# orottier/web-audio-api-rs

Hardware: NVIDIA H100
Metric: offline render-quanta/sec (48kHz stereo, 128-frame) (higher is better)
Workload: dtype f64 filter state / f32 PCM

## Files before the change

### include/wae.h

```cpp
#ifndef WAE_H
#define WAE_H

#include <stddef.h>
#include <stdint.h>

#ifdef __cplusplus
extern "C" {
#endif

#ifndef WAE_API
#define WAE_API __attribute__((visibility("default")))
#endif

#define WAE_RENDER_QUANTUM_SIZE 128u
#define WAE_MAX_CHANNELS 32u

typedef int32_t wae_status;
enum {
    WAE_OK = 0,
    WAE_INVALID_ARGUMENT = 1,
    WAE_INVALID_STATE = 2,
    WAE_NOT_SUPPORTED = 3,
    WAE_UNSUPPORTED = 4,
    WAE_CUDA_ERROR = 5,
    WAE_OUT_OF_MEMORY = 6,
    WAE_NO_DEVICE = 7
};

typedef struct wae_engine wae_engine;
typedef struct wae_graph wae_graph;
typedef uint32_t wae_node_id;

enum { WAE_COUNT_MODE_MAX = 0, WAE_COUNT_MODE_CLAMPED_MAX = 1, WAE_COUNT_MODE_EXPLICIT = 2 };
enum { WAE_INTERPRETATION_SPEAKERS = 0, WAE_INTERPRETATION_DISCRETE = 1 };

typedef struct wae_channel_config {
    uint32_t count;
    uint32_t count_mode;
    uint32_t interpretation;
} wae_channel_config;

typedef struct wae_audio_buffer {
    uint32_t number_of_channels;
    uint64_t length;
    float sample_rate;
    const float* const* channels;
} wae_audio_buffer;


enum { WAE_OSC_SINE = 0, WAE_OSC_SQUARE = 1, WAE_OSC_SAWTOOTH = 2, WAE_OSC_TRIANGLE = 3, WAE_OSC_CUSTOM = 4 };
typedef struct wae_oscillator_options {
    uint32_t type;
    float frequency;
    float detune;
    const float* periodic_wave;
    uint32_t periodic_wave_len;
} wae_oscillator_options;
enum { WAE_OSC_PARAM_FREQUENCY = 0, WAE_OSC_PARAM_DETUNE = 1 };

enum {
    WAE_BIQUAD_LOWPASS = 0, WAE_BIQUAD_HIGHPASS = 1, WAE_BIQUAD_BANDPASS = 2, WAE_BIQUAD_NOTCH = 3,
    WAE_BIQUAD_ALLPASS = 4, WAE_BIQUAD_PEAKING = 5, WAE_BIQUAD_LOWSHELF = 6, WAE_BIQUAD_HIGHSHELF = 7
};
typedef struct wae_biquad_options {
    uint32_t type;
    float q;
    float detune;
    float frequency;
    float gain;
    wae_channel_config channel_config;
} wae_biquad_options;
enum { WAE_BIQUAD_PARAM_Q = 0, WAE_BIQUAD_PARAM_DETUNE = 1, WAE_BIQUAD_PARAM_FREQUENCY = 2, WAE_BIQUAD_PARAM_GAIN = 3 };

typedef struct wae_iir_options {
    const double* feedforward;
    uint32_t feedforward_len;
    const double* feedback;
    uint32_t feedback_len;
    wae_channel_config channel_config;
} wae_iir_options;

typedef struct wae_gain_options {
    float gain;
    wae_channel_config channel_config;
} wae_gain_options;

typedef struct wae_buffer_source_options {
    const wae_audio_buffer* buffer;
    float detune;
    float playback_rate;
    uint32_t loop;
    double loop_start;
    double loop_end;
} wae_buffer_source_options;
enum { WAE_ABSN_PARAM_DETUNE = 0, WAE_ABSN_PARAM_PLAYBACK_RATE = 1 };

typedef struct wae_constant_source_options {
    float offset;
} wae_constant_source_options;

typedef struct wae_convolver_options {
    const wae_audio_buffer* buffer;
    uint32_t disable_normalization;
    wae_channel_config channel_config;
} wae_convolver_options;

enum { WAE_OVERSAMPLE_NONE = 0, WAE_OVERSAMPLE_X2 = 1, WAE_OVERSAMPLE_X4 = 2 };
typedef struct wae_wave_shaper_options {
    const float* curve;
    uint32_t curve_len;
    uint32_t oversample;
    wae_channel_config channel_config;
} wae_wave_shaper_options;

typedef struct wae_delay_options {
    double max_delay_time;
    double delay_time;
    wae_channel_config channel_config;
} wae_delay_options;

typedef struct wae_stereo_panner_options {
    float pan;
    wae_channel_config channel_config;
} wae_stereo_panner_options;

enum { WAE_PANNING_EQUALPOWER = 0, WAE_PANNING_HRTF = 1 };
enum { WAE_DISTANCE_LINEAR = 0, WAE_DISTANCE_INVERSE = 1, WAE_DISTANCE_EXPONENTIAL = 2 };
typedef struct wae_panner_options {
    uint32_t panning_model;
    uint32_t distance_model;
    float position_x, position_y, position_z;
    float orientation_x, orientation_y, orientation_z;
    double ref_distance, max_distance, rolloff_factor;
    double cone_inner_angle, cone_outer_angle, cone_outer_gain;
    wae_channel_config channel_config;
} wae_panner_options;

typedef struct wae_analyser_options {
    uint32_t fft_size;
    double smoothing_time_constant;
    double min_decibels;
    double max_decibels;
    wae_channel_config channel_config;
} wae_analyser_options;

typedef struct wae_dynamics_compressor_options {
    float attack, knee, ratio, release, threshold;
    wae_channel_config channel_config;
} wae_dynamics_compressor_options;

typedef struct wae_channel_merger_options {
    uint32_t number_of_inputs;
} wae_channel_merger_options;
typedef struct wae_channel_splitter_options {
    uint32_t number_of_outputs;
} wae_channel_splitter_options;

enum {
    WAE_EVENT_SET_VALUE = 0,
    WAE_EVENT_SET_VALUE_AT_TIME = 1,
    WAE_EVENT_LINEAR_RAMP_TO_VALUE_AT_TIME = 2,
    WAE_EVENT_EXPONENTIAL_RAMP_TO_VALUE_AT_TIME = 3,
    WAE_EVENT_CANCEL_SCHEDULED_VALUES = 4,
    WAE_EVENT_SET_TARGET_AT_TIME = 5,
    WAE_EVENT_CANCEL_AND_HOLD_AT_TIME = 6,
    WAE_EVENT_SET_VALUE_CURVE_AT_TIME = 7
};
enum { WAE_AUTOMATION_RATE_A = 0, WAE_AUTOMATION_RATE_K = 1 };

typedef struct wae_param_event {
    uint32_t type;
    float value;
    double time;
    double aux;
    const float* values;
    uint32_t values_len;
} wae_param_event;


WAE_API wae_status wae_engine_create(int32_t device_ordinal, wae_engine** out_engine);
WAE_API wae_status wae_engine_destroy(wae_engine* engine);
WAE_API const char* wae_last_error(void);
WAE_API const char* wae_version(void);

enum {
    WAE_OPT_CHUNK_FRAMES = 1,
    WAE_OPT_FUSE = 2,
    WAE_OPT_SERIAL_FILTERS = 3,
    WAE_OPT_PIPELINE_GROUPS = 4,
    WAE_OPT_PARAM_PARALLEL = 5,
    WAE_OPT_BIND_NUMA = 6,
    WAE_OPT_HOST_WORKERS = 7,
    WAE_OPT_CHAIN_TMA = 8,
    WAE_OPT_CHAIN_WAVES = 9,
    WAE_OPT_CHAIN_PREPASS = 10,
    WAE_OPT_VOICE_SUM = 11
};
WAE_API wae_status wae_engine_set_option(wae_engine* engine, uint32_t option, int64_t value);
WAE_API wae_status wae_engine_stream(wae_engine* engine, void** out_stream);


WAE_API wae_status wae_graph_create(wae_engine* engine, uint32_t number_of_channels, uint64_t length,
                                    float sample_rate, wae_graph** out_graph);
WAE_API wae_status wae_graph_render_order(wae_graph* graph, wae_node_id* ids, uint32_t cap, uint32_t* n);
WAE_API wae_status wae_graph_destroy(wae_graph* graph);

WAE_API wae_status wae_create_oscillator(wae_graph*, const wae_oscillator_options*, wae_node_id* out);
WAE_API wae_status wae_create_biquad_filter(wae_graph*, const wae_biquad_options*, wae_node_id* out);
WAE_API wae_status wae_create_iir_filter(wae_graph*, const wae_iir_options*, wae_node_id* out);
WAE_API wae_status wae_create_gain(wae_graph*, const wae_gain_options*, wae_node_id* out);
WAE_API wae_status wae_create_buffer_source(wae_graph*, const wae_buffer_source_options*, wae_node_id* out);
WAE_API wae_status wae_create_constant_source(wae_graph*, const wae_constant_source_options*, wae_node_id* out);
WAE_API wae_status wae_create_convolver(wae_graph*, const wae_convolver_options*, wae_node_id* out);
WAE_API wae_status wae_create_wave_shaper(wae_graph*, const wae_wave_shaper_options*, wae_node_id* out);
WAE_API wae_status wae_create_delay(wae_graph*, const wae_delay_options*, wae_node_id* out);
WAE_API wae_status wae_create_stereo_panner(wae_graph*, const wae_stereo_panner_options*, wae_node_id* out);
WAE_API wae_status wae_create_panner(wae_graph*, const wae_panner_options*, wae_node_id* out);
WAE_API wae_status wae_create_analyser(wae_graph*, const wae_analyser_options*, wae_node_id* out);
WAE_API wae_status wae_create_dynamics_compressor(wae_graph*, const wae_dynamics_compressor_options*, wae_node_id* out);
WAE_API wae_status wae_create_channel_merger(wae_graph*, const wae_channel_merger_options*, wae_node_id* out);
WAE_API wae_status wae_create_channel_splitter(wae_graph*, const wae_channel_splitter_options*, wae_node_id* out);

WAE_API wae_status wae_connect(wae_graph*, wae_node_id from, uint32_t output, wae_node_id to, uint32_t input);
typedef struct wae_param_sim wae_param_sim;
WAE_API wae_status wae_param_sim_create(uint32_t a_rate, float default_value, float min_value, float max_value, wae_param_sim** out);
WAE_API wae_status wae_param_sim_destroy(wae_param_sim* sim);
WAE_API wae_status wae_param_sim_push(wae_param_sim* sim, const wae_param_event* event);
WAE_API wae_status wae_param_sim_set_automation_rate(wae_param_sim* sim, uint32_t a_rate);
WAE_API wae_status wae_param_sim_set_walker(wae_param_sim* sim, uint32_t walker);
WAE_API wae_status wae_param_sim_speculation(wae_param_sim* sim, uint64_t* tried, uint64_t* hits);
WAE_API wae_status wae_param_sim_compute(wae_param_sim* sim, double block_time, double dt, uint32_t count, float* out, uint32_t* len);

WAE_API wae_status wae_graph_suspend(wae_graph* graph, double suspend_time);

WAE_API wae_status wae_connect_param(wae_graph*, wae_node_id from, uint32_t output, wae_node_id to, uint32_t param_index);
WAE_API wae_status wae_disconnect(wae_graph*, wae_node_id from);
#define WAE_NODE_NONE 0xFFFFFFFFu
WAE_API wae_status wae_disconnect_from(wae_graph*, wae_node_id from, int32_t output, wae_node_id to, int32_t input);
WAE_API wae_status wae_disconnect_param(wae_graph*, wae_node_id from, int32_t output, wae_node_id to, uint32_t param_index);

WAE_API wae_status wae_param_event_push(wae_graph*, wae_node_id node, uint32_t param_index, const wae_param_event* event);
WAE_API wae_status wae_param_set_automation_rate(wae_graph*, wae_node_id node, uint32_t param_index, uint32_t rate);
WAE_API wae_status wae_listener_param_event_push(wae_graph*, uint32_t param_index, const wae_param_event* event);

WAE_API wae_status wae_source_start(wae_graph*, wae_node_id node, double when, double offset, double duration);
WAE_API wae_status wae_source_stop(wae_graph*, wae_node_id node, double when);

WAE_API wae_status wae_oscillator_set_type(wae_graph*, wae_node_id node, uint32_t type);
WAE_API wae_status wae_biquad_set_type(wae_graph*, wae_node_id node, uint32_t type);


enum {
    WAE_RENDER_OUT_HOST = 0,
    WAE_RENDER_OUT_DEVICE = 1
};

WAE_API wae_status wae_render_batch(wae_engine* engine, wae_graph* const* graphs, uint32_t n_graphs,
                                    float* out, uint32_t flags);

WAE_API wae_status wae_host_alloc(wae_engine* engine, uint64_t bytes, void** out);
WAE_API wae_status wae_host_free(wae_engine* engine, void* p);
WAE_API wae_status wae_host_register(wae_engine* engine, void* p, uint64_t bytes);
WAE_API wae_status wae_host_unregister(wae_engine* engine, void* p);

WAE_API wae_status wae_selftest_conv_fft(float* data, uint32_t mode);

typedef struct wae_batch wae_batch;
WAE_API wae_status wae_batch_prepare(wae_engine* engine, wae_graph* const* graphs, uint32_t n_graphs, wae_batch** out_batch);
WAE_API wae_status wae_batch_upload(wae_batch* batch);
WAE_API wae_status wae_batch_set_timing(wae_batch* batch, uint32_t per_stage);
WAE_API wae_status wae_batch_run(wae_batch* batch);
WAE_API wae_status wae_batch_run_pipelined(wae_batch* batch, float* host_out);
WAE_API wae_status wae_batch_group_count(wae_batch* batch, uint32_t* n_groups);
WAE_API wae_status wae_batch_group_range(wae_batch* batch, uint32_t group, uint32_t* first_graph, uint32_t* last_graph);
WAE_API wae_status wae_batch_run_group(wae_batch* batch, uint32_t group);
WAE_API wae_status wae_batch_sync(wae_batch* batch);
WAE_API wae_status wae_batch_output_device_ptr(wae_batch* batch, float** out_dev, uint64_t* out_floats);
WAE_API wae_status wae_batch_fetch(wae_batch* batch, float* host_out);
WAE_API wae_status wae_batch_destroy(wae_batch* batch);

typedef struct wae_batch_stats {
    uint64_t kernel_launches_per_run;
    uint64_t stages;
    uint64_t chunks;
    uint64_t arena_bytes;
    uint64_t asset_bytes;
    uint64_t algorithmic_bytes;
    uint64_t graph_quanta;
    float last_run_ms;
    float dominant_kernel_ms;
    char dominant_kernel[64];
} wae_batch_stats;
WAE_API wae_status wae_batch_get_stats(wae_batch* batch, wae_batch_stats* out);
WAE_API wae_status wae_batch_stage_time(wae_batch* batch, uint32_t index, char* name64, float* ms, uint32_t* n_instances);

WAE_API wae_status wae_analyser_get_float_time_domain_data(wae_batch*, uint32_t graph_index, wae_node_id node, float* out, uint32_t len);
WAE_API wae_status wae_analyser_get_float_frequency_data(wae_batch*, uint32_t graph_index, wae_node_id node, float* out, uint32_t len);

WAE_API wae_status wae_engine_set_hrir_sphere(wae_engine* engine, const void* data, uint64_t len);

WAE_API wae_status wae_analyser_get_byte_time_domain_data(wae_batch* batch, uint32_t graph_index, wae_node_id node, uint8_t* out, uint32_t len);
WAE_API wae_status wae_analyser_get_byte_frequency_data(wae_batch* batch, uint32_t graph_index, wae_node_id node, uint8_t* out, uint32_t len);

WAE_API wae_status wae_compressor_reduction(wae_batch* batch, uint32_t graph_index, wae_node_id node, float* out);

WAE_API wae_status wae_resample_linear(wae_engine* engine, const float* in, uint64_t len, float from_rate, float to_rate, float* out,
                                       uint64_t out_cap, uint64_t* out_len);

typedef struct wae_plan_info {
    uint32_t groups;
    uint32_t segments;
    uint32_t stages;
    uint32_t has_feedback;
    uint64_t chunk_frames;
    uint64_t chunks;
    uint64_t arena_floats_per_frame;
    uint64_t source_floats;
    char stage_kinds[512];
} wae_plan_info;
WAE_API wae_status wae_batch_plan(wae_graph* const* graphs, uint32_t n_graphs, wae_plan_info* info);

WAE_API wae_status wae_periodic_wave_table(const float* real, const float* imag, uint32_t len, uint32_t disable_normalization, float* table,
                                           uint32_t table_len);

WAE_API wae_status wae_sched_first_frame_at_or_after(float sample_rate, double time, int64_t* frame, double* frame_time);

WAE_API wae_status wae_spatial_params(uint32_t distance_model, const double* model6, const float* v15, float* out4);

WAE_API int32_t wae_hrtf_locate(const float* pos, const uint32_t* faces, uint32_t n_faces, const float* dir, uint32_t* idx, float* weights);

WAE_API wae_status wae_buffer_source_set_buffer(wae_graph* graph, wae_node_id node, const wae_audio_buffer* buffer);
WAE_API wae_status wae_convolver_set_buffer(wae_graph* graph, wae_node_id node, const wae_audio_buffer* buffer);
WAE_API wae_status wae_wave_shaper_set_curve(wae_graph* graph, wae_node_id node, const float* curve, uint32_t len);
WAE_API wae_status wae_oscillator_set_periodic_wave(wae_graph* graph, wae_node_id node, const float* table, uint32_t len);
enum {
    WAE_ATTR_LOOP = 1, WAE_ATTR_LOOP_START = 2, WAE_ATTR_LOOP_END = 3,
    WAE_ATTR_NORMALIZE = 4,
    WAE_ATTR_OVERSAMPLE = 5,
    WAE_ATTR_PANNING_MODEL = 6, WAE_ATTR_DISTANCE_MODEL = 7, WAE_ATTR_REF_DISTANCE = 8, WAE_ATTR_MAX_DISTANCE = 9,
    WAE_ATTR_ROLLOFF_FACTOR = 10, WAE_ATTR_CONE_INNER_ANGLE = 11, WAE_ATTR_CONE_OUTER_ANGLE = 12, WAE_ATTR_CONE_OUTER_GAIN = 13,
    WAE_ATTR_FFT_SIZE = 14, WAE_ATTR_SMOOTHING_TIME_CONSTANT = 15, WAE_ATTR_MIN_DECIBELS = 16, WAE_ATTR_MAX_DECIBELS = 17
};
WAE_API wae_status wae_node_set_attribute(wae_graph* graph, wae_node_id node, uint32_t attribute, double value);

WAE_API wae_status wae_node_set_channel_count(wae_graph* graph, wae_node_id node, uint32_t count);
WAE_API wae_status wae_node_set_channel_count_mode(wae_graph* graph, wae_node_id node, uint32_t count_mode);
WAE_API wae_status wae_node_set_channel_interpretation(wae_graph* graph, wae_node_id node, uint32_t interpretation);

WAE_API wae_status wae_hrir_resample(const float* hrir, uint32_t len, double ratio, float* out, uint32_t cap, uint32_t* out_len);

WAE_API void wae_biquad_coefs(uint32_t type, double sample_rate, double computed_frequency, double gain, double q, double* out5);
WAE_API void wae_biquad_frequency_response(uint32_t type, float sample_rate, float frequency, float detune, float q, float gain,
                                           const float* frequency_hz, float* mag_response, float* phase_response, uint32_t n);
WAE_API void wae_iir_frequency_response(const double* feedforward, uint32_t n_feedforward, const double* feedback, uint32_t n_feedback,
                                        float sample_rate, const float* frequency_hz, float* mag_response, float* phase_response, uint32_t n);

#ifdef __cplusplus
}
#endif
#endif
```

### web-audio-api-rs_b200/__init__.py

```python
import ctypes
import os

from . import _binding
from ._binding import Api, WaeError
from .context import *
from . import context
from . import parallel

_HERE = os.path.dirname(os.path.abspath(__file__))
LIB_PATH = os.path.join(_HERE, "libwae_b200.so")

_api = None


def api():
    global _api
    if _api is None:
        if not os.path.exists(LIB_PATH):
            raise RuntimeError(f"{LIB_PATH} is missing: run `python -c 'import __graft_entry__ as g; g.build()'` "
                               "(there is no CPU fallback in this package)")
        _api = Api(ctypes.CDLL(LIB_PATH), "wae_")
    return _api


class Engine:

    def __init__(self, device=0):
        a = api()
        h = ctypes.c_void_p()
        a.check(a.engine_create(int(device), ctypes.byref(h)))
        self.handle = h
        self.backend = context.Backend(a, h)
        self.device = device

    def set_option(self, option, value):
        a = api()
        a.check(a.engine_set_option(self.handle, option, int(value)))

    def stream(self):
        a = api()
        p = ctypes.c_void_p()
        a.check(a.engine_stream(self.handle, ctypes.byref(p)))
        return p.value

    def context(self, number_of_channels, length, sample_rate):
        return context.OfflineAudioContext(number_of_channels, length, sample_rate, self.backend)

    def resample(self, samples, from_rate, to_rate):
        import math
        import numpy as np
        a = api()
        x = np.ascontiguousarray(samples, np.float32)
        cap = max(len(x), int(math.ceil(len(x) * (float(to_rate) / float(from_rate)))) + 1)
        out = np.zeros(cap, np.float32)
        n = ctypes.c_uint64(0)
        fp = ctypes.POINTER(ctypes.c_float)
        a.check(a.resample_linear(self.handle, x.ctypes.data_as(fp), len(x), float(from_rate), float(to_rate),
                                  out.ctypes.data_as(fp), cap, ctypes.byref(n)))
        return out[:n.value]

    def close(self):
        if self.handle:
            self.backend.close_batches()
            api().engine_destroy(self.handle)
            self.handle = None


OPT_CHUNK_FRAMES, OPT_FUSE, OPT_SERIAL_FILTERS, OPT_PIPELINE_GROUPS, OPT_PARAM_PARALLEL = 1, 2, 3, 4, 5
OPT_BIND_NUMA, OPT_HOST_WORKERS, OPT_CHAIN_TMA, OPT_CHAIN_WAVES, OPT_CHAIN_PREPASS, OPT_VOICE_SUM = 6, 7, 8, 9, 10, 11
```

### web-audio-api-rs_b200/_binding.py

```python
import ctypes as C

import numpy as np

c_float_p = C.POINTER(C.c_float)
c_double_p = C.POINTER(C.c_double)


class ChannelConfig(C.Structure):
    _fields_ = [("count", C.c_uint32), ("count_mode", C.c_uint32), ("interpretation", C.c_uint32)]


class AudioBufferDesc(C.Structure):
    _fields_ = [("number_of_channels", C.c_uint32), ("length", C.c_uint64), ("sample_rate", C.c_float),
                ("channels", C.POINTER(c_float_p))]


class OscillatorOptions(C.Structure):
    _fields_ = [("type", C.c_uint32), ("frequency", C.c_float), ("detune", C.c_float),
                ("periodic_wave", c_float_p), ("periodic_wave_len", C.c_uint32)]


class BiquadOptions(C.Structure):
    _fields_ = [("type", C.c_uint32), ("q", C.c_float), ("detune", C.c_float), ("frequency", C.c_float),
                ("gain", C.c_float), ("channel_config", ChannelConfig)]


class IirOptions(C.Structure):
    _fields_ = [("feedforward", c_double_p), ("feedforward_len", C.c_uint32), ("feedback", c_double_p),
                ("feedback_len", C.c_uint32), ("channel_config", ChannelConfig)]


class GainOptions(C.Structure):
    _fields_ = [("gain", C.c_float), ("channel_config", ChannelConfig)]


class BufferSourceOptions(C.Structure):
    _fields_ = [("buffer", C.POINTER(AudioBufferDesc)), ("detune", C.c_float), ("playback_rate", C.c_float),
                ("loop", C.c_uint32), ("loop_start", C.c_double), ("loop_end", C.c_double)]


class ConstantSourceOptions(C.Structure):
    _fields_ = [("offset", C.c_float)]


class ConvolverOptions(C.Structure):
    _fields_ = [("buffer", C.POINTER(AudioBufferDesc)), ("disable_normalization", C.c_uint32),
                ("channel_config", ChannelConfig)]


class WaveShaperOptions(C.Structure):
    _fields_ = [("curve", c_float_p), ("curve_len", C.c_uint32), ("oversample", C.c_uint32),
                ("channel_config", ChannelConfig)]


class DelayOptions(C.Structure):
    _fields_ = [("max_delay_time", C.c_double), ("delay_time", C.c_double), ("channel_config", ChannelConfig)]


class StereoPannerOptions(C.Structure):
    _fields_ = [("pan", C.c_float), ("channel_config", ChannelConfig)]


class PannerOptions(C.Structure):
    _fields_ = [("panning_model", C.c_uint32), ("distance_model", C.c_uint32),
                ("position_x", C.c_float), ("position_y", C.c_float), ("position_z", C.c_float),
                ("orientation_x", C.c_float), ("orientation_y", C.c_float), ("orientation_z", C.c_float),
                ("ref_distance", C.c_double), ("max_distance", C.c_double), ("rolloff_factor", C.c_double),
                ("cone_inner_angle", C.c_double), ("cone_outer_angle", C.c_double), ("cone_outer_gain", C.c_double),
                ("channel_config", ChannelConfig)]


class AnalyserOptions(C.Structure):
    _fields_ = [("fft_size", C.c_uint32), ("smoothing_time_constant", C.c_double), ("min_decibels", C.c_double),
                ("max_decibels", C.c_double), ("channel_config", ChannelConfig)]


class DynamicsCompressorOptions(C.Structure):
    _fields_ = [("attack", C.c_float), ("knee", C.c_float), ("ratio", C.c_float), ("release", C.c_float),
                ("threshold", C.c_float), ("channel_config", ChannelConfig)]


class ChannelMergerOptions(C.Structure):
    _fields_ = [("number_of_inputs", C.c_uint32)]


class ChannelSplitterOptions(C.Structure):
    _fields_ = [("number_of_outputs", C.c_uint32)]


class ParamEvent(C.Structure):
    _fields_ = [("type", C.c_uint32), ("value", C.c_float), ("time", C.c_double), ("aux", C.c_double),
                ("values", c_float_p), ("values_len", C.c_uint32)]


(ATTR_LOOP, ATTR_LOOP_START, ATTR_LOOP_END, ATTR_NORMALIZE, ATTR_OVERSAMPLE, ATTR_PANNING_MODEL, ATTR_DISTANCE_MODEL, ATTR_REF_DISTANCE,
 ATTR_MAX_DISTANCE, ATTR_ROLLOFF_FACTOR, ATTR_CONE_INNER_ANGLE, ATTR_CONE_OUTER_ANGLE, ATTR_CONE_OUTER_GAIN, ATTR_FFT_SIZE,
 ATTR_SMOOTHING_TIME_CONSTANT, ATTR_MIN_DECIBELS, ATTR_MAX_DECIBELS) = range(1, 18)


class PlanInfo(C.Structure):
    _fields_ = [("groups", C.c_uint32), ("segments", C.c_uint32), ("stages", C.c_uint32), ("has_feedback", C.c_uint32),
                ("chunk_frames", C.c_uint64), ("chunks", C.c_uint64), ("arena_floats_per_frame", C.c_uint64), ("source_floats", C.c_uint64),
                ("stage_kinds", C.c_char * 512)]


class BatchStats(C.Structure):
    _fields_ = [("kernel_launches_per_run", C.c_uint64), ("stages", C.c_uint64), ("chunks", C.c_uint64),
                ("arena_bytes", C.c_uint64), ("asset_bytes", C.c_uint64), ("algorithmic_bytes", C.c_uint64),
                ("graph_quanta", C.c_uint64), ("last_run_ms", C.c_float), ("dominant_kernel_ms", C.c_float),
                ("dominant_kernel", C.c_char * 64)]


STATUS_NAMES = {0: "OK", 1: "INVALID_ARGUMENT", 2: "INVALID_STATE", 3: "NOT_SUPPORTED", 4: "UNSUPPORTED",
                5: "CUDA_ERROR", 6: "OUT_OF_MEMORY", 7: "NO_DEVICE"}


class WaeError(RuntimeError):

    def __init__(self, status, message):
        super().__init__(f"[{STATUS_NAMES.get(status, status)}] {message}")
        self.status = status
        self.message = message


CREATE_FUNCS = {
    "create_oscillator": OscillatorOptions, "create_biquad_filter": BiquadOptions, "create_iir_filter": IirOptions,
    "create_gain": GainOptions, "create_buffer_source": BufferSourceOptions,
    "create_constant_source": ConstantSourceOptions, "create_convolver": ConvolverOptions,
    "create_wave_shaper": WaveShaperOptions, "create_delay": DelayOptions,
    "create_stereo_panner": StereoPannerOptions, "create_panner": PannerOptions, "create_analyser": AnalyserOptions,
    "create_dynamics_compressor": DynamicsCompressorOptions, "create_channel_merger": ChannelMergerOptions,
    "create_channel_splitter": ChannelSplitterOptions,
}

WAE_SYMBOLS = [
    "wae_engine_create", "wae_engine_destroy", "wae_last_error", "wae_version", "wae_engine_set_option", "wae_engine_stream",
    "wae_graph_create", "wae_graph_destroy",
] + ["wae_" + n for n in CREATE_FUNCS] + [
    "wae_connect", "wae_connect_param", "wae_disconnect", "wae_param_event_push", "wae_param_set_automation_rate",
    "wae_listener_param_event_push", "wae_source_start", "wae_source_stop", "wae_oscillator_set_type",
    "wae_biquad_set_type", "wae_render_batch", "wae_batch_prepare", "wae_batch_upload", "wae_batch_set_timing", "wae_batch_run", "wae_batch_run_pipelined", "wae_batch_sync", "wae_batch_group_count", "wae_batch_group_range", "wae_batch_run_group", "wae_host_alloc", "wae_host_free", "wae_host_register", "wae_host_unregister", "wae_selftest_conv_fft", "wae_param_sim_speculation",
    "wae_batch_output_device_ptr", "wae_batch_fetch", "wae_batch_destroy", "wae_batch_get_stats", "wae_batch_stage_time",
    "wae_analyser_get_float_time_domain_data", "wae_analyser_get_float_frequency_data", "wae_resample_linear", "wae_compressor_reduction", "wae_analyser_get_byte_time_domain_data", "wae_analyser_get_byte_frequency_data", "wae_engine_set_hrir_sphere", "wae_graph_suspend", "wae_param_sim_create", "wae_param_sim_destroy", "wae_param_sim_push",
    "wae_param_sim_set_automation_rate", "wae_param_sim_compute", "wae_biquad_coefs", "wae_biquad_frequency_response", "wae_iir_frequency_response",
    "wae_node_set_channel_count", "wae_node_set_channel_count_mode", "wae_node_set_channel_interpretation", "wae_graph_render_order", "wae_hrir_resample", "wae_batch_plan", "wae_buffer_source_set_buffer", "wae_convolver_set_buffer", "wae_wave_shaper_set_curve",
    "wae_oscillator_set_periodic_wave", "wae_node_set_attribute", "wae_disconnect_from", "wae_disconnect_param", "wae_periodic_wave_table", "wae_param_sim_set_walker", "wae_sched_first_frame_at_or_after", "wae_spatial_params", "wae_hrtf_locate",
]


class Api:

    def __init__(self, lib, prefix):
        self.lib = lib
        self.prefix = prefix
        self.is_product = prefix == "wae_"
        f = self._f
        f("last_error", C.c_char_p, [])
        gp = C.c_void_p
        for name, opt in CREATE_FUNCS.items():
            f(name, C.c_int32, [gp, C.POINTER(opt), C.POINTER(C.c_uint32)])
        f("graph_destroy", C.c_int32, [gp])
        if self.is_product:
            f("graph_render_order", C.c_int32, [gp, C.POINTER(C.c_uint32), C.c_uint32, C.POINTER(C.c_uint32)])
        else:
            f("render_order", C.c_uint32, [gp, C.POINTER(C.c_uint32), C.c_uint32])
        f("graph_suspend", C.c_int32, [gp, C.c_double])
        f("param_sim_create", C.c_int32, [C.c_uint32, C.c_float, C.c_float, C.c_float, C.POINTER(C.c_void_p)])
        f("param_sim_destroy", C.c_int32, [C.c_void_p])
        f("param_sim_push", C.c_int32, [C.c_void_p, C.POINTER(ParamEvent)])
        f("param_sim_set_automation_rate", C.c_int32, [C.c_void_p, C.c_uint32])
        f("param_sim_compute", C.c_int32, [C.c_void_p, C.c_double, C.c_double, C.c_uint32, c_float_p, C.POINTER(C.c_uint32)])
        if self.is_product:
            f("param_sim_set_walker", C.c_int32, [C.c_void_p, C.c_uint32])
            f("param_sim_speculation", C.c_int32, [C.c_void_p, C.POINTER(C.c_uint64), C.POINTER(C.c_uint64)])
            f("selftest_conv_fft", C.c_int32, [c_float_p, C.c_uint32])
            f("sched_first_frame_at_or_after", C.c_int32, [C.c_float, C.c_double, C.POINTER(C.c_int64), C.POINTER(C.c_double)])
        f("connect", C.c_int32, [gp, C.c_uint32, C.c_uint32, C.c_uint32, C.c_uint32])
        f("connect_param", C.c_int32, [gp, C.c_uint32, C.c_uint32, C.c_uint32, C.c_uint32])
        f("disconnect", C.c_int32, [gp, C.c_uint32])
        f("disconnect_from", C.c_int32, [gp, C.c_uint32, C.c_int32, C.c_uint32, C.c_int32])
        f("disconnect_param", C.c_int32, [gp, C.c_uint32, C.c_int32, C.c_uint32, C.c_uint32])
        f("param_event_push", C.c_int32, [gp, C.c_uint32, C.c_uint32, C.POINTER(ParamEvent)])
        f("param_set_automation_rate", C.c_int32, [gp, C.c_uint32, C.c_uint32, C.c_uint32])
        f("listener_param_event_push", C.c_int32, [gp, C.c_uint32, C.POINTER(ParamEvent)])
        f("source_start", C.c_int32, [gp, C.c_uint32, C.c_double, C.c_double, C.c_double])
        f("source_stop", C.c_int32, [gp, C.c_uint32, C.c_double])
        f("oscillator_set_type", C.c_int32, [gp, C.c_uint32, C.c_uint32])
        f("biquad_set_type", C.c_int32, [gp, C.c_uint32, C.c_uint32])
        f("buffer_source_set_buffer", C.c_int32, [gp, C.c_uint32, C.POINTER(AudioBufferDesc)])
        f("convolver_set_buffer", C.c_int32, [gp, C.c_uint32, C.POINTER(AudioBufferDesc)])
        f("wave_shaper_set_curve", C.c_int32, [gp, C.c_uint32, c_float_p, C.c_uint32])
        f("oscillator_set_periodic_wave", C.c_int32, [gp, C.c_uint32, c_float_p, C.c_uint32])
        f("node_set_attribute", C.c_int32, [gp, C.c_uint32, C.c_uint32, C.c_double])
        f("spatial_params", C.c_int32, [C.c_uint32, c_double_p, c_float_p, c_float_p])
        f("hrtf_locate", C.c_int32, [c_float_p, C.POINTER(C.c_uint32), C.c_uint32, c_float_p, C.POINTER(C.c_uint32), c_float_p])
        f("periodic_wave_table", C.c_int32, [c_float_p, c_float_p, C.c_uint32, C.c_uint32, c_float_p, C.c_uint32])
        f("hrir_resample", C.c_int32, [c_float_p, C.c_uint32, C.c_double, c_float_p, C.c_uint32, C.POINTER(C.c_uint32)])
        for name in ("node_set_channel_count", "node_set_channel_count_mode", "node_set_channel_interpretation"):
            f(name, C.c_int32, [gp, C.c_uint32, C.c_uint32])
        f("biquad_coefs", None, [C.c_uint32, C.c_double, C.c_double, C.c_double, C.c_double, c_double_p])
        f("biquad_frequency_response", None, [C.c_uint32, C.c_float, C.c_float, C.c_float, C.c_float, C.c_float,
                                              c_float_p, c_float_p, c_float_p, C.c_uint32])
        f("iir_frequency_response", None, [c_double_p, C.c_uint32, c_double_p, C.c_uint32, C.c_float,
                                           c_float_p, c_float_p, c_float_p, C.c_uint32])
        if self.is_product:
            f("version", C.c_char_p, [])
            f("engine_create", C.c_int32, [C.c_int32, C.POINTER(C.c_void_p)])
            f("engine_destroy", C.c_int32, [C.c_void_p])
            f("engine_set_option", C.c_int32, [C.c_void_p, C.c_uint32, C.c_int64])
            f("engine_stream", C.c_int32, [C.c_void_p, C.POINTER(C.c_void_p)])
            f("graph_create", C.c_int32, [C.c_void_p, C.c_uint32, C.c_uint64, C.c_float, C.POINTER(C.c_void_p)])
            f("render_batch", C.c_int32, [C.c_void_p, C.POINTER(C.c_void_p), C.c_uint32, C.c_void_p, C.c_uint32])
            f("batch_prepare", C.c_int32, [C.c_void_p, C.POINTER(C.c_void_p), C.c_uint32, C.POINTER(C.c_void_p)])
            f("batch_plan", C.c_int32, [C.POINTER(C.c_void_p), C.c_uint32, C.POINTER(PlanInfo)])
            f("batch_upload", C.c_int32, [C.c_void_p])
            f("batch_set_timing", C.c_int32, [C.c_void_p, C.c_uint32])
            f("batch_run", C.c_int32, [C.c_void_p])
            f("batch_run_pipelined", C.c_int32, [C.c_void_p, C.c_void_p])
            f("batch_sync", C.c_int32, [C.c_void_p])
            f("host_alloc", C.c_int32, [C.c_void_p, C.c_uint64, C.POINTER(C.c_void_p)])
            f("host_free", C.c_int32, [C.c_void_p, C.c_void_p])
            f("host_register", C.c_int32, [C.c_void_p, C.c_void_p, C.c_uint64])
            f("host_unregister", C.c_int32, [C.c_void_p, C.c_void_p])
            f("batch_group_count", C.c_int32, [C.c_void_p, C.POINTER(C.c_uint32)])
            f("batch_group_range", C.c_int32, [C.c_void_p, C.c_uint32, C.POINTER(C.c_uint32), C.POINTER(C.c_uint32)])
            f("batch_run_group", C.c_int32, [C.c_void_p, C.c_uint32])
            f("batch_output_device_ptr", C.c_int32, [C.c_void_p, C.POINTER(C.c_void_p), C.POINTER(C.c_uint64)])
            f("batch_fetch", C.c_int32, [C.c_void_p, C.c_void_p])
            f("batch_destroy", C.c_int32, [C.c_void_p])
            f("batch_get_stats", C.c_int32, [C.c_void_p, C.POINTER(BatchStats)])
            f("batch_stage_time", C.c_int32, [C.c_void_p, C.c_uint32, C.c_char_p, c_float_p, C.POINTER(C.c_uint32)])
            f("analyser_get_float_time_domain_data", C.c_int32, [C.c_void_p, C.c_uint32, C.c_uint32, c_float_p, C.c_uint32])
            f("analyser_get_float_frequency_data", C.c_int32, [C.c_void_p, C.c_uint32, C.c_uint32, c_float_p, C.c_uint32])
            f("compressor_reduction", C.c_int32, [C.c_void_p, C.c_uint32, C.c_uint32, c_float_p])
            f("analyser_get_byte_time_domain_data", C.c_int32, [C.c_void_p, C.c_uint32, C.c_uint32, C.POINTER(C.c_uint8), C.c_uint32])
            f("analyser_get_byte_frequency_data", C.c_int32, [C.c_void_p, C.c_uint32, C.c_uint32, C.POINTER(C.c_uint8), C.c_uint32])
            f("engine_set_hrir_sphere", C.c_int32, [C.c_void_p, C.c_void_p, C.c_uint64])
            f("resample_linear", C.c_int32, [C.c_void_p, c_float_p, C.c_uint64, C.c_float, C.c_float, c_float_p, C.c_uint64, C.POINTER(C.c_uint64)])
        else:
            f("graph_create", C.c_int32, [C.c_uint32, C.c_uint64, C.c_float, C.POINTER(C.c_void_p)])
            f("render", C.c_int32, [gp, c_float_p])
            f("render_many", C.c_int32, [C.POINTER(C.c_void_p), C.c_uint32, c_float_p, C.c_uint32, c_double_p])
            f("analyser_get_float_time_domain_data", C.c_int32, [gp, C.c_uint32, c_float_p, C.c_uint32])
            f("analyser_get_float_frequency_data", C.c_int32, [gp, C.c_uint32, c_float_p, C.c_uint32])
            f("analyser_get_byte_frequency_data", C.c_int32, [gp, C.c_uint32, C.POINTER(C.c_uint8), C.c_uint32])
            f("analyser_get_byte_time_domain_data", C.c_int32, [gp, C.c_uint32, C.POINTER(C.c_uint8), C.c_uint32])
            f("compressor_reduction", C.c_int32, [gp, C.c_uint32, c_float_p])
            f("blackman", None, [C.c_uint32, c_float_p])
            f("db_to_lin", C.c_float, [C.c_float])
            f("lin_to_db", C.c_float, [C.c_float])
            f("set_hrir_sphere", C.c_int32, [C.c_void_p, C.c_uint64])
            f("convolver_normalize", C.c_float, [C.POINTER(AudioBufferDesc)])
            f("resample_linear", C.c_uint64, [c_float_p, C.c_uint64, C.c_float, C.c_float, c_float_p, C.c_uint64])
            f("mix", None, [c_float_p, C.c_uint32, C.c_uint32, C.c_uint32, c_float_p])

    def _f(self, name, restype, argtypes):
        fn = getattr(self.lib, self.prefix + name)
        fn.restype = restype
        fn.argtypes = argtypes
        setattr(self, name, fn)

    def check(self, status):
        if status != 0:
            msg = self.last_error()
            raise WaeError(status, msg.decode() if msg else "")


def as_f32(a):
    return np.ascontiguousarray(a, dtype=np.float32)


def fptr(a):
    return a.ctypes.data_as(c_float_p)


def buffer_desc(channels, sample_rate):
    chans = [as_f32(c) for c in channels]
    n = len(chans)
    arr = (c_float_p * n)(*[fptr(c) for c in chans])
    d = AudioBufferDesc(n, len(chans[0]) if n else 0, float(sample_rate), arr)
    return d, (chans, arr)
```

### web-audio-api-rs_b200/csrc/wae_engine.cu

```cuda
#include "wae_graph.h"
#include "wae_hostmath.h"
#include "wae_hrtf_host.h"
#include "wae_resample_host.h"
#include "wae_kernels.h"
#include "wae_param_core.h"
#include "wae_param_host.h"

#include <cuda_runtime.h>
#include <emmintrin.h>

#include <algorithm>
#include <atomic>
#include <chrono>
#include <condition_variable>
#include <cstdlib>
#include <deque>
#include <fstream>
#include <mutex>
#include <sched.h>
#include <sstream>
#include <thread>
#include <cmath>
#include <cstdio>
#include <cstring>
#include <functional>
#include <limits>
#include <map>
#include <memory>
#include <set>
#include <tuple>
#include <unordered_map>
#include <unordered_set>

using namespace wae;
namespace hm = wae::hostmath;

#define CUDA_TRY(expr)                                                                                       \
    do {                                                                                                     \
        cudaError_t _e = (expr);                                                                             \
        if (_e != cudaSuccess) return fail(WAE_CUDA_ERROR, std::string(#expr) + ": " + cudaGetErrorString(_e)); \
    } while (0)

struct WorkerPool {
    std::vector<std::thread> threads;
    std::mutex mu;
    std::condition_variable cv;
    std::deque<std::function<void()>> q;
    bool stop = false;
    WorkerPool(int n, int device) {
        for (int i = 0; i < n; i++)
            threads.emplace_back([this, device] {
                cudaSetDevice(device);
                for (;;) {
                    std::function<void()> f;
                    {
                        std::unique_lock<std::mutex> lk(mu);
                        cv.wait(lk, [this] { return stop || !q.empty(); });
                        if (q.empty()) return;
                        f = std::move(q.front());
                        q.pop_front();
                    }
                    f();
                }
            });
    }
    ~WorkerPool() {
        {
            std::lock_guard<std::mutex> lk(mu);
            stop = true;
        }
        cv.notify_all();
        for (auto& t : threads) t.join();
    }
    void submit(std::function<void()> f) {
        {
            std::lock_guard<std::mutex> lk(mu);
            q.push_back(std::move(f));
        }
        cv.notify_one();
    }
    int size() const { return (int)threads.size(); }
    void parallel_for(int n, const std::function<void(int)>& fn) {
        if (n <= 0) return;
        std::mutex dm;
        std::condition_variable dcv;
        int left = n;
        for (int i = 0; i < n; i++)
            submit([&, i] {
                fn(i);
                std::lock_guard<std::mutex> lk(dm);
                if (--left == 0) dcv.notify_all();
            });
        std::unique_lock<std::mutex> lk(dm);
        dcv.wait(lk, [&] { return left == 0; });
    }
};

struct wae_engine {
    int device = 0;
    cudaStream_t stream = nullptr;
    cudaStream_t s_h2d = nullptr, s_d2h = nullptr;
    int64_t chunk_frames = 0;
    bool fuse = true;
    int voice_sum = -1;
    bool serial_filters = false;
    int pipeline_groups = 0;
    int param_parallel = 2;
    float* d_sine = nullptr;
    wae::HrirSphere* sphere = nullptr;
    float* d_sphere_ir = nullptr;
    float* d_sphere_pos = nullptr;
    uint32_t* d_sphere_tri = nullptr;
    struct RateSphere {
        float* d_ir = nullptr;
        uint32_t taps = 0;
        std::vector<float> ir_host;
    };
    std::map<uint32_t, RateSphere> sphere_rates;
    std::mutex sphere_mu;
    void drop_rate_spheres() {
        for (auto& kv : sphere_rates)
            if (kv.second.d_ir) cudaFree(kv.second.d_ir);
        sphere_rates.clear();
    }
    std::mutex mem_mu;
    std::multimap<size_t, void*> dev_free;
    std::unordered_map<void*, size_t> dev_size;
    size_t dev_cached_bytes = 0;
    static size_t round_block(size_t b) {
        if (b < 512) return 512;
        if (b < ((size_t)1 << 16)) return (b + 511) / 512 * 512;
        if (b < ((size_t)2 << 20)) return (b + 65535) / 65536 * 65536;
        return (b + (((size_t)2 << 20) - 1)) / ((size_t)2 << 20) * ((size_t)2 << 20);
    }
    void* dev_alloc(size_t bytes, bool* fresh = nullptr) {
        const size_t r = round_block(bytes);
        {
            std::lock_guard<std::mutex> lk(mem_mu);
            auto it = dev_free.lower_bound(r);
            if (it != dev_free.end() && it->first <= r + std::max<size_t>(r / 8, 4096)) {
                void* p = it->second;
                dev_cached_bytes -= it->first;
                dev_free.erase(it);
                if (fresh) *fresh = false;
                return p;
            }
        }
        void* p = nullptr;
        if (cudaMalloc(&p, r) != cudaSuccess) {
            cudaGetLastError();
            dev_trim();
            if (cudaMalloc(&p, r) != cudaSuccess) {
                cudaGetLastError();
                return nullptr;
            }
        }
        std::lock_guard<std::mutex> lk(mem_mu);
        dev_size[p] = r;
        if (fresh) *fresh = true;
        return p;
    }
    void dev_release(void* p) {
        std::lock_guard<std::mutex> lk(mem_mu);
        auto it = dev_size.find(p);
        if (it == dev_size.end()) return;
        dev_free.emplace(it->second, p);
        dev_cached_bytes += it->second;
    }
    void dev_trim() {
        std::lock_guard<std::mutex> lk(mem_mu);
        for (auto& kv : dev_free) {
            cudaFree(kv.second);
            dev_size.erase(kv.second);
        }
        dev_free.clear();
        dev_cached_bytes = 0;
    }
    WorkerPool* pool = nullptr;
    int n_workers = 0;
    WorkerPool* workers() {
        if (!pool) {
            int n = n_workers;
            if (n <= 0) {
                const unsigned hw = std::thread::hardware_concurrency();
                n = (int)std::min<unsigned>(16u, std::max<unsigned>(2u, hw / 8u));
            }
            pool = new WorkerPool(n, device);
        }
        return pool;
    }
    static constexpr int kStageSlots = 4;
    float* h_stage[kStageSlots] = {nullptr, nullptr, nullptr, nullptr};
    size_t h_stage_bytes = 0;
    bool ensure_stage(size_t bytes) {
        if (h_stage_bytes >= bytes) return true;
        for (int i = 0; i < kStageSlots; i++) {
            if (h_stage[i]) cudaFreeHost(h_stage[i]);
            h_stage[i] = nullptr;
        }
        h_stage_bytes = 0;
        for (int i = 0; i < kStageSlots; i++)
            if (cudaHostAlloc((void**)&h_stage[i], bytes, cudaHostAllocDefault) != cudaSuccess) {
                cudaGetLastError();
                return false;
            }
        h_stage_bytes = bytes;
        return true;
    }
    char* h_ring = nullptr;
    size_t h_ring_bytes = 0;
    bool ensure_ring(size_t bytes) {
        if (h_ring_bytes >= bytes) return true;
        if (h_ring) cudaFreeHost(h_ring);
        h_ring = nullptr;
        h_ring_bytes = 0;
        if (cudaHostAlloc((void**)&h_ring, bytes, cudaHostAllocDefault) != cudaSuccess) {
            cudaGetLastError();
            return false;
        }
        h_ring_bytes = bytes;
        return true;
    }
    std::string numa_cpus;
};

namespace wae {
int engine_device(const wae_engine* eng) { return eng ? eng->device : 0; }
}

namespace {

enum StageKind : int {
    S_MIX = 0, S_MIX_DYN, S_OSC, S_CONST, S_ABSN, S_BIQUAD, S_IIR, S_GAIN, S_SHAPER, S_SPAN, S_PAN, S_ROUTE, S_DELAY_MONO, S_DELAY, S_DELAY_WRITE, S_COMP, S_ANALYSER,
    S_CONV_FFT, S_CONV_MAC, S_CONV_MAC_ACC, S_CHAIN, S_PARAM, S_OSC_AR, S_BIQUAD_AR, S_ABSN_SLOW, S_HRTF, S_PAN_DYN, S_ABSN_SERIAL, S_SHAPER_OS, S_META, S_VSUM, S_CONV_CMP, S_KINDS
};
const char* kStageNames[S_KINDS] = {"k_mix", "k_mix_dyn", "k_oscillator", "k_constant", "k_buffer_source", "k_biquad_serial", "k_iir_serial", "k_gain",
                                    "k_shaper", "k_stereo_panner", "k_panner_eq", "k_route", "k_delay_mono", "k_delay_read", "k_ring_write", "k_compressor",
                                    "k_analyser", "k_conv_fft_in", "k_conv_mac_ifft", "k_conv_mac_ifft(acc)", "k_chain", "k_param", "k_osc_arate", "k_biquad_arate", "k_buffer_source_slow", "k_hrtf_fir", "k_panner_dyn", "k_buffer_source_serial", "k_shaper_os", "k_meta", "k_voice_sum", "k_conv_compact"};

struct StageBuild {
    int cls = 0;
    int level = 0;
    int kind = 0;
    int variant = 0;
    std::vector<OscInst> osc;
    std::vector<ConstInst> cst;
    std::vector<AbsnInst> absn;
    std::vector<BiquadInst> biquad;
    std::vector<ChainInst> chain;
    std::vector<ParamInst> param;
    std::vector<OscArInst> osc_ar;
    std::vector<BiquadArInst> biquad_ar;
    std::vector<AbsnSlowInst> absn_slow;
    std::vector<ScanCoef> scan_coef;
    size_t n_scan_coef = 0;
    template <typename MakeFn>
    int32_t add_scan_coef(bool build, MakeFn&& make) {
        if (build) scan_coef.push_back(make());
        return (int32_t)n_scan_coef++;
    }
    std::vector<IirInst> iir;
    std::vector<GainInst> gain;
    std::vector<ShaperInst> shaper;
    std::vector<SPanInst> span;
    std::vector<float2> span_gains;
    std::vector<PanInst> pan;
    std::vector<HrtfInst> hrtf;
    std::vector<HrtfSelInst> hrtf_sel;
    std::vector<PanDynInst> pan_dyn;
    std::vector<AbsnSerialInst> absn_serial;
    std::vector<ShaperOsInst> shaper_os;
    std::vector<RouteInst> route;
    std::vector<DelayInst> delay;
    std::vector<CompInst> comp;
    std::vector<AnalyserInst> analyser;
    std::vector<MixInst> mix;
    std::vector<MixEdge> mix_edges;
    std::vector<MixDynInst> mix_dyn;
    std::vector<MetaInst> meta;
    std::vector<ConvInput> conv_in;
    std::vector<ConvPath> conv_path;
    std::vector<ConvCmpInst> conv_cmp;
    std::vector<VoiceGroup> vgroups;
    int max_ch = 1;
};

struct Stage {
    int cls = 0;
    int seg = 0;
    int kind = 0;
    int variant = 0;
    int group = 0;
    int n = 0;
    int n_b = 0;
    int max_ch = 1;
    void* d_a = nullptr;
    void* d_b = nullptr;
    void* d_c = nullptr;
    float ms = 0.f;
    ChainAux chain;
};

struct AnalyserRec {
    uint32_t graph_index;
    uint32_t node;
    float* d_ring;
    uint32_t fft_size;
    double smoothing;
    float* d_last_fft;
    float* d_db;
    bool computed;
    double min_db, max_db;
};

}

struct wae_batch {
    wae_engine* engine = nullptr;
    uint32_t n_graphs = 0, channels = 0;
    uint64_t length = 0;
    int64_t lq = 0;
    int64_t chunk = 0;
    std::vector<void*> allocs;
    std::vector<Stage> stages;
    float* d_out = nullptr;
    std::vector<std::pair<void*, size_t>> zero_on_run;
    std::vector<AnalyserRec> analysers;
    struct CompRec { uint32_t graph; wae_node_id node; const float* d_state; };
    std::vector<CompRec> compressors;
    struct Group {
        uint32_t g0 = 0, g1 = 0;
        size_t stage0 = 0, stage1 = 0;
        std::vector<std::pair<size_t, size_t>> seg_stages;
        std::vector<int64_t> seg_bounds;
        float* d_src = nullptr;
        float* h_src = nullptr;
        struct SrcCopy {
            std::shared_ptr<PcmBuffer> buf;
            size_t offset, floats;
        };
        std::vector<SrcCopy> src_copies;
        std::vector<size_t> graph_src_base;
        size_t src_floats = 0;
        cudaEvent_t ev_h2d = nullptr, ev_done = nullptr;
    };
    std::vector<Group> groups;
    struct StateKey {
        uint32_t graph, node, seq;
        uint64_t salt;
        bool operator<(const StateKey& o) const { return std::tie(graph, node, seq, salt) < std::tie(o.graph, o.node, o.seq, o.salt); }
    };
    std::map<StateKey, std::pair<void*, size_t>> state_map;
    std::vector<void*> pinned;
    cudaStream_t s_h2d = nullptr, s_d2h = nullptr;
    std::recursive_mutex mu;
    struct Timed {
        size_t stage, e0, e1;
    };
    std::vector<Timed> timed;
    wae_batch_stats stats{};
    cudaEvent_t ev0 = nullptr, ev1 = nullptr;
    std::vector<cudaEvent_t> stage_events;
    bool time_stages = false;
    size_t timed_events_used = 0;
    std::atomic<uint64_t> arena_bytes{0}, asset_bytes{0};
    uint64_t n_cuda_malloc = 0;

    char* slab = nullptr;
    size_t slab_used = 0, slab_cap = 0;
    void* slab_alloc(size_t bytes) {
        bytes = (bytes + 255) / 256 * 256;
        if (bytes > (1u << 20)) return nullptr;
        if (!slab || slab_used + bytes > slab_cap) {
            slab_cap = 8u << 20;
            bool fresh = false;
            void* p = engine->dev_alloc(slab_cap, &fresh);
            if (!p) return nullptr;
            n_cuda_malloc += fresh ? 1 : 0;
            allocs.push_back(p);
            cudaMemsetAsync(p, 0, slab_cap, engine->stream);
            zero_on_run.push_back({p, slab_cap});
            slab = (char*)p;
            slab_used = 0;
        }
        void* r = slab + slab_used;
        slab_used += bytes;
        return r;
    }
    char* tslab = nullptr;
    size_t tslab_used = 0, tslab_cap = 0;
    void* table_alloc(size_t bytes) {
        bytes = (bytes + 255) / 256 * 256;
        if (bytes > (512u << 10)) return nullptr;
        if (!tslab || tslab_used + bytes > tslab_cap) {
            tslab_cap = 4u << 20;
            bool fresh = false;
            void* p = engine->dev_alloc(tslab_cap, &fresh);
            if (!p) return nullptr;
            n_cuda_malloc += fresh ? 1 : 0;
            allocs.push_back(p);
            tslab = (char*)p;
            tslab_used = 0;
        }
        void* r = tslab + tslab_used;
        tslab_used += bytes;
        return r;
    }
    template <typename T>
    T* dalloc(size_t count, bool zero = false, bool rezero_on_run = false) {
        std::lock_guard<std::recursive_mutex> lk(mu);
        if (rezero_on_run && count * sizeof(T) <= (1u << 20)) {
            void* r = slab_alloc(count * sizeof(T));
            if (r) return (T*)r;
        }
        size_t bytes = count * sizeof(T);
        if (bytes == 0) bytes = 16;
        if (!rezero_on_run) {
            void* r = table_alloc(bytes);
            if (r) {
                if (zero) cudaMemsetAsync(r, 0, bytes, engine->stream);
                return (T*)r;
            }
        }
        bool fresh = false;
        void* p = engine->dev_alloc(bytes, &fresh);
        if (!p) return nullptr;
        n_cuda_malloc += fresh ? 1 : 0;
        allocs.push_back(p);
        if (zero || rezero_on_run) cudaMemsetAsync(p, 0, bytes, engine->stream);
        if (rezero_on_run) zero_on_run.push_back({p, bytes});
        return (T*)p;
    }
    char* uslab = nullptr;
    std::vector<char> uslab_host;
    size_t uslab_used = 0, uslab_cap = 0, uslab_flushed = 0;
    void flush_uploads() {
        std::lock_guard<std::recursive_mutex> lk(mu);
        if (uslab && uslab_used > uslab_flushed) {
            cudaMemcpyAsync(uslab + uslab_flushed, uslab_host.data() + uslab_flushed, uslab_used - uslab_flushed, cudaMemcpyHostToDevice, engine->stream);
            uslab_flushed = uslab_used;
        }
    }
    void* upload_alloc(size_t bytes) {
        bytes = (bytes + 255) / 256 * 256;
        if (bytes > (512u << 10)) return nullptr;
        if (!uslab || uslab_used + bytes > uslab_cap) {
            flush_uploads();
            bool fresh = false;
            void* p = engine->dev_alloc(4u << 20, &fresh);
            if (!p) return nullptr;
            n_cuda_malloc += fresh ? 1 : 0;
            allocs.push_back(p);
            uslab = (char*)p;
            uslab_cap = 4u << 20;
            uslab_used = uslab_flushed = 0;
            if (uslab_host.size() != uslab_cap) uslab_host.assign(uslab_cap, 0);
        }
        void* r = uslab + uslab_used;
        uslab_used += bytes;
        return r;
    }
    template <typename T>
    T* dupload(const std::vector<T>& v) {
        std::lock_guard<std::recursive_mutex> lk(mu);
        const size_t bytes = v.size() * sizeof(T);
        if (bytes > 0)
            if (void* r = upload_alloc(bytes)) {
                std::memcpy(uslab_host.data() + ((char*)r - uslab), v.data(), bytes);
                return (T*)r;
            }
        return dupload_now(v);
    }
    template <typename T>
    T* dupload_now(const std::vector<T>& v) {
        std::lock_guard<std::recursive_mutex> lk(mu);
        T* p = dalloc<T>(v.size());
        if (p && !v.empty()) cudaMemcpyAsync(p, v.data(), v.size() * sizeof(T), cudaMemcpyHostToDevice, engine->stream);
        return p;
    }
};

namespace {

struct EdgeTable {
    std::vector<const std::vector<Edge>*> v;
    std::vector<char> has;
    static const std::vector<Edge>& none() {
        static const std::vector<Edge> e;
        return e;
    }
    void reset(uint32_t max_id) {
        v.assign((size_t)max_id + 1, &none());
        has.assign((size_t)max_id + 1, 0);
    }
    void set(uint32_t id, const std::vector<Edge>* edges) {
        if (id >= v.size()) {
            v.resize((size_t)id + 1, &none());
            has.resize((size_t)id + 1, 0);
        }
        has[id] = 1;
        v[id] = edges;
    }
    void clear(uint32_t id) { set(id, &none()); }
    bool count(uint32_t id) const { return id < v.size() && has[id]; }
    const std::vector<Edge>* find(uint32_t id) const { return count(id) ? v[id] : nullptr; }
    const std::vector<Edge>& at(uint32_t id) const {
        if (!count(id)) throw std::out_of_range("orderer: unknown node id");
        return *v[id];
    }
};

struct Orderer {
    wae_graph* g;
    EdgeTable edges;
    std::vector<uint32_t> ordered, marked, marked_temp, in_cycle, cycle_breakers, broken;
    static bool contains(const std::vector<uint32_t>& v, uint32_t x) { return std::find(v.begin(), v.end(), x) != v.end(); }
    struct IdSet {
        std::vector<char> f;
        void reset(size_t n) { f.assign(n, 0); }
        bool count(uint32_t id) const { return id < f.size() && f[id]; }
        bool insert(uint32_t id) {
            if (id >= f.size()) f.resize((size_t)id + 1, 0);
            const bool fresh = !f[id];
            f[id] = 1;
            return fresh;
        }
        void erase(uint32_t id) { if (id < f.size()) f[id] = 0; }
    };
    IdSet marked_set, temp_set;
    bool visit(uint32_t id) {
        if (temp_set.count(id)) {
            auto it = std::find(marked_temp.begin(), marked_temp.end(), id);
            for (auto jt = it; jt != marked_temp.end(); ++jt)
                if (g->nodes.at(*jt).cycle_breaker) {
                    cycle_breakers.push_back(*jt);
                    return true;
                }
            in_cycle.insert(in_cycle.end(), it, marked_temp.end());
            return false;
        }
        if (!marked_set.insert(id)) return false;
        marked_temp.push_back(id);
        temp_set.insert(id);
        const std::vector<Edge>& out = edges.at(id);
        for (size_t i = 0; i < out.size(); i++)
            if (edges.count(out[i].other_id) && visit(out[i].other_id)) return true;
        ordered.push_back(id);
        if (!marked_temp.empty() && marked_temp.back() == id) marked_temp.pop_back();
        else marked_temp.erase(std::remove(marked_temp.begin(), marked_temp.end(), id), marked_temp.end());
        temp_set.erase(id);
        return false;
    }
    void run() {
        edges.reset(g->nodes.empty() ? 0 : g->nodes.max_id());
        for (auto& kv : g->nodes) edges.set(kv.first, &kv.second.outgoing);
        ordered.reserve(g->nodes.size());
        for (;;) {
            ordered.clear(); marked.clear(); marked_temp.clear(); in_cycle.clear(); cycle_breakers.clear();
            marked_set.reset(edges.v.size()); temp_set.reset(edges.v.size());
            bool applied = false;
            for (auto& kv : g->nodes) {
                applied = visit(kv.first);
                if (applied) break;
            }
            if (!applied) break;
            for (uint32_t id : cycle_breakers) {
                edges.clear(id);
                if (!contains(broken, id)) broken.push_back(id);
            }
        }
        if (!in_cycle.empty()) {
            std::unordered_set<uint32_t> muted(in_cycle.begin(), in_cycle.end());
            ordered.erase(std::remove_if(ordered.begin(), ordered.end(), [&](uint32_t o) { return muted.count(o) != 0; }), ordered.end());
        }
        std::reverse(ordered.begin(), ordered.end());
    }
};

struct PortRef {
    uint32_t node;
    int port;
};

struct Lay {
    uint8_t lo = 1, hi = 1, nlo = 1, nhi = 1;
    bool may_silent = false;
    bool dyn() const { return lo != hi || may_silent; }
    static Lay fixed(int ch) { return Lay{(uint8_t)ch, (uint8_t)ch, (uint8_t)ch, (uint8_t)ch, false}; }
    static Lay gated(int ch) { return Lay{1, (uint8_t)ch, (uint8_t)ch, (uint8_t)ch, true}; }
};

struct PNode {
    Node* n = nullptr;
    int level = 0;
    std::vector<std::vector<PortRef>> in_edges;
    std::vector<int> in_ch;
    std::vector<BufRef> in_buf;
    std::vector<Lay> in_lay;
    std::vector<int> out_ch;
    std::vector<BufRef> out_buf;
    std::vector<Lay> out_lay;
    bool wrote_dest = false;
    Lay lay_out(int port) const { return port < (int)out_lay.size() ? out_lay[port] : Lay::fixed(out_ch[port]); }
};

struct NodeTable {
    std::vector<PNode> v;
    std::vector<char> has;
    void reset(uint32_t max_id) {
        if (v.size() < (size_t)max_id + 1) v.resize((size_t)max_id + 1);
        has.assign(v.size(), 0);
    }
    PNode& put(uint32_t id, Node* n) {
        if (id >= v.size()) {
            v.resize((size_t)id + 1);
            has.resize((size_t)id + 1, 0);
        }
        PNode& p = v[id];
        p.n = n;
        p.level = 0;
        p.in_edges.resize((size_t)n->n_inputs);
        for (auto& port : p.in_edges) port.clear();
        p.in_ch.clear();
        p.in_buf.clear();
        p.in_lay.clear();
        p.out_ch.clear();
        p.out_buf.clear();
        p.out_lay.clear();
        p.wrote_dest = false;
        has[id] = 1;
        return p;
    }
    PNode* find(uint32_t id) { return id < v.size() && has[id] ? &v[id] : nullptr; }
    bool count(uint32_t id) const { return id < v.size() && has[id]; }
    PNode& at(uint32_t id) {
        if (!(id < v.size() && has[id])) throw std::out_of_range("planner: unknown node id");
        return v[id];
    }
};

struct Planner {
    wae_batch* b;
    wae_engine* eng;
    std::map<std::pair<int, int>, StageBuild> builds;
    std::string error;
    int error_code = 0;
    uint64_t algorithmic_bytes = 0;
    struct IrSpectra {
        float2* h;
        int S;
        int channels;
    };
    std::unordered_map<uint64_t, IrSpectra> own_ir_cache;
    std::unordered_map<uint64_t, IrSpectra>* ir_cache = &own_ir_cache;
    std::map<int, std::pair<const float2*, const float2*>> os_filters;

    bool has_feedback = false;
    std::map<std::pair<uint32_t, uint32_t>, int>* delay_ch_hint = nullptr;
    std::map<std::pair<uint32_t, uint32_t>, int> delay_ch_seen;
    struct DelayRing {
        float* ring;
        uint32_t ring_len;
        int ch;
        int64_t* mono_at;
        int32_t mono_len;
    };
    std::map<std::pair<uint32_t, uint32_t>, DelayRing> delay_rings;
    std::map<std::pair<uint32_t, uint32_t>, int> conv_paths_seen;
    bool dry = false;
    int group_graphs = 1;
    int vs_mode = -1;
    int voice_sum_mode() {
        if (eng->voice_sum >= 0) return eng->voice_sum;
        if (vs_mode < 0) {
            const char* e = getenv("WAE_VOICE_SUM");
            vs_mode = e ? std::max(0, std::min(2, atoi(e))) : 0;
        }
        return vs_mode;
    }
    uint64_t arena_floats_per_frame = 0;
    float* d_src = nullptr;
    std::vector<wae_batch::Group::SrcCopy>* src_copies = nullptr;
    size_t src_cursor = 0;
    struct PendingChain {
        ChainInst inst;
        hm::BiquadCoefs coefs[CHAIN_MAX_BIQUADS] = {};
        int ch = 1;
        int phase = 0;
        int cls = 0;
        Lay lay;
    };

    uint32_t key_graph = 0, key_node = 0, key_seq = 0;
    uint64_t key_salt = 0;
    template <typename T>
    T* alloc(size_t count, bool zero = false, bool rezero_on_run = false) {
        if (dry) return reinterpret_cast<T*>(uintptr_t(256));
        if (seg_start == 0 && seg_end >= b->lq) return b->dalloc<T>(count, zero, rezero_on_run);
        const wae_batch::StateKey key{key_graph, key_node, key_seq++, key_salt};
        const size_t bytes = count * sizeof(T);
        std::lock_guard<std::recursive_mutex> lk(b->mu);
        auto it = b->state_map.find(key);
        if (it != b->state_map.end() && it->second.second == bytes) return (T*)it->second.first;
        T* p = b->dalloc<T>(count, zero, rezero_on_run);
        if (p) b->state_map[key] = {(void*)p, bytes};
        return p;
    }
    std::map<int, std::vector<float*>> arena_pool;
    std::map<int, size_t> arena_used;
    std::map<std::pair<uint32_t, uint32_t>, size_t> src_offsets;
    std::unordered_map<const PcmBuffer*, size_t> buf_offsets;
    struct ParamRecord {
        size_t n_source_events = 0;
        ParamTimeline tl;
        int64_t init_frame = 0;
    };
    std::unordered_map<uint64_t, ParamRecord> param_records;
    const ParamTimeline* param_timeline(uint32_t gi, uint32_t pid, const Param& prm, float sample_rate) {
        const uint64_t rec_key = (uint64_t)gi << 32 | pid;
        auto it = param_records.find(rec_key);
        if (it == param_records.end()) {
            ParamRecord r;
            r.tl = build_param_timeline(prm);
            r.n_source_events = prm.events.size();
            r.init_frame = seg_start;
            return &param_records.emplace(rec_key, std::move(r)).first->second.tl;
        }
        ParamRecord& r = it->second;
        if (r.n_source_events == prm.events.size() || !r.tl.error.empty()) return &r.tl;
        ParamInst host{};
        host.events = r.tl.events.data();
        host.curves = r.tl.curves.data();
        host.n_events = (int32_t)r.tl.events.size();
        host.a_rate = prm.a_rate ? 1 : 0;
        host.sample_rate = sample_rate;
        ParamState st{};
        st.intrinsic = r.tl.intrinsic;
        st.has_last = r.tl.has_last ? 1 : 0;
        st.last = r.tl.last;
        st.inited = 1;
        float buf[128];
        for (int64_t f = r.init_frame; f < seg_start; f += 128) param_compute_buffer(host, st, (double)f / (double)sample_rate, buf);
        ParamTimeline next;
        next.curves = r.tl.curves;
        for (int i = st.head; i < host.n_events; i++) next.events.push_back(i == st.head && st.override_valid ? st.override_ev : r.tl.events[i]);
        next.intrinsic = st.intrinsic;
        next.has_last = st.has_last != 0;
        next.last = st.last;
        fold_param_events(next, prm.events.data() + r.n_source_events, prm.events.size() - r.n_source_events);
        r.tl = std::move(next);
        r.n_source_events = prm.events.size();
        r.init_frame = seg_start;
        return &r.tl;
    }
    int64_t seg_start = 0, seg_end = 0;
    void begin_segment(int64_t f0, int64_t f1) {
        seg_start = f0;
        seg_end = f1;
        builds.clear();
        arena_used.clear();
        arena_floats_per_frame = 0;
    }
    template <typename T>
    T* upload(const std::vector<T>& v) {
        if (dry) return reinterpret_cast<T*>(uintptr_t(256));
        return b->dupload(v);
    }

    bool bail(int code, const std::string& msg) {
        if (!error_code) {
            error_code = code;
            error = msg;
        }
        return false;
    }

    int cur_cls = 0;
    StageBuild& stage(int level, int kind, int variant = 0) {
        const int cls = cur_cls;
        StageBuild& s = builds[{cls * 1000000 + level, kind * 64 + variant}];
        s.cls = cls;
        s.level = level;
        s.kind = kind;
        s.variant = variant;
        return s;
    }

    BufRef arena_buf(int ch, bool with_meta = false) {
        arena_floats_per_frame += (uint64_t)ch;
        const uint32_t mstride = (uint32_t)((b->chunk / 128 + 16) / 16 * 16);
        BufRef r{reinterpret_cast<float*>(uintptr_t(256)), (uint32_t)b->chunk, 0, nullptr, 0, 0};
        if (!dry) {
            std::vector<float*>& pool = arena_pool[ch];
            size_t& used = arena_used[ch];
            if (used < pool.size()) {
                r.p = pool[used++];
            } else {
                const size_t floats = (size_t)ch * (size_t)b->chunk;
                float* p = b->dalloc<float>(floats + ((size_t)ch * mstride + 3) / 4);
                b->arena_bytes += floats * 4;
                if (p) {
                    pool.push_back(p);
                    used++;
                }
                r.p = p;
            }
        }
        if (with_meta && r.p) {
            r.meta = reinterpret_cast<uint8_t*>(r.p + (size_t)ch * (size_t)b->chunk);
            r.meta_stride = mstride;
        }
        return r;
    }
    void meta_stage(int L, int mode, const BufRef& in, int in_ch, const BufRef& out, int out_ch, int count = 0, int aux = 0) {
        MetaInst m{};
        m.in = in;
        m.out = out;
        m.mode = mode;
        m.in_ch = in_ch;
        m.out_ch = out_ch;
        m.count = count;
        m.aux = aux;
        stage(L, S_META).meta.push_back(m);
    }

    NodeTable node_table;
    NodeTable* cur_pn = nullptr;
    struct PRef {
        bool dyn = false;
        float v = 0.f;
        BufRef track{nullptr, 0, 0};
    };
    PRef param_ref(wae_graph* g, uint32_t pid);
    bool plan_graph(wae_graph* g, uint32_t gi);
    bool plan_convolver(wae_graph* g, PNode& pn, int level, const BufRef* dest = nullptr, int64_t dest_limit = -1, const PcmBuffer* ir_override = nullptr);
};

static uint64_t fnv1a(const void* data, size_t bytes, uint64_t h = 1469598103934665603ull) {
    const uint8_t* p = (const uint8_t*)data;
    size_t n8 = bytes / 8;
    const uint64_t* q = (const uint64_t*)p;
    for (size_t i = 0; i < n8; i++) {
        h ^= q[i];
        h *= 1099511628211ull;
    }
    for (size_t i = n8 * 8; i < bytes; i++) {
        h ^= p[i];
        h *= 1099511628211ull;
    }
    return h;
}

static bool plan_digest_wanted() {
    static const bool on = [] { const char* e = getenv("WAE_PLAN_DIGEST"); return e && atoi(e) != 0; }();
    return on;
}
template <typename T>
static uint64_t digest_vec(const std::vector<T>& v, uint64_t h) {
    const uint64_t n = v.size();
    h = fnv1a(&n, sizeof n, h);
    if (v.empty()) return h;
    static const bool dump = [] { const char* e = getenv("WAE_PLAN_DIGEST"); return e && atoi(e) >= 2; }();
    if (dump) {
        std::fprintf(stderr, "  [%s] n %zu size %zu:", __PRETTY_FUNCTION__, v.size(), sizeof(T));
        const uint64_t* q = (const uint64_t*)v.data();
        for (size_t i = 0; i < sizeof(T) / 8 && i < 400; i++) std::fprintf(stderr, " %llx", (unsigned long long)q[i]);
        std::fprintf(stderr, "\n");
    }
    return fnv1a(v.data(), v.size() * sizeof(T), h);
}
static uint64_t digest_builds(const std::map<std::pair<int, int>, StageBuild>& builds, uint64_t h) {
    for (auto& kv : builds) {
        const StageBuild& s = kv.second;
        const int key[6] = {kv.first.first, kv.first.second, s.cls, s.level, s.kind * 64 + s.variant, s.max_ch};
        h = fnv1a(key, sizeof key, h);
        h = digest_vec(s.osc, h); h = digest_vec(s.cst, h); h = digest_vec(s.absn, h); h = digest_vec(s.biquad, h); h = digest_vec(s.chain, h);
        h = digest_vec(s.param, h); h = digest_vec(s.osc_ar, h); h = digest_vec(s.biquad_ar, h); h = digest_vec(s.absn_slow, h);
        h = digest_vec(s.scan_coef, h); h = digest_vec(s.iir, h); h = digest_vec(s.gain, h); h = digest_vec(s.shaper, h); h = digest_vec(s.span, h);
        h = digest_vec(s.span_gains, h); h = digest_vec(s.pan, h); h = digest_vec(s.hrtf, h); h = digest_vec(s.hrtf_sel, h); h = digest_vec(s.pan_dyn, h);
        h = digest_vec(s.absn_serial, h); h = digest_vec(s.shaper_os, h); h = digest_vec(s.route, h); h = digest_vec(s.delay, h); h = digest_vec(s.comp, h);
        h = digest_vec(s.analyser, h); h = digest_vec(s.mix, h); h = digest_vec(s.mix_edges, h); h = digest_vec(s.mix_dyn, h); h = digest_vec(s.meta, h);
        h = digest_vec(s.conv_in, h); h = digest_vec(s.conv_path, h); h = digest_vec(s.vgroups, h);
        if (!s.conv_cmp.empty()) h = digest_vec(s.conv_cmp, h);
    }
    return h;
}

using Builds = std::map<std::pair<int, int>, StageBuild>;
template <typename T>
static void append_vec(std::vector<T>& d, std::vector<T>& s) {
    if (d.empty()) d = std::move(s);
    else d.insert(d.end(), s.begin(), s.end());
}
static void merge_builds(Builds& dst, Builds& src) {
    struct Base {
        size_t mix_edges = 0, scan = 0, chain = 0, conv_in = 0;
    };
    std::map<std::pair<int, int>, Base> base;
    for (auto& kv : src) {
        auto it = dst.find(kv.first);
        if (it != dst.end()) base[kv.first] = Base{it->second.mix_edges.size(), it->second.n_scan_coef, it->second.chain.size(), it->second.conv_in.size()};
        else base[kv.first] = Base{};
    }
    for (auto& kv : src) {
        StageBuild& s = kv.second;
        const Base bs = base[kv.first];
        for (auto& m : s.mix) m.edge_offset += (uint32_t)bs.mix_edges;
        for (auto& m : s.mix_dyn) m.edge_offset += (uint32_t)bs.mix_edges;
        for (auto& c : s.chain)
            for (int k = 0; k < c.n_biquad; k++) c.bq[k].coef += (int32_t)bs.scan;
        for (auto& v : s.vgroups) v.first += (int32_t)bs.chain;
        if (s.kind == S_CONV_MAC || s.kind == S_CONV_MAC_ACC) {
            const std::pair<int, int> fft_key{kv.first.first, S_CONV_FFT * 64};
            size_t off = 0;
            auto bi = base.find(fft_key);
            if (bi != base.end()) off = bi->second.conv_in;
            else if (dst.count(fft_key)) off = dst[fft_key].conv_in.size();
            for (auto& cp : s.conv_path) cp.input += (int32_t)off;
        }
        auto it = dst.find(kv.first);
        if (it == dst.end()) {
            dst.emplace(kv.first, std::move(s));
            continue;
        }
        StageBuild& d = it->second;
        append_vec(d.osc, s.osc); append_vec(d.cst, s.cst); append_vec(d.absn, s.absn); append_vec(d.biquad, s.biquad); append_vec(d.chain, s.chain);
        append_vec(d.param, s.param); append_vec(d.osc_ar, s.osc_ar); append_vec(d.biquad_ar, s.biquad_ar); append_vec(d.absn_slow, s.absn_slow);
        append_vec(d.scan_coef, s.scan_coef); append_vec(d.iir, s.iir); append_vec(d.gain, s.gain); append_vec(d.shaper, s.shaper); append_vec(d.span, s.span);
        append_vec(d.span_gains, s.span_gains); append_vec(d.pan, s.pan); append_vec(d.hrtf, s.hrtf); append_vec(d.hrtf_sel, s.hrtf_sel);
        append_vec(d.pan_dyn, s.pan_dyn); append_vec(d.absn_serial, s.absn_serial); append_vec(d.shaper_os, s.shaper_os); append_vec(d.route, s.route);
        append_vec(d.delay, s.delay); append_vec(d.comp, s.comp); append_vec(d.analyser, s.analyser); append_vec(d.mix, s.mix);
        append_vec(d.mix_edges, s.mix_edges); append_vec(d.mix_dyn, s.mix_dyn); append_vec(d.meta, s.meta); append_vec(d.conv_in, s.conv_in);
        append_vec(d.conv_path, s.conv_path); append_vec(d.vgroups, s.vgroups); append_vec(d.conv_cmp, s.conv_cmp);
        d.n_scan_coef += s.n_scan_coef;
        d.max_ch = std::max(d.max_ch, s.max_ch);
    }
}

static int computed_channels(const ChannelCfg& cfg, int max_in) {
    switch (cfg.mode) {
        case WAE_COUNT_MODE_MAX: return max_in;
        case WAE_COUNT_MODE_EXPLICIT: return cfg.count;
        default: return std::min(max_in, cfg.count);
    }
}

static uint32_t next_pow2(uint64_t v) {
    uint32_t p = 1;
    while (p < v) p <<= 1;
    return p;
}

static ScanCoef make_scan_coef(const hm::BiquadCoefs& c) {
    ScanCoef sc{};
    struct M2 {
        double a, b, c, d;
    };
    auto mul = [](const M2& x, const M2& y) { return M2{x.a * y.a + x.b * y.c, x.a * y.b + x.b * y.d, x.c * y.a + x.d * y.c, x.c * y.b + x.d * y.d}; };
    const M2 M{-c.a1, -c.a2, 1., 0.};
    M2 r{1., 0., 0., 1.};
    for (int j = 0; j < WAE_CHAIN_K; j++) r = mul(M, r);
    const M2 A = r;
    M2 pw = A;
    for (int d = 0; d < 5; d++) {
        sc.Pshfl[d][0] = pw.a; sc.Pshfl[d][1] = pw.b; sc.Pshfl[d][2] = pw.c; sc.Pshfl[d][3] = pw.d;
        pw = mul(pw, pw);
    }
    sc.Pwarp[0] = pw.a; sc.Pwarp[1] = pw.b; sc.Pwarp[2] = pw.c; sc.Pwarp[3] = pw.d;
    M2 pl = A;
    for (int l = 0; l < 32; l++) {
        sc.Plane[l][0] = pl.a; sc.Plane[l][1] = pl.b; sc.Plane[l][2] = pl.c; sc.Plane[l][3] = pl.d;
        pl = mul(A, pl);
    }
    static_assert(WAE_CHAIN_PRE_TILES * WAE_CHAIN_K * 128 == 1 << 15, "GL below is G^(2^15)");
    double g[16] = {0., 0., 0., 0., 1., 0., 0., 0., c.b1, c.b2, -c.a1, -c.a2, 0., 0., 1., 0.}, h[16];
    for (int sq = 0; sq < 15; sq++) {
        for (int r = 0; r < 4; r++)
            for (int cc = 0; cc < 4; cc++) {
                double a = 0.;
                for (int k = 0; k < 4; k++) a += g[4 * r + k] * g[4 * k + cc];
                h[4 * r + cc] = a;
            }
        std::memcpy(g, h, sizeof g);
    }
    std::memcpy(sc.GL, g, sizeof g);
    return sc;
}

bool Planner::plan_convolver(wae_graph* g, PNode& pn, int level, const BufRef* dest, int64_t dest_limit, const PcmBuffer* ir_override) {
    Node& n = *pn.n;
    int in_ch = pn.in_ch[0];
    const bool mono_mix = ir_override && in_ch == 2;
    if (mono_mix) in_ch = 1;
    if ((n.buffer || ir_override) && cur_cls == 1)
        return bail(WAE_UNSUPPORTED, "a ConvolverNode inside a DelayNode feedback cycle is not lowered to the GPU (before or after the cycle it is)");
    const Lay in_lay = pn.in_lay.empty() ? Lay::fixed(in_ch) : pn.in_lay[0];
    if (!n.buffer && !ir_override) {
        pn.out_ch = {in_ch};
        pn.out_buf = {pn.in_buf[0]};
        pn.out_lay = {in_lay};
        return true;
    }
    const PcmBuffer& ir = ir_override ? *ir_override : *n.buffer;
    int ir_ch = (int)ir.channels.size();
    size_t ir_len = ir.length();
    float scale = 1.f;
    if (n.normalize && !ir_override) {
        float power = 0.f;
        for (auto& c : ir.channels) {
            float s = 0.f;
            for (float v : c) s += v * v;
            power += s;
        }
        power = std::sqrt(power / (float)((size_t)ir_ch * ir_len));
        if (!std::isfinite(power) || power < 0.000125f) power = 0.000125f;
        scale = 1.f / power;
        scale *= 0.00125f;
        scale *= 44100.f / ir.sample_rate;
        if (ir_ch == 4) scale *= 0.5f;
    }
    int n_conv = std::max(ir_ch, 2);
    std::vector<std::vector<float>> scaled(ir_ch);
    size_t trimmed_len = 0;
    for (int c = 0; c < ir_ch; c++) {
        scaled[c].resize(ir_len);
        for (size_t i = 0; i < ir_len; i++) scaled[c][i] = ir.channels[c][i] * scale;
    }
    std::vector<int> S(ir_ch);
    for (int c = 0; c < ir_ch; c++) {
        size_t m = ir_len;
        while (!ir_override && m > 0 && std::fabs(scaled[c][m - 1]) < 0.000001f) m--;
        while (ir_override && m > 0 && scaled[c][m - 1] == 0.f) m--;
        S[c] = (int)((m + WAE_CONV_BLOCK - 1) / WAE_CONV_BLOCK);
        trimmed_len = std::max(trimmed_len, m);
        for (size_t i = m; i < ir_len; i++) scaled[c][i] = 0.f;
    }
    int Smax = *std::max_element(S.begin(), S.end());
    pn.out_ch = {ir_ch == 1 && in_ch == 1 ? 1 : 2};
    const bool compact = in_lay.dyn() && ir_ch == 1 && in_lay.hi >= 2;
    if (compact && in_ch != 2) return bail(WAE_UNSUPPORTED, "unsupported convolver channel routing");
    if (ir_ch == 1 && in_ch == 2 && !ir_override) {
        int& seen = conv_paths_seen[{key_graph, key_node}];
        seen |= compact ? 1 : 2;
        if (seen == 3)
            return bail(WAE_UNSUPPORTED, "a ConvolverNode with a mono response whose input changes between a constant two-channel layout and a "
                                         "changing one at a suspend point is not lowered to the GPU (its second convolver's history would not "
                                         "carry over, convolver.rs:378-400)");
    }
    const uint32_t key_base = key_seq;
    auto role = [&](uint32_t r) { key_seq = key_base + r; };
    const bool conv_dyn = in_lay.dyn();
    const bool direct = dest && !conv_dyn && Smax > 0 && pn.out_ch[0] == (int)b->channels;
    pn.out_buf = {direct ? *dest : arena_buf(pn.out_ch[0], conv_dyn && Smax > 0)};
    pn.wrote_dest = direct;
    if (conv_dyn && Smax > 0) {
        const int oc = pn.out_ch[0];
        pn.out_lay = {Lay{(uint8_t)(in_lay.may_silent ? 1 : oc), (uint8_t)oc, (uint8_t)oc, (uint8_t)oc, in_lay.may_silent}};
        if (compact)
            pn.out_lay = {Lay{(uint8_t)(in_lay.may_silent || in_lay.lo < 2 ? 1 : 2), 2,
                              (uint8_t)(in_lay.may_silent || in_lay.nlo < 2 ? 1 : 2), 2, in_lay.may_silent}};
        MetaInst m{};
        m.in = pn.in_buf[0];
        m.out = pn.out_buf[0];
        m.mode = META_CONV;
        m.in_ch = in_ch;
        m.out_ch = oc;
        m.aux = ir_ch;
        m.tail_len = (int64_t)ir_len;
        role(0);
        m.state = alloc<int64_t>(1, true, true);
        if (!m.state) return bail(WAE_OUT_OF_MEMORY, "out of device memory (convolver tail counter)");
        stage(level, S_META).meta.push_back(m);
    }
    if (Smax == 0) {
        StageBuild& ms = stage(level, S_MIX);
        ms.mix.push_back(MixInst{pn.out_buf[0], pn.out_ch[0], 0, 0, (uint32_t)ms.mix_edges.size(), -1});
        return true;
    }
    uint64_t key = fnv1a(&scale, sizeof(scale));
    for (int c = 0; c < ir_ch; c++) key = fnv1a(ir.channels[c].data(), ir_len * sizeof(float), key);
    key = fnv1a(&ir_len, sizeof(ir_len), key);
    IrSpectra spec;
    std::unique_lock<std::recursive_mutex> ir_lock(b->mu);
    auto it = ir_cache->find(key);
    if (it != ir_cache->end()) {
        spec = it->second;
    } else {
        std::vector<float> flat((size_t)ir_ch * ir_len);
        for (int c = 0; c < ir_ch; c++) std::memcpy(flat.data() + (size_t)c * ir_len, scaled[c].data(), ir_len * sizeof(float));
        float* d_ir = dry ? upload(flat) : b->dupload_now(flat);
        if (!dry) cudaStreamSynchronize(eng->stream);
        spec.S = Smax;
        spec.channels = ir_ch;
        spec.h = dry ? alloc<float2>(1) : b->dalloc<float2>((size_t)ir_ch * (Smax + WAE_CONV_H_PAD) * WAE_CONV_SPEC, true);
        if (!d_ir || !spec.h) return bail(WAE_OUT_OF_MEMORY, "out of device memory (IR spectra)");
        if (!dry) launch_conv_ir_fft(d_ir, (int64_t)ir_len, (int64_t)ir_len, spec.h, Smax, ir_ch, eng->stream);
        b->asset_bytes += (size_t)ir_ch * (Smax + WAE_CONV_H_PAD) * WAE_CONV_SPEC * 8;
        (*ir_cache)[key] = spec;
    }
    ir_lock.unlock();
    StageBuild& fs = stage(level, S_CONV_FFT);
    int blocks_per_chunk = (int)((b->chunk + WAE_CONV_BLOCK - 1) / WAE_CONV_BLOCK);
    int ring_blocks = Smax + blocks_per_chunk;
    int in_base = (int)fs.conv_in.size();
    for (int c = 0; c < (compact ? 1 : in_ch); c++) {
        ConvInput ci;
// ... 1230 lines not shown
                        h.sel = si.sel;
                        hs.hrtf_sel.push_back(si);
                    } else {
                        float proj[3];
                        spatial::projected_source(sp0, proj);
                        const float dir[3] = {proj[0], proj[2], proj[1]};
                        h.static_sel = HrtfSel{{0, 0, 0}, {0.f, 0.f, 0.f}, sp0.cone_gain * sp0.dist_gain, 0.f};
                        sph->locate(dir, h.static_sel.v, h.static_sel.w);
                    }
                    hs.hrtf.push_back(h);
                    break;
                }
                if (moving) {
                    PanDynInst d{};
                    d.in = p.in_buf[0];
                    d.out = p.out_buf[0];
                    d.sp = tr;
                    d.model = model;
                    d.in_ch = ch;
                    stage(L, S_PAN_DYN).pan_dyn.push_back(d);
                    break;
                }
                PanInst pi{};
                pi.in = p.in_buf[0];
                pi.out = p.out_buf[0];
                pi.in_ch = ch;
                pi.azimuth = sp0.azimuth;
                pi.dist_gain = sp0.dist_gain;
                pi.cone_gain = sp0.cone_gain;
                stage(L, S_PAN).pan.push_back(pi);
                break;
            }
            case K_DELAY_W: {
                p.out_ch = {p.in_ch[0]};
                p.out_buf = {p.in_buf[0]};
                p.out_lay = {in0};
                if (Orderer::contains(ord.broken, id)) {
                    delay_ch_seen[{gi, n.delay_peer}] = p.in_ch[0];
                    auto it = delay_rings.find({gi, id});
                    if (it == delay_rings.end()) return bail(WAE_UNSUPPORTED, "DelayNode writer processed before its reader inside a cycle");
                    if (it->second.ch != p.in_ch[0]) {
                        if (!dry) return bail(WAE_UNSUPPORTED, "channel layout of a DelayNode in a feedback cycle did not converge");
                        break;
                    }
                    DelayInst d{};
                    d.in = p.in_buf[0];
                    d.ch = it->second.ch;
                    d.ring = it->second.ring;
                    d.ring_len = it->second.ring_len;
                    d.mono_at = it->second.mono_at;
                    d.mono_len = it->second.mono_len;
                    d.dyn = it->second.mono_at ? 3 : 0;
                    stage(L, S_DELAY_WRITE).delay.push_back(d);
                }
                break;
            }
            case K_DELAY_R: {
                PRef pdl = param_ref(g, n.params[0]);
                float dt = pdl.v;
                const bool in_cycle = Orderer::contains(ord.broken, n.delay_peer);
                int ch = p.in_ch[0];
                if (in_cycle) {
                    ch = 1;
                    if (delay_ch_hint) {
                        auto it = delay_ch_hint->find({gi, id});
                        if (it != delay_ch_hint->end()) ch = it->second;
                    }
                }
                if (!need_out(ch)) return bail(WAE_OUT_OF_MEMORY, "out of device memory (arena)");
                DelayInst d{};
                d.in = p.in_buf[0];
                d.out = p.out_buf[0];
                d.ch = ch;
                d.in_cycle = in_cycle ? 1 : 0;
                if (pdl.dyn) d.delay_track = pdl.track;
                d.sample_rate = g->sample_rate;
                double delay = (double)dt;
                if (in_cycle) delay = std::max(delay, 128. / sr);
                double num_samples = delay * sr;
                double position = 0. - num_samples;
                double pf = std::floor(position);
                d.fl = (int64_t)pf;
                d.k = (float)(position - pf);
                uint64_t max_frames = (uint64_t)std::ceil(std::max(n.max_delay_time, 128. / sr) * sr) + 2;
                d.ring_len = next_pow2(max_frames + 128);
                d.ring = alloc<float>((size_t)ch * d.ring_len, true, true);
                if (!d.ring) return bail(WAE_OUT_OF_MEMORY, "out of device memory (delay ring)");
                b->arena_bytes += (size_t)ch * d.ring_len * 4;
                if (ch <= 2) {
                    d.dyn = 1;
                    d.mono_len = (int32_t)next_pow2((uint64_t)(b->chunk / 128 + 2));
                    d.mono_at = alloc<int64_t>((size_t)d.mono_len, true, true);
                    if (!d.mono_at) return bail(WAE_OUT_OF_MEMORY, "out of device memory (delay layout track)");
                    const Lay wl = in_cycle ? Lay{1, (uint8_t)ch, 1, (uint8_t)ch, true} : in0;
                    out_dynamic(Lay{1, (uint8_t)ch, (uint8_t)(wl.dyn() ? 1 : ch), (uint8_t)ch, true});
                    d.out = p.out_buf[0];
                    if (!in_cycle) stage(L, S_DELAY_MONO).delay.push_back(d);
                }
                stage(L, S_DELAY).delay.push_back(d);
                if (in_cycle) delay_rings[{gi, n.delay_peer}] = DelayRing{d.ring, d.ring_len, ch, d.mono_at, d.mono_len};
                else stage(L, S_DELAY_WRITE).delay.push_back(d);
                break;
            }
            case K_COMP: {
                PRef cp[5];
                for (int i = 0; i < 5; i++) cp[i] = param_ref(g, n.params[i]);
                const float at = cp[0].v, kn = cp[1].v, ra = cp[2].v, re = cp[3].v, th = cp[4].v;
                int ch = p.in_ch[0];
                if (!need_out(ch)) return bail(WAE_OUT_OF_MEMORY, "out of device memory (arena)");
                CompInst c{};
                c.in = p.in_buf[0];
                c.out = p.out_buf[0];
                c.ch = ch;
                int ring_size = (int)std::ceil(g->sample_rate * 0.006f / 128.f) + 1;
                c.delay_frames = (ring_size - 1) * 128;
                c.ring_len = next_pow2((uint64_t)c.delay_frames + 128);
                c.ring = alloc<float>((size_t)ch * c.ring_len, true, true);
                c.state = alloc<float>(2, true, true);
                c.meta_ring = alloc<uint8_t>(8, true, true);
                if (!c.ring || !c.state || !c.meta_ring) return bail(WAE_OUT_OF_MEMORY, "out of device memory (compressor)");
                out_dynamic(Lay{1, in0.hi, in0.nlo, in0.nhi, true});
                c.out = p.out_buf[0];
                c.threshold = th; c.knee = kn; c.ratio = ra; c.attack = at; c.release = re;
                for (int i = 0; i < 5; i++) c.track[i] = cp[i].dyn ? cp[i].track : BufRef{nullptr, 0, 0};
                c.sample_rate = g->sample_rate;
                stage(L, S_COMP).comp.push_back(c);
                if (!dry) {
                    std::lock_guard<std::recursive_mutex> lk(b->mu);
                    bool known = false;
                    for (auto& r : b->compressors) known = known || (r.graph == gi && r.node == id);
                    if (!known) b->compressors.push_back(wae_batch::CompRec{gi, id, c.state});
                }
                break;
            }
            case K_ANALYSER: {
                int ch = p.in_ch[0];
                p.out_ch = {ch};
                p.out_buf = {p.in_buf[0]};
                p.out_lay = {in0};
                AnalyserInst a{};
                a.in = p.in_buf[0];
                a.out = BufRef{nullptr, 0, 0};
                a.ch = ch;
                a.ring = alloc<float>(32768 + 128, true, true);
                if (!a.ring) return bail(WAE_OUT_OF_MEMORY, "out of device memory (analyser ring)");
                stage(L, S_ANALYSER).analyser.push_back(a);
                {
                    float* last = alloc<float>(16384, true, true);
                    float* db = alloc<float>(16384);
                    if (!last || !db) return bail(WAE_OUT_OF_MEMORY, "out of device memory (analyser)");
                    if (!dry) {
                        std::lock_guard<std::recursive_mutex> lk(b->mu);
                        bool known = false;
                        for (auto& r : b->analysers) known = known || (r.graph_index == gi && r.node == id);
                        if (!known) b->analysers.push_back(AnalyserRec{gi, id, a.ring, n.fft_size, n.smoothing, last, db, false, n.min_db, n.max_db});
                    }
                }
                algorithmic_bytes += (uint64_t)b->lq * 4;
                break;
            }
            case K_MERGER: {
                int k = n.n_inputs;
                if (!need_out(k)) return bail(WAE_OUT_OF_MEMORY, "out of device memory (arena)");
                {
                    bool some_always_on = false, any_dyn = false;
                    for (int i = 0; i < k; i++) {
                        some_always_on = some_always_on || !p.in_lay[i].may_silent;
                        any_dyn = any_dyn || p.in_lay[i].dyn();
                    }
                    if (any_dyn && !some_always_on) {
                        out_dynamic(Lay{1, (uint8_t)k, (uint8_t)k, (uint8_t)k, true});
                        if (p.out_buf[0].meta) {
                            MetaInst m{};
                            m.out = p.out_buf[0];
                            m.mode = META_MERGE;
                            m.out_ch = k;
                            m.count = k;
                            m.n_more = k;
                            m.more = upload(p.in_buf);
                            if (!m.more) return bail(WAE_OUT_OF_MEMORY, "out of device memory (merger inputs)");
                            stage(L, S_META).meta.push_back(m);
                        }
                    }
                }
                for (int i = 0; i < k; i++) stage(L, S_ROUTE).route.push_back(RouteInst{p.in_buf[i], p.out_buf[0], 0, i, 0, 1});
                break;
            }
            case K_SPLITTER: {
                int k = n.n_outputs;
                p.out_ch.assign(k, 1);
                p.out_buf.resize(k);
                p.out_lay.assign(k, Lay::fixed(1));
                for (int i = 0; i < k; i++) {
                    if (i < p.in_ch[0] && in0.dyn()) {
                        p.out_buf[i] = arena_buf(1, true);
                        if (!p.out_buf[i].p) return bail(WAE_OUT_OF_MEMORY, "out of device memory (arena)");
                        p.out_lay[i] = Lay{1, 1, 1, 1, true};
                        stage(L, S_ROUTE).route.push_back(RouteInst{p.in_buf[0], p.out_buf[i], i, 0, 0, p.in_ch[0]});
                        meta_stage(L, META_SPLIT, p.in_buf[0], p.in_ch[0], p.out_buf[i], 1, 0, i);
                    } else if (i < p.in_ch[0]) {
                        BufRef r = p.in_buf[0];
                        r.p += (size_t)i * r.stride;
                        p.out_buf[i] = r;
                    } else {
                        p.out_buf[i] = arena_buf(1);
                        stage(L, S_ROUTE).route.push_back(RouteInst{p.in_buf[0], p.out_buf[i], 0, 0, 1, 0});
                    }
                }
                break;
            }
            case K_CONV: {
                const BufRef* dest = nullptr;
                BufRef fin{b->d_out + (size_t)gi * b->channels * b->length, (uint32_t)b->length, 1};
                if (fuse && cur_cls == 0 && b->length <= 0xffffffffull) {
                    int n_out = 0;
                    uint32_t to = 0;
                    int to_port = -1;
                    for (auto& e : ord.edges.at(id))
                        if (e.other_index >= 0) n_out++, to = e.other_id, to_port = e.other_index;
                    if (n_out == 1 && to_port == 0 && g->nodes.at(to).kind == K_DEST && pn.at(to).in_edges[0].size() == 1 &&
                        computed_channels(g->nodes.at(to).cfg, (n.buffer && n.buffer->channels.size() == 1 && p.in_ch[0] == 1) ? 1 : 2) == (int)b->channels)
                        dest = &fin;
                }
                if (!plan_convolver(g, p, L, dest, (int64_t)b->length)) return false;
                break;
            }
            default: return bail(WAE_UNSUPPORTED, "node kind not lowered to the GPU");
        }
    }
    while (!pending.empty())
        if (!materialize(pending.begin()->first)) return false;
    return true;
}

template <typename T>
static void* up(wae_batch* b, const std::vector<T>& v) {
    return (void*)b->dupload(v);
}

struct EpochView {
    wae_graph* g;
    size_t e;
    EpochView(wae_graph* g_, int64_t frame) : g(g_), e(0) {
        while (e < g->epochs.size() && (int64_t)g->epochs[e].frame <= frame) e++;
        if (e < g->epochs.size()) std::swap(g->nodes, g->epochs[e].nodes);
    }
    ~EpochView() {
        if (e < g->epochs.size()) std::swap(g->nodes, g->epochs[e].nodes);
    }
    EpochView(const EpochView&) = delete;
    EpochView& operator=(const EpochView&) = delete;
};

static bool bind_to_device_numa_node(wae_engine* eng) {
    char bus[64] = {0};
    if (cudaDeviceGetPCIBusId(bus, sizeof bus, eng->device) != cudaSuccess) {
        cudaGetLastError();
        return false;
    }
    for (char* c = bus; *c; c++) *c = (char)std::tolower((unsigned char)*c);
    std::ifstream f(std::string("/sys/bus/pci/devices/") + bus + "/local_cpulist");
    std::string list;
    if (!f || !std::getline(f, list) || list.empty()) return false;
    cpu_set_t set;
    CPU_ZERO(&set);
    std::stringstream ss(list);
    std::string part;
    int n = 0;
    while (std::getline(ss, part, ',')) {
        int a = 0, b2 = 0;
        if (std::sscanf(part.c_str(), "%d-%d", &a, &b2) == 2) {
            for (int c = a; c <= b2 && c < CPU_SETSIZE; c++, n++) CPU_SET(c, &set);
        } else if (std::sscanf(part.c_str(), "%d", &a) == 1 && a < CPU_SETSIZE) {
            CPU_SET(a, &set);
            n++;
        }
    }
    if (n == 0 || sched_setaffinity(0, sizeof set, &set) != 0) return false;
    eng->numa_cpus = list;
    return true;
}

}

extern "C" {

WAE_API wae_status wae_engine_create(int32_t device_ordinal, wae_engine** out) {
    if (!out) return fail(WAE_INVALID_ARGUMENT, "null out pointer");
    int count = 0;
    cudaError_t e = cudaGetDeviceCount(&count);
    if (e != cudaSuccess || count == 0)
        return fail(WAE_NO_DEVICE, std::string("no CUDA device usable (") + cudaGetErrorString(e) + "): this library has no CPU fallback");
    if (device_ordinal < 0 || device_ordinal >= count) return fail(WAE_NO_DEVICE, "device ordinal out of range");
    CUDA_TRY(cudaSetDevice(device_ordinal));
    cudaDeviceProp prop;
    CUDA_TRY(cudaGetDeviceProperties(&prop, device_ordinal));
    if (prop.major != 9 || prop.minor != 0) return fail(WAE_NO_DEVICE, "the kernels are built for sm_90a (H100) only");
    set_num_sms(prop.multiProcessorCount);
    auto* eng = new wae_engine;
    eng->device = device_ordinal;
    CUDA_TRY(cudaStreamCreateWithFlags(&eng->stream, cudaStreamNonBlocking));
    CUDA_TRY(cudaStreamCreateWithFlags(&eng->s_h2d, cudaStreamNonBlocking));
    CUDA_TRY(cudaStreamCreateWithFlags(&eng->s_d2h, cudaStreamNonBlocking));
    if (const char* e = getenv("WAE_BIND_NUMA"))
        if (atoi(e) != 0) bind_to_device_numa_node(eng);
    std::vector<float> sine = hm::sine_table();
    CUDA_TRY(cudaMalloc(&eng->d_sine, sine.size() * sizeof(float)));
    CUDA_TRY(cudaMemcpy(eng->d_sine, sine.data(), sine.size() * sizeof(float), cudaMemcpyHostToDevice));
    upload_twiddles();
    CUDA_TRY(cudaDeviceSynchronize());
    *out = eng;
    return WAE_OK;
}

WAE_API wae_status wae_engine_destroy(wae_engine* eng) {
    if (!eng) return WAE_OK;
    cudaSetDevice(eng->device);
    if (eng->d_sine) cudaFree(eng->d_sine);
    if (eng->d_sphere_ir) cudaFree(eng->d_sphere_ir);
    if (eng->d_sphere_pos) cudaFree(eng->d_sphere_pos);
    if (eng->d_sphere_tri) cudaFree(eng->d_sphere_tri);
    eng->drop_rate_spheres();
    delete eng->sphere;
    delete eng->pool;
    eng->dev_trim();
    for (int i = 0; i < wae_engine::kStageSlots; i++)
        if (eng->h_stage[i]) cudaFreeHost(eng->h_stage[i]);
    if (eng->h_ring) cudaFreeHost(eng->h_ring);
    if (eng->stream) cudaStreamDestroy(eng->stream);
    if (eng->s_h2d) cudaStreamDestroy(eng->s_h2d);
    if (eng->s_d2h) cudaStreamDestroy(eng->s_d2h);
    delete eng;
    return WAE_OK;
}

WAE_API wae_status wae_engine_set_hrir_sphere(wae_engine* eng, const void* data, uint64_t len) {
    if (!eng) return fail(WAE_INVALID_ARGUMENT, "null engine");
    auto* sp = new HrirSphere();
    std::string err;
    if (!sp->parse(static_cast<const uint8_t*>(data), len, err)) {
        delete sp;
        return fail(WAE_INVALID_ARGUMENT, err.c_str());
    }
    CUDA_TRY(cudaSetDevice(eng->device));
    float* d = nullptr;
    if (cudaMalloc(&d, sp->ir.size() * sizeof(float)) != cudaSuccess) {
        delete sp;
        return fail(WAE_OUT_OF_MEMORY, "out of device memory (HRIR sphere)");
    }
    float* dpos = nullptr;
    uint32_t* dtri = nullptr;
    if (cudaMalloc(&dpos, sp->pos.size() * sizeof(float)) != cudaSuccess || cudaMalloc(&dtri, sp->tri.size() * sizeof(uint32_t)) != cudaSuccess) {
        cudaFree(d);
        if (dpos) cudaFree(dpos);
        delete sp;
        return fail(WAE_OUT_OF_MEMORY, "out of device memory (HRIR sphere)");
    }
    cudaMemcpy(d, sp->ir.data(), sp->ir.size() * sizeof(float), cudaMemcpyHostToDevice);
    cudaMemcpy(dpos, sp->pos.data(), sp->pos.size() * sizeof(float), cudaMemcpyHostToDevice);
    cudaMemcpy(dtri, sp->tri.data(), sp->tri.size() * sizeof(uint32_t), cudaMemcpyHostToDevice);
    CUDA_TRY(cudaStreamSynchronize(eng->stream));
    if (eng->d_sphere_ir) cudaFree(eng->d_sphere_ir);
    if (eng->d_sphere_pos) cudaFree(eng->d_sphere_pos);
    if (eng->d_sphere_tri) cudaFree(eng->d_sphere_tri);
    eng->drop_rate_spheres();
    eng->d_sphere_pos = dpos;
    eng->d_sphere_tri = dtri;
    delete eng->sphere;
    eng->sphere = sp;
    eng->d_sphere_ir = d;
    return WAE_OK;
}

WAE_API wae_status wae_engine_stream(wae_engine* eng, void** out_stream) {
    *out_stream = (void*)eng->stream;
    return WAE_OK;
}

WAE_API wae_status wae_engine_set_option(wae_engine* eng, uint32_t option, int64_t value) {
    switch (option) {
        case WAE_OPT_CHUNK_FRAMES:
            if (value < 0 || value % 128 != 0) return fail(WAE_INVALID_ARGUMENT, "chunk frames must be a multiple of 128");
            eng->chunk_frames = value;
            return WAE_OK;
        case WAE_OPT_FUSE: eng->fuse = value != 0; return WAE_OK;
        case WAE_OPT_VOICE_SUM: eng->voice_sum = value < 0 ? 0 : (value > 2 ? 2 : (int)value); return WAE_OK;
        case WAE_OPT_SERIAL_FILTERS: eng->serial_filters = value != 0; return WAE_OK;
        case WAE_OPT_PIPELINE_GROUPS:
            if (value < 0 || value > 1024) return fail(WAE_INVALID_ARGUMENT, "pipeline groups must be in [0, 1024]");
            eng->pipeline_groups = (int)value;
            return WAE_OK;
        case WAE_OPT_PARAM_PARALLEL: eng->param_parallel = value > 2 ? 2 : (int)value; return WAE_OK;
        case WAE_OPT_BIND_NUMA:
            if (value != 0 && eng->pool) return fail(WAE_INVALID_STATE, "bind the engine to its NUMA node before its first render (worker threads already run)");
            if (value != 0 && !bind_to_device_numa_node(eng)) return fail(WAE_UNSUPPORTED, "could not read / apply the CPU list of the GPU's NUMA node");
            return WAE_OK;
        case WAE_OPT_HOST_WORKERS:
            if (value < 0 || value > 256) return fail(WAE_INVALID_ARGUMENT, "host workers must be in [0, 256]");
            if (eng->pool) return fail(WAE_INVALID_STATE, "the worker threads already run");
            eng->n_workers = (int)value;
            return WAE_OK;
        case WAE_OPT_CHAIN_TMA: chain_set_tuning(value != 0 ? 1 : 0, -1); return WAE_OK;
        case WAE_OPT_CHAIN_WAVES:
            if (value < 0 || value > 1024) return fail(WAE_INVALID_ARGUMENT, "chain waves must be in [0, 1024]");
            chain_set_tuning(-1, (int)value);
            return WAE_OK;
        case WAE_OPT_CHAIN_PREPASS: chain_set_prepass(value != 0 ? 1 : 0); return WAE_OK;
        default: return fail(WAE_INVALID_ARGUMENT, "unknown option");
    }
}

WAE_API wae_status wae_batch_destroy(wae_batch* b) {
    if (!b) return WAE_OK;
    cudaSetDevice(b->engine->device);
    if (b->engine->stream) {
        cudaStreamSynchronize(b->engine->stream);
        cudaStreamSynchronize(b->engine->s_h2d);
        cudaStreamSynchronize(b->engine->s_d2h);
    }
    for (void* h : b->pinned) cudaFreeHost(h);
    for (auto& g : b->groups) {
        if (g.ev_h2d) cudaEventDestroy(g.ev_h2d);
        if (g.ev_done) cudaEventDestroy(g.ev_done);
    }
    for (void* p : b->allocs) b->engine->dev_release(p);
    if (b->ev0) cudaEventDestroy(b->ev0);
    if (b->ev1) cudaEventDestroy(b->ev1);
    for (auto e : b->stage_events) cudaEventDestroy(e);
    delete b;
    return WAE_OK;
}

WAE_API wae_status wae_graph_render_order(wae_graph* g, wae_node_id* ids, uint32_t cap, uint32_t* n) {
    if (!g || !n || (cap && !ids)) return fail(WAE_INVALID_ARGUMENT, "null argument");
    Orderer o;
    o.g = g;
    o.run();
    *n = (uint32_t)o.ordered.size();
    for (uint32_t i = 0; i < *n && i < cap; i++) ids[i] = o.ordered[i];
    return WAE_OK;
}

struct PrepState {
    std::map<std::pair<uint32_t, uint32_t>, int> delay_ch_hint;
    std::unordered_map<uint64_t, Planner::IrSpectra> ir_cache;
    uint64_t algorithmic_bytes = 0;
    std::chrono::steady_clock::time_point t0, t1;
};
struct GroupPlan {
    std::vector<Stage> stages;
    std::vector<std::pair<size_t, size_t>> seg_ranges;
    uint64_t algorithmic_bytes = 0;
    int code = WAE_OK;
    std::string error;
};

static wae_status prep_begin(wae_engine* eng, wae_graph* const* graphs, uint32_t n_graphs, wae_plan_info* plan, wae_batch** out_b, PrepState& ps,
                             bool want_d_out) {
    if (!eng || !graphs || n_graphs == 0) return fail(WAE_INVALID_ARGUMENT, "null / empty batch");
    if (!plan) CUDA_TRY(cudaSetDevice(eng->device));
    for (uint32_t i = 0; i < n_graphs; i++) {
        if (!graphs[i]) return fail(WAE_INVALID_ARGUMENT, "null graph in the batch");
        if (graphs[i]->channels != graphs[0]->channels || graphs[i]->length != graphs[0]->length ||
            graphs[i]->sample_rate != graphs[0]->sample_rate)
            return fail(WAE_INVALID_ARGUMENT, "all graphs of a batch must share number_of_channels, length and sample_rate");
    }
    ps.t0 = std::chrono::steady_clock::now();
    auto* b = new wae_batch;
    b->engine = eng;
    b->s_h2d = eng->s_h2d;
    b->s_d2h = eng->s_d2h;
    b->n_graphs = n_graphs;
    b->channels = graphs[0]->channels;
    b->length = graphs[0]->length;
    b->lq = (int64_t)((b->length + 127) / 128 * 128);
    bool has_conv = false, has_hrtf = false;
    std::vector<char> graph_has_conv(n_graphs, 0);
    std::vector<std::vector<int64_t>> cuts(n_graphs);
    for (uint32_t i = 0; i < n_graphs; i++) {
        for (auto& kv : graphs[i]->nodes) {
            if (kv.second.kind == K_CONV && kv.second.buffer) graph_has_conv[i] = 1;
            if (kv.second.kind == K_PANNER && kv.second.panning_model == WAE_PANNING_HRTF) has_hrtf = true;
        }
        for (auto& ep : graphs[i]->epochs) {
            if ((int64_t)ep.frame > 0 && (int64_t)ep.frame < b->lq) cuts[i].push_back((int64_t)ep.frame);
            for (auto& kv : ep.nodes)
                if (kv.second.kind == K_CONV && kv.second.buffer) graph_has_conv[i] = 1;
        }
        has_conv = has_conv || graph_has_conv[i];
    }
    size_t out_floats = (size_t)n_graphs * b->channels * b->length;
    if (!plan && want_d_out) {
        b->d_out = b->dalloc<float>(out_floats, true);
        if (!b->d_out) {
            wae_batch_destroy(b);
            return fail(WAE_OUT_OF_MEMORY, "out of device memory (output PCM)");
        }
    }
    int n_groups = eng->pipeline_groups;
    if (n_groups == 0) n_groups = n_graphs >= 512 ? 32 : (n_graphs >= 64 ? 8 : 1);
    if (eng->pipeline_groups == 0 && n_graphs >= 512) {
        static const int env_groups = [] { const char* e = getenv("WAE_AUTO_GROUPS"); return e ? atoi(e) : 0; }();
        if (env_groups > 0) n_groups = env_groups;
    }
    n_groups = std::max(1, std::min<int>(n_groups, (int)n_graphs));
    {
        const uint32_t target = (n_graphs + (uint32_t)n_groups - 1) / (uint32_t)n_groups;
        uint32_t g0 = 0;
        for (uint32_t i = 1; i <= n_graphs; i++)
            if (i == n_graphs || cuts[i] != cuts[g0] || i - g0 >= target) {
                wae_batch::Group grp;
                grp.g0 = g0;
                grp.g1 = i;
                grp.seg_bounds.push_back(0);
                for (int64_t f : cuts[g0]) grp.seg_bounds.push_back(f);
                grp.seg_bounds.push_back(b->lq);
                b->groups.push_back(grp);
                g0 = i;
            }
        n_groups = (int)b->groups.size();
    }
    for (auto& grp : b->groups) {
        bool conv = false;
        for (uint32_t i = grp.g0; i < grp.g1; i++) conv = conv || graph_has_conv[i];
        if (!conv) continue;
        for (int64_t f : grp.seg_bounds)
            if (f != b->lq && f % WAE_CONV_BLOCK != 0) {
                wae_batch_destroy(b);
                return fail(WAE_UNSUPPORTED, "a suspend point that is not a multiple of the convolver partition (8192 frames) in a graph with a ConvolverNode is not lowered to the GPU");
            }
    }
    b->chunk = 2048;
    uint64_t fpf = 0;
    bool has_feedback = false;
    std::vector<std::vector<int>> plan_stage_lists;
    struct SizeOut {
        uint64_t fpf = 0;
        bool has_feedback = false;
        std::map<std::pair<uint32_t, uint32_t>, int> delay_ch_seen;
        std::vector<std::vector<int>> stage_lists;
        uint64_t digest = 1469598103934665603ull;
        int code = WAE_OK;
        std::string error;
    };
    WorkerPool* pool = (!plan && n_groups > 1 && n_graphs >= 64) ? eng->workers() : nullptr;
    bool converged = false;
    for (int iter = 0; iter < 8; iter++) {
        bool hints_changed = false;
        fpf = 0;
        plan_stage_lists.clear();
        std::vector<SizeOut> so(n_groups);
        struct RangeOut {
            uint64_t fpf = 0;
            size_t src_floats = 0;
            bool has_feedback = false;
            std::map<std::pair<uint32_t, uint32_t>, int> delay_ch_seen;
            std::vector<wae_batch::Group::SrcCopy> copies;
            std::vector<size_t> graph_base;
            Builds builds;
            int code = WAE_OK;
            std::string error;
        };
        auto size_range = [&](int k, uint32_t i0, uint32_t i1, RangeOut& ro, size_t cursor0) {
            Planner sizing{b, eng};
            sizing.dry = true;
            sizing.group_graphs = (int)(b->groups[k].g1 - b->groups[k].g0);
            sizing.delay_ch_hint = &ps.delay_ch_hint;
            sizing.d_src = reinterpret_cast<float*>(uintptr_t(256));
            sizing.src_copies = &ro.copies;
            sizing.src_cursor = cursor0;
            sizing.begin_segment(0, b->lq);
            for (uint32_t i = i0; i < i1; i++) {
                EpochView view(graphs[i], 0);
                ro.graph_base.push_back(sizing.src_cursor);
                if (!sizing.plan_graph(graphs[i], i)) {
                    ro.code = sizing.error_code;
                    ro.error = sizing.error;
                    return;
                }
            }
            if (plan) ro.builds = std::move(sizing.builds);
            ro.fpf = sizing.arena_floats_per_frame;
            ro.src_floats = sizing.src_cursor - cursor0;
            ro.has_feedback = sizing.has_feedback;
            ro.delay_ch_seen = std::move(sizing.delay_ch_seen);
        };
        auto size_group_split = [&](int k, WorkerPool* wp, int parts, RangeOut& out, const std::vector<size_t>* known_base = nullptr) {
            const uint32_t g0 = b->groups[k].g0, n = b->groups[k].g1 - g0;
            std::vector<RangeOut> ro((size_t)parts);
            auto run = [&](int t) {
                const uint32_t i0 = (uint32_t)((uint64_t)n * t / parts), i1 = (uint32_t)((uint64_t)n * (t + 1) / parts);
                size_range(k, g0 + i0, g0 + i1, ro[t], known_base ? (*known_base)[i0] : 0);
            };
            if (wp) wp->parallel_for(parts, run);
            else
                for (int t = 0; t < parts; t++) run(t);
            for (auto& r : ro) {
                if (r.code != WAE_OK) {
                    out.code = r.code;
                    out.error = r.error;
                    return false;
                }
                const size_t rebase = known_base ? 0 : out.src_floats;
                for (auto& c : r.copies) out.copies.push_back(wae_batch::Group::SrcCopy{c.buf, c.offset + rebase, c.floats});
                for (size_t gb : r.graph_base) out.graph_base.push_back(gb + rebase);
                if (plan) merge_builds(out.builds, r.builds);
                out.fpf += r.fpf;
                out.src_floats += r.src_floats;
                out.has_feedback = out.has_feedback || r.has_feedback;
                for (auto& kv : r.delay_ch_seen) out.delay_ch_seen[kv.first] = kv.second;
            }
            return true;
        };
        auto group_nodes = [&](int k) {
            size_t nn = 0;
            for (uint32_t i = b->groups[k].g0; i < b->groups[k].g1; i++) nn += graphs[i]->nodes.size();
            return nn;
        };
        static const bool check_split = [] { const char* e = getenv("WAE_PLAN_PARALLEL"); return e && atoi(e) != 0; }();
        auto size_group = [&](int k) {
            const uint32_t n_in_group = b->groups[k].g1 - b->groups[k].g0;
            const bool one_segment = b->groups[k].seg_bounds.size() == 2;
            if (!plan && !pool && one_segment && n_in_group >= 2 && group_nodes(k) >= 4096) {
                WorkerPool* wp = eng->workers();
                RangeOut out;
                if (!size_group_split(k, wp, (int)std::min<uint32_t>(n_in_group, (uint32_t)wp->size()), out)) {
                    so[k].code = out.code;
                    so[k].error = out.error;
                    return;
                }
                b->groups[k].src_copies = std::move(out.copies);
                b->groups[k].graph_src_base = std::move(out.graph_base);
                b->groups[k].src_floats = out.src_floats;
                so[k].fpf = out.fpf;
                so[k].has_feedback = out.has_feedback;
                so[k].delay_ch_seen = std::move(out.delay_ch_seen);
                return;
            }
            Planner sizing{b, eng};
            sizing.dry = true;
            sizing.group_graphs = (int)n_in_group;
            sizing.delay_ch_hint = &ps.delay_ch_hint;
            sizing.d_src = reinterpret_cast<float*>(uintptr_t(256));
            b->groups[k].src_copies.clear();
            b->groups[k].graph_src_base.clear();
            sizing.src_copies = &b->groups[k].src_copies;
            const std::vector<int64_t>& bounds = b->groups[k].seg_bounds;
            uint64_t serial_digest = 0;
            for (size_t sg = 0; sg + 1 < bounds.size(); sg++) {
                sizing.begin_segment(bounds[sg], bounds[sg + 1]);
                for (uint32_t i = b->groups[k].g0; i < b->groups[k].g1; i++) {
                    EpochView view(graphs[i], bounds[sg]);
                    if (one_segment) b->groups[k].graph_src_base.push_back(sizing.src_cursor);
                    if (!sizing.plan_graph(graphs[i], i)) {
                        so[k].code = sizing.error_code;
                        so[k].error = sizing.error;
                        return;
                    }
                }
                so[k].fpf = std::max(so[k].fpf, sizing.arena_floats_per_frame);
                if (plan) {
                    std::vector<int> kinds;
                    for (auto& kv : sizing.builds) kinds.push_back(kv.second.kind);
                    so[k].stage_lists.push_back(std::move(kinds));
                    if (plan_digest_wanted()) so[k].digest = digest_builds(sizing.builds, so[k].digest);
                    if (check_split && one_segment) serial_digest = digest_builds(sizing.builds, 1469598103934665603ull);
                }
            }
            b->groups[k].src_floats = sizing.src_cursor;
            so[k].has_feedback = sizing.has_feedback;
            so[k].delay_ch_seen = std::move(sizing.delay_ch_seen);
            if (plan && check_split && one_segment && n_in_group >= 2) {
                RangeOut out;
                static const bool threaded = [] { const char* e = getenv("WAE_PLAN_PARALLEL"); return e && atoi(e) >= 2; }();
                std::unique_ptr<WorkerPool> tmp_pool(threaded ? new WorkerPool(3, 0) : nullptr);
                const bool ok = size_group_split(k, tmp_pool.get(), (int)std::min<uint32_t>(n_in_group, 3u), out);
                bool same = ok && out.fpf == so[k].fpf && out.src_floats == b->groups[k].src_floats && out.has_feedback == so[k].has_feedback &&
                            out.delay_ch_seen == so[k].delay_ch_seen && out.copies.size() == b->groups[k].src_copies.size() &&
                            out.graph_base == b->groups[k].graph_src_base;
                if (same) {
                    RangeOut abs_out;
                    same = size_group_split(k, nullptr, (int)std::min<uint32_t>(n_in_group, 3u), abs_out, &b->groups[k].graph_src_base) &&
                           abs_out.graph_base == b->groups[k].graph_src_base && digest_builds(abs_out.builds, 1469598103934665603ull) == serial_digest;
                }
                for (size_t c = 0; same && c < out.copies.size(); c++) {
                    const auto& x = out.copies[c];
                    const auto& y = b->groups[k].src_copies[c];
                    same = x.buf == y.buf && x.offset == y.offset && x.floats == y.floats;
                }
                if (!same) {
                    so[k].code = WAE_INVALID_STATE;
                    so[k].error = "internal: the split sizing pass disagrees with the serial one";
                }
            }
        };
        if (pool) pool->parallel_for(n_groups, size_group);
        else
            for (int k = 0; k < n_groups; k++) size_group(k);
        for (int k = 0; k < n_groups; k++) {
            if (so[k].code != WAE_OK) {
                int code = so[k].code;
                std::string msg = so[k].error;
                wae_batch_destroy(b);
                return fail(code, msg);
            }
            fpf = std::max(fpf, so[k].fpf);
            has_feedback = has_feedback || so[k].has_feedback;
            for (auto& l : so[k].stage_lists) plan_stage_lists.push_back(std::move(l));
            if (plan && plan_digest_wanted()) std::fprintf(stderr, "[wae plan digest] group %d fpf %llu src %zu: %016llx\n", k, (unsigned long long)so[k].fpf, b->groups[k].src_floats, (unsigned long long)so[k].digest);
            for (auto& kv : so[k].delay_ch_seen) {
                auto it = ps.delay_ch_hint.find(kv.first);
                int cur = it == ps.delay_ch_hint.end() ? 1 : it->second;
                if (cur != kv.second) {
                    ps.delay_ch_hint[kv.first] = kv.second;
                    hints_changed = true;
                }
            }
        }
        if (!hints_changed) {
            converged = true;
            break;
        }
    }
    if (!converged) {
        wae_batch_destroy(b);
        return fail(WAE_UNSUPPORTED, "the channel layout of DelayNodes inside feedback cycles did not settle (graph not lowered to the GPU)");
    }
    ps.t1 = std::chrono::steady_clock::now();
    b->arena_bytes = 0;
    b->asset_bytes = 0;
    int64_t chunk = eng->chunk_frames;
    if (chunk == 0) {
        if (fpf == 0) {
            chunk = b->lq;
        } else {
            chunk = (int64_t)(1024.0 * 1024 * 1024 / (4.0 * (double)fpf));
            chunk = std::max<int64_t>(8192, std::min<int64_t>(chunk, 1 << 20));
            chunk = chunk / 2048 * 2048;
        }
        if (has_conv || has_hrtf) chunk = std::max<int64_t>(chunk, 8 * WAE_CONV_BLOCK);
    }
    (void)has_feedback;
    if (has_conv || has_hrtf) chunk = (chunk + WAE_CONV_BLOCK - 1) / WAE_CONV_BLOCK * WAE_CONV_BLOCK;
    if (chunk > b->lq) chunk = (has_conv || has_hrtf) ? (b->lq + WAE_CONV_BLOCK - 1) / WAE_CONV_BLOCK * WAE_CONV_BLOCK : b->lq;
    b->chunk = chunk;
    if (plan) {
        std::memset(plan, 0, sizeof *plan);
        plan->groups = (uint32_t)n_groups;
        plan->chunk_frames = (uint64_t)chunk;
        plan->chunks = (uint64_t)((b->lq + chunk - 1) / chunk);
        plan->arena_floats_per_frame = fpf;
        plan->has_feedback = has_feedback ? 1u : 0u;
        uint32_t per_kind[S_KINDS] = {0};
        for (auto& grp : b->groups) {
            plan->source_floats += grp.src_floats;
            plan->segments += (uint32_t)grp.seg_bounds.size() - 1;
        }
        for (auto& kinds : plan_stage_lists) {
            plan->stages += (uint32_t)kinds.size();
            for (int k : kinds) per_kind[k]++;
        }
        std::string txt;
        for (int k = 0; k < S_KINDS; k++)
            if (per_kind[k]) txt += (txt.empty() ? "" : ", ") + std::string(kStageNames[k]) + " x " + std::to_string(per_kind[k]);
        std::snprintf(plan->stage_kinds, sizeof plan->stage_kinds, "%s", txt.c_str());
        delete b;
        *out_b = nullptr;
        return WAE_OK;
    }
    for (auto& grp : b->groups) {
        if (cudaEventCreateWithFlags(&grp.ev_h2d, cudaEventDisableTiming) != cudaSuccess ||
            cudaEventCreateWithFlags(&grp.ev_done, cudaEventDisableTiming) != cudaSuccess) {
            const std::string msg = std::string("prepare: cudaEventCreate: ") + cudaGetErrorString(cudaGetLastError());
            wae_batch_destroy(b);
            return fail(WAE_CUDA_ERROR, msg);
        }
        if (grp.src_floats) {
            grp.d_src = b->dalloc<float>(grp.src_floats, false);
            if (!grp.d_src) {
                wae_batch_destroy(b);
                return fail(WAE_OUT_OF_MEMORY, "out of device memory (source PCM slab)");
            }
        }
    }
    *out_b = b;
    return WAE_OK;
}

static void prep_plan_group(wae_batch* b, wae_graph* const* graphs, int k, PrepState& ps, GroupPlan& gp) {
    wae_engine* eng = b->engine;
    wae_batch::Group& grp = b->groups[k];
    Planner pl{b, eng};
    pl.d_src = grp.d_src;
    pl.group_graphs = (int)(grp.g1 - grp.g0);
    pl.src_copies = nullptr;
    pl.delay_ch_hint = &ps.delay_ch_hint;
    pl.ir_cache = &ps.ir_cache;
    auto oom = [&](const char* what) {
        gp.code = WAE_OUT_OF_MEMORY;
        gp.error = std::string("out of device memory (") + what + ")";
    };
    int split_parts = 0;
    {
        static const bool split_on = [] { const char* e = getenv("WAE_PLAN_SPLIT"); return !e || atoi(e) != 0; }();
        const uint32_t n_in_group = grp.g1 - grp.g0;
        size_t nn = 0;
        for (uint32_t i = grp.g0; i < grp.g1; i++) nn += graphs[i]->nodes.size();
        if (split_on && b->groups.size() == 1 && grp.seg_bounds.size() == 2 && n_in_group >= 2 && nn >= 4096 && grp.graph_src_base.size() == n_in_group) {
            const int free_workers = eng->workers()->size() - 1;
            if (free_workers >= 2) split_parts = (int)std::min<uint32_t>(n_in_group, (uint32_t)free_workers);
        }
    }
    for (int sg = 0; sg + 1 < (int)grp.seg_bounds.size(); sg++) {
        pl.begin_segment(grp.seg_bounds[sg], grp.seg_bounds[sg + 1]);
        const uint64_t alg_before = pl.algorithmic_bytes;
        if (split_parts >= 2) {
            struct Run {
                Builds builds;
                uint64_t algorithmic_bytes = 0;
                int code = WAE_OK;
                std::string error;
            };
            std::vector<Run> runs((size_t)split_parts);
            const uint32_t n = grp.g1 - grp.g0;
            eng->workers()->parallel_for(split_parts, [&](int t) {
                const uint32_t i0 = (uint32_t)((uint64_t)n * t / split_parts), i1 = (uint32_t)((uint64_t)n * (t + 1) / split_parts);
                Planner rp{b, eng};
                rp.d_src = grp.d_src;
                rp.group_graphs = (int)n;
                rp.src_copies = nullptr;
                rp.delay_ch_hint = &ps.delay_ch_hint;
                rp.ir_cache = &ps.ir_cache;
                rp.src_cursor = grp.graph_src_base[i0];
                rp.begin_segment(grp.seg_bounds[sg], grp.seg_bounds[sg + 1]);
                for (uint32_t i = grp.g0 + i0; i < grp.g0 + i1; i++) {
                    EpochView view(graphs[i], grp.seg_bounds[sg]);
                    if (!rp.plan_graph(graphs[i], i)) {
                        runs[t].code = rp.error_code;
                        runs[t].error = rp.error;
                        return;
                    }
                }
                runs[t].builds = std::move(rp.builds);
                runs[t].algorithmic_bytes = rp.algorithmic_bytes;
            });
            for (auto& r : runs) {
                if (r.code != WAE_OK) {
                    gp.code = r.code;
                    gp.error = r.error;
                    return;
                }
                merge_builds(pl.builds, r.builds);
                pl.algorithmic_bytes += r.algorithmic_bytes;
            }
        } else
        for (uint32_t i = grp.g0; i < grp.g1; i++) {
            EpochView view(graphs[i], grp.seg_bounds[sg]);
            if (!pl.plan_graph(graphs[i], i)) {
                gp.code = pl.error_code;
                gp.error = pl.error;
                return;
            }
        }
        gp.algorithmic_bytes += (uint64_t)((double)(pl.algorithmic_bytes - alg_before) * (double)(pl.seg_end - pl.seg_start) / (double)b->lq);
        const size_t seg_stage0 = gp.stages.size();
        void* last_conv_inputs = nullptr;
        for (auto& kv : pl.builds) {
            StageBuild& s = kv.second;
            Stage st;
            st.seg = sg;
            st.cls = s.cls;
            st.kind = s.kind;
            st.variant = s.variant;
            st.group = k;
            st.max_ch = s.max_ch;
            switch (s.kind) {
                case S_MIX: {
                    for (auto& m : s.mix) {
                        bool simple = true, all_mono = m.n_edges > 0;
                        for (int e = 0; e < m.n_edges; e++) {
                            const MixEdge& ed = s.mix_edges[m.edge_offset + e];
                            bool same = ed.src_ch == m.out_ch;
                            bool dup = ed.src_ch == 1 && m.out_ch == 2 && m.interp == WAE_INTERPRETATION_SPEAKERS;
                            if (!(same || dup)) simple = false;
                            if (ed.src_ch != 1) all_mono = false;
                            if (ed.src.absolute || (ed.src.stride & 3) != 0 || (reinterpret_cast<uintptr_t>(ed.src.p) & 15) != 0) simple = false;
                        }
                        m.simple = simple ? 1 : 0;
                        m.all_mono = (simple && all_mono && (m.out_ch == 1 || (m.out_ch == 2 && m.interp == WAE_INTERPRETATION_SPEAKERS))) ? 1 : 0;
                    }
                    st.n = (int)s.mix.size(); st.d_a = up(b, s.mix); st.d_b = up(b, s.mix_edges);
                    for (auto& m : s.mix) st.n_b = std::max(st.n_b, (int)m.n_edges);
                    break;
                }
                case S_MIX_DYN: {
                    for (auto& m : s.mix_dyn) {
                        bool ok = m.out_ch <= 2;
                        for (int e = 0; e < m.n_edges && ok; e++) {
                            const MixEdge& ed = s.mix_edges[m.edge_offset + e];
                            if (ed.src_ch > 2 || ed.src.absolute || (ed.src.stride & 3) != 0 || (reinterpret_cast<uintptr_t>(ed.src.p) & 15) != 0) ok = false;
                        }
                        m.stereo4 = ok ? 1 : 0;
                    }
                    st.n = (int)s.mix_dyn.size(); st.d_a = up(b, s.mix_dyn); st.d_b = up(b, s.mix_edges);
                    break;
                }
                case S_META: st.n = (int)s.meta.size(); st.d_a = up(b, s.meta); break;
                case S_OSC: st.n = (int)s.osc.size(); st.d_a = up(b, s.osc); break;
                case S_CONST: st.n = (int)s.cst.size(); st.d_a = up(b, s.cst); break;
                case S_ABSN: st.n = (int)s.absn.size(); st.d_a = up(b, s.absn); break;
                case S_BIQUAD: st.n = (int)s.biquad.size(); st.d_a = up(b, s.biquad); break;
                case S_CHAIN: {
                    st.n = (int)s.chain.size(); st.d_a = up(b, s.chain); st.d_b = up(b, s.scan_coef);
                    const int nb = (s.variant % 6) / 2;
                    int slabs = 1, tps = 1;
                    int pre_log2 = -1;
                    if (nb > 0) chain_plan_slabs(st.n, st.max_ch, (int)std::min<int64_t>(b->chunk, pl.seg_end - pl.seg_start), nb, &slabs, &tps, &pre_log2);
                    if (slabs > 1) {
                        const size_t slots = (size_t)st.n * st.max_ch * slabs;
                        st.chain.slab_stride = slabs;
                        st.chain.ticket = b->dalloc<unsigned>(1, true);
                        st.chain.flags = b->dalloc<unsigned>(slots, true);
                        st.chain.handoff = b->dalloc<double>(slots * CHAIN_MAX_BIQUADS * 4);
                        if (!st.chain.ticket || !st.chain.flags || !st.chain.handoff) return oom("chain hand-off");
                    }
                    break;
                }
                case S_VSUM: {
                    st.n = (int)s.vgroups.size(); st.d_a = up(b, s.chain); st.d_b = up(b, s.scan_coef); st.d_c = up(b, s.vgroups);
                    const int64_t nf_max = std::min<int64_t>(b->chunk, pl.seg_end - pl.seg_start);
                    const int tiles = (int)((nf_max + 2047) / 2048);
                    st.chain.slab_stride = tiles;
                    st.chain.ticket = b->dalloc<unsigned>(1, true);
                    st.chain.flags = b->dalloc<unsigned>((size_t)st.n * tiles, true);
                    st.chain.handoff = b->dalloc<double>(s.chain.size() * 2 * 4);
                    if (!st.chain.ticket || !st.chain.flags || !st.chain.handoff) return oom("voice-sum hand-off");
                    break;
                }
                case S_PARAM: st.n = (int)s.param.size(); st.d_a = up(b, s.param); break;
                case S_OSC_AR: st.n = (int)s.osc_ar.size(); st.d_a = up(b, s.osc_ar); break;
                case S_BIQUAD_AR: st.n = (int)s.biquad_ar.size(); st.d_a = up(b, s.biquad_ar); break;
                case S_ABSN_SLOW: st.n = (int)s.absn_slow.size(); st.d_a = up(b, s.absn_slow); break;
                case S_IIR: st.n = (int)s.iir.size(); st.d_a = up(b, s.iir); break;
                case S_GAIN: st.n = (int)s.gain.size(); st.d_a = up(b, s.gain); break;
                case S_SHAPER: st.n = (int)s.shaper.size(); st.d_a = up(b, s.shaper); break;
                case S_SPAN: st.n = (int)s.span.size(); st.d_a = up(b, s.span); st.d_b = up(b, s.span_gains); break;
                case S_PAN: st.n = (int)s.pan.size(); st.d_a = up(b, s.pan); break;
                case S_HRTF: st.n = (int)s.hrtf.size(); st.d_a = up(b, s.hrtf); st.max_ch = s.hrtf.empty() ? 0 : s.hrtf[0].L;
                    st.n_b = (int)s.hrtf_sel.size(); st.d_b = up(b, s.hrtf_sel); break;
                case S_PAN_DYN: st.n = (int)s.pan_dyn.size(); st.d_a = up(b, s.pan_dyn); break;
                case S_ABSN_SERIAL: st.n = (int)s.absn_serial.size(); st.d_a = up(b, s.absn_serial); break;
                case S_SHAPER_OS: st.n = (int)s.shaper_os.size(); st.d_a = up(b, s.shaper_os); break;
                case S_ROUTE: st.n = (int)s.route.size(); st.d_a = up(b, s.route); break;
                case S_DELAY_MONO:
                case S_DELAY:
                case S_DELAY_WRITE: st.n = (int)s.delay.size(); st.d_a = up(b, s.delay); break;
                case S_COMP: st.n = (int)s.comp.size(); st.d_a = up(b, s.comp); break;
                case S_ANALYSER: st.n = (int)s.analyser.size(); st.d_a = up(b, s.analyser); break;
                case S_CONV_FFT: st.n = (int)s.conv_in.size(); st.d_a = up(b, s.conv_in); last_conv_inputs = st.d_a; break;
                case S_CONV_CMP: st.n = (int)s.conv_cmp.size(); st.d_a = up(b, s.conv_cmp); break;
                case S_CONV_MAC:
                case S_CONV_MAC_ACC:
                    st.n = (int)s.conv_path.size();
                    st.d_a = up(b, s.conv_path);
                    st.d_b = last_conv_inputs;
                    break;
            }
            if (st.n > 0) {
                if (!st.d_a) return oom("stage tables");
                gp.stages.push_back(st);
            }
        }
        gp.seg_ranges.push_back({seg_stage0, gp.stages.size()});
    }
    b->flush_uploads();
}

static void prep_append_group(wae_batch* b, int k, PrepState& ps, GroupPlan& gp) {
    wae_batch::Group& grp = b->groups[k];
    grp.stage0 = b->stages.size();
    for (auto& r : gp.seg_ranges) grp.seg_stages.push_back({grp.stage0 + r.first, grp.stage0 + r.second});
    for (auto& st : gp.stages) b->stages.push_back(st);
    grp.stage1 = b->stages.size();
    ps.algorithmic_bytes += gp.algorithmic_bytes;
}

static wae_status enqueue_source_copies(wae_batch* b, wae_batch::Group& grp, cudaStream_t s) {
    for (auto& sc : grp.src_copies)
        CUDA_TRY(cudaMemcpyAsync(grp.d_src + sc.offset, sc.buf->base, sc.floats * sizeof(float), cudaMemcpyHostToDevice, s));
    return WAE_OK;
}

static wae_status prep_finish(wae_batch* b, PrepState& ps) {
    CUDA_TRY(cudaEventCreate(&b->ev0));
    CUDA_TRY(cudaEventCreate(&b->ev1));
    int64_t n_chunks = 0;
    for (auto& grp : b->groups)
    {
        int64_t c = 0;
        for (size_t sg = 0; sg + 1 < grp.seg_bounds.size(); sg++) c += (grp.seg_bounds[sg + 1] - grp.seg_bounds[sg] + b->chunk - 1) / b->chunk;
        n_chunks = std::max(n_chunks, c);
    }
    uint64_t launches = 0;
    for (auto& st : b->stages) {
        const uint64_t k = (st.kind == S_CONV_FFT || st.kind == S_CONV_MAC || st.kind == S_CONV_MAC_ACC || st.kind == S_SHAPER_OS) ? 2
                           : st.kind == S_HRTF ? (st.n_b > 0 ? 3 : 2) : st.kind == S_CONV_CMP ? 6 : 1;
        const std::vector<int64_t>& sb = b->groups[st.group].seg_bounds;
        const int64_t seg_len = sb[st.seg + 1] - sb[st.seg];
        launches += st.cls == 1 ? k * (uint64_t)(seg_len / 128) : k * (uint64_t)((seg_len + b->chunk - 1) / b->chunk);
    }
    std::memset(&b->stats, 0, sizeof(b->stats));
    b->stats.kernel_launches_per_run = launches;
    b->stats.stages = b->stages.size();
    b->stats.chunks = (uint64_t)n_chunks;
    b->stats.arena_bytes = b->arena_bytes;
    b->stats.asset_bytes = b->asset_bytes;
    b->stats.algorithmic_bytes = ps.algorithmic_bytes;
    b->stats.graph_quanta = (uint64_t)b->n_graphs * (uint64_t)(b->lq / 128);
    return WAE_OK;
}

static wae_status prepare_impl(wae_engine* eng, wae_graph* const* graphs, uint32_t n_graphs, wae_batch** out, wae_plan_info* plan) {
    if (!out && !plan) return fail(WAE_INVALID_ARGUMENT, "null out pointer");
    PrepState ps;
    wae_batch* b = nullptr;
    wae_status st = prep_begin(eng, graphs, n_graphs, plan, &b, ps, true);
    if (st != WAE_OK || plan) return st;
    const int n_groups = (int)b->groups.size();
    std::vector<GroupPlan> gps(n_groups);
    WorkerPool* pool = (n_groups > 1 && n_graphs >= 64) ? eng->workers() : nullptr;
    if (pool) pool->parallel_for(n_groups, [&](int k) { prep_plan_group(b, graphs, k, ps, gps[k]); });
    else
        for (int k = 0; k < n_groups; k++) prep_plan_group(b, graphs, k, ps, gps[k]);
    for (int k = 0; k < n_groups; k++) {
        if (gps[k].code != WAE_OK) {
            int code = gps[k].code;
            std::string msg = gps[k].error;
            wae_batch_destroy(b);
            return fail(code, msg);
        }
        prep_append_group(b, k, ps, gps[k]);
        wae_status cs = enqueue_source_copies(b, b->groups[k], eng->stream);
        if (cs != WAE_OK) {
            wae_batch_destroy(b);
            return cs;
        }
    }
    const auto t_prep2 = std::chrono::steady_clock::now();
    st = prep_finish(b, ps);
    if (st == WAE_OK && cudaStreamSynchronize(eng->stream) != cudaSuccess) st = fail(WAE_CUDA_ERROR, "prepare: stream synchronisation failed");
    if (st != WAE_OK) {
        wae_batch_destroy(b);
        return st;
    }
    if (getenv("WAE_PREPARE_PROFILE")) {
        const auto t_prep3 = std::chrono::steady_clock::now();
        auto ms = [](std::chrono::steady_clock::time_point a, std::chrono::steady_clock::time_point c) { return std::chrono::duration<double, std::milli>(c - a).count(); };
        std::fprintf(stderr, "[wae prepare] sizing %.1f ms, plan+alloc+upload %.1f ms, sync %.1f ms, fresh device blocks %llu, stages %zu\n", ms(ps.t0, ps.t1),
                     ms(ps.t1, t_prep2), ms(t_prep2, t_prep3), (unsigned long long)b->n_cuda_malloc, b->stages.size());
    }
    cudaError_t le = cudaGetLastError();
    if (le != cudaSuccess) {
        wae_batch_destroy(b);
        return fail(WAE_CUDA_ERROR, std::string("prepare: ") + cudaGetErrorString(le));
    }
    *out = b;
    return WAE_OK;
}

WAE_API wae_status wae_batch_prepare(wae_engine* eng, wae_graph* const* graphs, uint32_t n_graphs, wae_batch** out) {
    if (!out) return fail(WAE_INVALID_ARGUMENT, "null out pointer");
    return prepare_impl(eng, graphs, n_graphs, out, nullptr);
}

WAE_API wae_status wae_batch_plan(wae_graph* const* graphs, uint32_t n_graphs, wae_plan_info* info) {
    if (!info) return fail(WAE_INVALID_ARGUMENT, "null info pointer");
    wae_engine host_only;
    return prepare_impl(&host_only, graphs, n_graphs, nullptr, info);
}

static void launch_stage(wae_batch* b, Stage& st, ChunkInfo ci) {
    cudaStream_t s = b->engine->stream;
    switch (st.kind) {
        case S_MIX: launch_mix((MixInst*)st.d_a, (MixEdge*)st.d_b, st.n, ci, s, st.n_b); break;
        case S_MIX_DYN: launch_mix_dyn((MixDynInst*)st.d_a, (MixEdge*)st.d_b, st.n, ci, s); break;
        case S_META: launch_meta((MetaInst*)st.d_a, st.n, ci, s); break;
        case S_DELAY_MONO: launch_delay_mono((DelayInst*)st.d_a, st.n, ci, s); break;
        case S_OSC: launch_oscillator((OscInst*)st.d_a, st.n, ci, s); break;
        case S_CONST: launch_constant((ConstInst*)st.d_a, st.n, ci, s); break;
        case S_ABSN: launch_buffer_source((AbsnInst*)st.d_a, st.n, ci, s); break;
        case S_BIQUAD:
            launch_biquad_serial((BiquadInst*)st.d_a, st.n, st.max_ch, ci, s);
            break;
        case S_PARAM: launch_param((ParamInst*)st.d_a, st.n, ci, s, b->engine->param_parallel); break;
        case S_OSC_AR: launch_osc_arate((OscArInst*)st.d_a, st.n, ci, s); break;
        case S_ABSN_SLOW: launch_buffer_source_slow((AbsnSlowInst*)st.d_a, st.n, ci, s); break;
        case S_BIQUAD_AR: launch_biquad_arate((BiquadArInst*)st.d_a, st.n, st.max_ch, ci, s); break;
        case S_CHAIN:
            st.chain.epoch++;
            launch_chain(st.variant, (ChainInst*)st.d_a, (ScanCoef*)st.d_b, st.n, st.max_ch, ci, s, st.chain);
            break;
        case S_VSUM:
            st.chain.epoch++;
            launch_voice_sum(st.variant, (ChainInst*)st.d_a, (ScanCoef*)st.d_b, (VoiceGroup*)st.d_c, st.n, ci, s, st.chain);
            break;
        case S_IIR: launch_iir((IirInst*)st.d_a, st.n, st.max_ch, ci, s); break;
        case S_GAIN: launch_gain((GainInst*)st.d_a, st.n, ci, s); break;
        case S_SHAPER: launch_shaper((ShaperInst*)st.d_a, st.n, ci, s); break;
        case S_SPAN: launch_stereo_panner((SPanInst*)st.d_a, (float2*)st.d_b, st.n, ci, s); break;
        case S_PAN: launch_panner_eq((PanInst*)st.d_a, st.n, ci, s); break;
        case S_HRTF: launch_hrtf((HrtfInst*)st.d_a, st.n, (HrtfSelInst*)st.d_b, st.n_b, st.max_ch, ci, s); break;
        case S_PAN_DYN: launch_panner_dyn((PanDynInst*)st.d_a, st.n, ci, s); break;
        case S_ABSN_SERIAL: launch_buffer_source_serial((AbsnSerialInst*)st.d_a, st.n, ci, s); break;
        case S_SHAPER_OS: launch_shaper_os((ShaperOsInst*)st.d_a, st.n, st.max_ch, ci, s); break;
        case S_ROUTE: launch_route((RouteInst*)st.d_a, st.n, ci, s); break;
        case S_DELAY: launch_delay_read((DelayInst*)st.d_a, st.n, ci, s); break;
        case S_DELAY_WRITE: launch_ring_write((DelayInst*)st.d_a, st.n, ci, s); break;
        case S_COMP: launch_compressor((CompInst*)st.d_a, st.n, ci, s); break;
        case S_ANALYSER: launch_analyser((AnalyserInst*)st.d_a, st.n, ci, s); break;
        case S_CONV_FFT: launch_conv_fft_in((ConvInput*)st.d_a, st.n, ci, s); break;
        case S_CONV_MAC:
        case S_CONV_MAC_ACC: launch_conv_mac_ifft((ConvPath*)st.d_a, (ConvInput*)st.d_b, st.n, ci, s); break;
        case S_CONV_CMP: launch_conv_compact((ConvCmpInst*)st.d_a, st.n, ci, s); break;
    }
}

static bool group_sources_pinned(const wae_batch::Group& g) {
    for (auto& sc : g.src_copies)
        if (!sc.buf->pinned) return false;
    return true;
}
static wae_status ensure_host_mirror(wae_batch* b) {
    for (auto& g : b->groups) {
        if (!g.src_floats || g.h_src || group_sources_pinned(g)) continue;
        void* hp = nullptr;
        if (cudaHostAlloc(&hp, g.src_floats * sizeof(float), cudaHostAllocDefault) != cudaSuccess) {
            cudaGetLastError();
            return fail(WAE_OUT_OF_MEMORY, "out of memory (pinned mirror of the source PCM)");
        }
        b->pinned.push_back(hp);
        g.h_src = (float*)hp;
        for (auto& sc : g.src_copies) std::memcpy(g.h_src + sc.offset, sc.buf->base, sc.floats * sizeof(float));
    }
    return WAE_OK;
}
static wae_status resend_group_sources(wae_batch* b, wae_batch::Group& g, cudaStream_t s) {
    if (!g.src_floats) return WAE_OK;
    if (g.h_src) {
        CUDA_TRY(cudaMemcpyAsync(g.d_src, g.h_src, g.src_floats * sizeof(float), cudaMemcpyHostToDevice, s));
        return WAE_OK;
    }
    return enqueue_source_copies(b, g, s);
}

WAE_API wae_status wae_batch_upload(wae_batch* b) {
    CUDA_TRY(cudaSetDevice(b->engine->device));
    wae_status ms = ensure_host_mirror(b);
    if (ms != WAE_OK) return ms;
    for (auto& g : b->groups) {
        ms = resend_group_sources(b, g, b->engine->stream);
        if (ms != WAE_OK) return ms;
    }
    return WAE_OK;
}

WAE_API wae_status wae_batch_set_timing(wae_batch* b, uint32_t per_stage) {
    b->time_stages = per_stage != 0;
    return WAE_OK;
}

static wae_status run_group(wae_batch* b, const wae_batch::Group& g) {
    cudaStream_t s = b->engine->stream;
    size_t e_prev = (size_t)-1;
    auto next_event = [&]() -> size_t {
        if (b->timed_events_used == b->stage_events.size()) {
            cudaEvent_t e;
            if (cudaEventCreate(&e) != cudaSuccess) return (size_t)-1;
            b->stage_events.push_back(e);
        }
        return b->timed_events_used++;
    };
    auto run = [&](size_t i, const ChunkInfo& ci) -> bool {
        launch_stage(b, b->stages[i], ci);
        if (b->time_stages) {
            size_t e = next_event();
            if (e == (size_t)-1) return false;
            if (cudaEventRecord(b->stage_events[e], s) != cudaSuccess) return false;
            b->timed.push_back({i, e_prev, e});
            e_prev = e;
        }
        return true;
    };
    for (size_t sg = 0; sg + 1 < g.seg_bounds.size(); sg++) {
        const size_t s0 = g.seg_stages[sg].first, s1 = g.seg_stages[sg].second;
        size_t c1 = s0, c2 = s0;
        while (c1 < s1 && b->stages[c1].cls == 0) c1++;
        c2 = c1;
        while (c2 < s1 && b->stages[c2].cls == 1) c2++;
        const int64_t seg_end = g.seg_bounds[sg + 1];
        for (int64_t f0 = g.seg_bounds[sg]; f0 < seg_end; f0 += b->chunk) {
            const ChunkInfo ci{f0, (int32_t)std::min<int64_t>(b->chunk, seg_end - f0), 0};
            if (b->time_stages) {
                e_prev = next_event();
                if (e_prev == (size_t)-1) return fail(WAE_CUDA_ERROR, "cudaEventCreate failed");
                CUDA_TRY(cudaEventRecord(b->stage_events[e_prev], s));
            }
            for (size_t i = s0; i < c1; i++)
                if (!run(i, ci)) return fail(WAE_CUDA_ERROR, "cudaEventRecord failed");
            if (c2 > c1)
                for (int32_t sub = 0; sub < ci.nf; sub += 128) {
                    const ChunkInfo cq{f0 + sub, 128, sub};
                    for (size_t i = c1; i < c2; i++)
                        if (!run(i, cq)) return fail(WAE_CUDA_ERROR, "cudaEventRecord failed");
                }
            for (size_t i = c2; i < s1; i++)
                if (!run(i, ci)) return fail(WAE_CUDA_ERROR, "cudaEventRecord failed");
        }
    }
    return WAE_OK;
}

static wae_status begin_run(wae_batch* b) {
    CUDA_TRY(cudaSetDevice(b->engine->device));
    cudaStream_t s = b->engine->stream;
    for (auto& z : b->zero_on_run) CUDA_TRY(cudaMemsetAsync(z.first, 0, z.second, s));
    b->timed.clear();
    b->timed_events_used = 0;
    for (auto& a : b->analysers) a.computed = false;
    CUDA_TRY(cudaEventRecord(b->ev0, s));
    return WAE_OK;
}

WAE_API wae_status wae_batch_run(wae_batch* b) {
    wae_status st = begin_run(b);
    if (st != WAE_OK) return st;
    for (auto& g : b->groups) {
        st = run_group(b, g);
        if (st != WAE_OK) return st;
    }
    CUDA_TRY(cudaEventRecord(b->ev1, b->engine->stream));
    cudaError_t le = cudaGetLastError();
    if (le != cudaSuccess) return fail(WAE_CUDA_ERROR, std::string("run: ") + cudaGetErrorString(le));
    return WAE_OK;
}

WAE_API wae_status wae_batch_group_count(wae_batch* b, uint32_t* n_groups) {
    if (!b || !n_groups) return fail(WAE_INVALID_ARGUMENT, "null argument");
    *n_groups = (uint32_t)b->groups.size();
    return WAE_OK;
}
WAE_API wae_status wae_batch_group_range(wae_batch* b, uint32_t group, uint32_t* first_graph, uint32_t* last_graph) {
    if (!b || !first_graph || !last_graph || group >= b->groups.size()) return fail(WAE_INVALID_ARGUMENT, "null argument / group out of range");
    *first_graph = b->groups[group].g0;
    *last_graph = b->groups[group].g1;
    return WAE_OK;
}
WAE_API wae_status wae_batch_run_group(wae_batch* b, uint32_t group) {
    if (!b || group >= b->groups.size()) return fail(WAE_INVALID_ARGUMENT, "null batch / group out of range");
    wae_status st = WAE_OK;
    if (group == 0) st = begin_run(b);
    else CUDA_TRY(cudaSetDevice(b->engine->device));
    if (st != WAE_OK) return st;
    st = run_group(b, b->groups[group]);
    if (st != WAE_OK) return st;
    if (group + 1 == b->groups.size()) CUDA_TRY(cudaEventRecord(b->ev1, b->engine->stream));
    cudaError_t le = cudaGetLastError();
    if (le != cudaSuccess) return fail(WAE_CUDA_ERROR, std::string("run_group: ") + cudaGetErrorString(le));
    return WAE_OK;
}

static wae_status run_pipelined(wae_batch* b, float* host_out, bool resend_sources) {
    wae_status st = resend_sources ? ensure_host_mirror(b) : WAE_OK;
    if (st != WAE_OK) return st;
    st = begin_run(b);
    if (st != WAE_OK) return st;
    cudaStream_t s = b->engine->stream;
    const size_t per_graph = (size_t)b->channels * b->length;
    for (auto& g : b->groups) {
        if (g.src_floats && resend_sources) {
            st = resend_group_sources(b, g, b->s_h2d);
            if (st != WAE_OK) return st;
            CUDA_TRY(cudaEventRecord(g.ev_h2d, b->s_h2d));
            CUDA_TRY(cudaStreamWaitEvent(s, g.ev_h2d, 0));
        }
        st = run_group(b, g);
        if (st != WAE_OK) return st;
        CUDA_TRY(cudaEventRecord(g.ev_done, s));
        CUDA_TRY(cudaStreamWaitEvent(b->s_d2h, g.ev_done, 0));
        CUDA_TRY(cudaMemcpyAsync(host_out + (size_t)g.g0 * per_graph, b->d_out + (size_t)g.g0 * per_graph,
                                 (size_t)(g.g1 - g.g0) * per_graph * sizeof(float), cudaMemcpyDeviceToHost, b->s_d2h));
    }
    CUDA_TRY(cudaEventRecord(b->ev1, s));
    CUDA_TRY(cudaStreamSynchronize(b->s_d2h));
    CUDA_TRY(cudaStreamSynchronize(s));
    cudaError_t le = cudaGetLastError();
    if (le != cudaSuccess) return fail(WAE_CUDA_ERROR, std::string("run_pipelined: ") + cudaGetErrorString(le));
    return WAE_OK;
}

WAE_API wae_status wae_batch_run_pipelined(wae_batch* b, float* host_out) { return run_pipelined(b, host_out, true); }

WAE_API wae_status wae_batch_sync(wae_batch* b) {
    CUDA_TRY(cudaSetDevice(b->engine->device));
    CUDA_TRY(cudaStreamSynchronize(b->engine->stream));
    float ms = 0.f;
    if (cudaEventElapsedTime(&ms, b->ev0, b->ev1) == cudaSuccess) b->stats.last_run_ms = ms;
    else cudaGetLastError();
    if (!b->timed.empty()) {
        for (auto& st : b->stages) st.ms = 0.f;
        for (auto& t : b->timed) {
            float v = 0.f;
            if (cudaEventElapsedTime(&v, b->stage_events[t.e0], b->stage_events[t.e1]) == cudaSuccess) b->stages[t.stage].ms += v;
            else cudaGetLastError();
        }
        int best = -1;
        for (size_t i = 0; i < b->stages.size(); i++)
            if (best < 0 || b->stages[i].ms > b->stages[best].ms) best = (int)i;
        if (best >= 0) {
            b->stats.dominant_kernel_ms = b->stages[best].ms;
            const char* nm = kStageNames[b->stages[best].kind];
            std::snprintf(b->stats.dominant_kernel, sizeof(b->stats.dominant_kernel), "%s", nm);
        }
    }
    return WAE_OK;
}

WAE_API wae_status wae_batch_output_device_ptr(wae_batch* b, float** out_dev, uint64_t* out_floats) {
    *out_dev = b->d_out;
    *out_floats = (uint64_t)b->n_graphs * b->channels * b->length;
    return WAE_OK;
}

WAE_API wae_status wae_batch_fetch(wae_batch* b, float* host_out) {
    CUDA_TRY(cudaSetDevice(b->engine->device));
    size_t bytes = (size_t)b->n_graphs * b->channels * b->length * sizeof(float);
    CUDA_TRY(cudaMemcpyAsync(host_out, b->d_out, bytes, cudaMemcpyDeviceToHost, b->engine->stream));
    CUDA_TRY(cudaStreamSynchronize(b->engine->stream));
    return WAE_OK;
}

WAE_API wae_status wae_batch_stage_time(wae_batch* b, uint32_t index, char* name64, float* ms, uint32_t* n_instances) {
    if (index >= b->stages.size()) return fail(WAE_INVALID_ARGUMENT, "stage index out of range");
    const Stage& st = b->stages[index];
    const char* nm = kStageNames[st.kind];
    std::snprintf(name64, 64, "%s", nm);
    *ms = st.ms;
    *n_instances = (uint32_t)st.n;
    return WAE_OK;
}

WAE_API wae_status wae_batch_get_stats(wae_batch* b, wae_batch_stats* out) {
    *out = b->stats;
    return WAE_OK;
}

static void copy_streaming(void* dst, const void* src, size_t n) {
    char* d = static_cast<char*>(dst);
    const char* sp = static_cast<const char*>(src);
    const size_t head = std::min(n, (size_t)((64 - (reinterpret_cast<uintptr_t>(d) & 63)) & 63));
    if (head) std::memcpy(d, sp, head);
    d += head; sp += head; n -= head;
    if ((reinterpret_cast<uintptr_t>(sp) & 15) == 0) {
        for (; n >= 64; n -= 64, d += 64, sp += 64) {
            const __m128i a = _mm_load_si128(reinterpret_cast<const __m128i*>(sp)), b2 = _mm_load_si128(reinterpret_cast<const __m128i*>(sp + 16));
            const __m128i c = _mm_load_si128(reinterpret_cast<const __m128i*>(sp + 32)), e = _mm_load_si128(reinterpret_cast<const __m128i*>(sp + 48));
            _mm_stream_si128(reinterpret_cast<__m128i*>(d), a);
            _mm_stream_si128(reinterpret_cast<__m128i*>(d + 16), b2);
            _mm_stream_si128(reinterpret_cast<__m128i*>(d + 32), c);
            _mm_stream_si128(reinterpret_cast<__m128i*>(d + 48), e);
        }
    } else {
        for (; n >= 64; n -= 64, d += 64, sp += 64) {
            const __m128i a = _mm_loadu_si128(reinterpret_cast<const __m128i*>(sp)), b2 = _mm_loadu_si128(reinterpret_cast<const __m128i*>(sp + 16));
            const __m128i c = _mm_loadu_si128(reinterpret_cast<const __m128i*>(sp + 32)), e = _mm_loadu_si128(reinterpret_cast<const __m128i*>(sp + 48));
            _mm_stream_si128(reinterpret_cast<__m128i*>(d), a);
            _mm_stream_si128(reinterpret_cast<__m128i*>(d + 16), b2);
            _mm_stream_si128(reinterpret_cast<__m128i*>(d + 32), c);
            _mm_stream_si128(reinterpret_cast<__m128i*>(d + 48), e);
        }
    }
    _mm_sfence();
    if (n) std::memcpy(d, sp, n);
}

static wae_status render_oneshot_host(wae_engine* eng, wae_graph* const* graphs, uint32_t n_graphs, float* out) {
    if (!out) return fail(WAE_INVALID_ARGUMENT, "null output buffer");
    PrepState ps;
    wae_batch* b = nullptr;
    wae_status st = prep_begin(eng, graphs, n_graphs, nullptr, &b, ps, true);
    if (st != WAE_OK) return st;
    const int n_groups = (int)b->groups.size();
    const size_t per_graph = (size_t)b->channels * b->length;
    cudaStream_t s = eng->stream;
    WorkerPool* pool = eng->workers();
    std::mutex mu;
    std::condition_variable cv;
    int pending = 0;
    std::vector<char> planned(n_groups, 0);
    std::vector<GroupPlan> gps(n_groups);
    auto task_done = [&] {
        std::lock_guard<std::mutex> lk(mu);
        pending--;
        cv.notify_all();
    };
    auto drain = [&] {
        std::unique_lock<std::mutex> lk(mu);
        cv.wait(lk, [&] { return pending == 0; });
    };
    wae_status result = WAE_OK;
    std::string result_msg;
    auto set_fail = [&](wae_status code, const std::string& msg) {
        if (result == WAE_OK) {
            result = code;
            result_msg = msg;
        }
    };
    for (int k = 0; k < n_groups && result == WAE_OK; k++) {
        wae_batch::Group& grp = b->groups[k];
        if (!grp.src_floats) continue;
        if (enqueue_source_copies(b, grp, eng->s_h2d) != WAE_OK || cudaEventRecord(grp.ev_h2d, eng->s_h2d) != cudaSuccess)
            set_fail(WAE_CUDA_ERROR, std::string("one-shot render: H2D of the source PCM failed: ") + wae_last_error());
    }
    if (result == WAE_OK) {
        std::lock_guard<std::mutex> lk(mu);
        pending += n_groups;
    }
    if (result == WAE_OK)
        for (int k = 0; k < n_groups; k++)
            pool->submit([&, k] {
                prep_plan_group(b, graphs, k, ps, gps[k]);
                {
                    std::lock_guard<std::mutex> lk(mu);
                    planned[k] = 1;
                }
                task_done();
            });
    bool out_pinned = false;
    {
        cudaPointerAttributes attr;
        if (cudaPointerGetAttributes(&attr, out) == cudaSuccess) out_pinned = attr.type == cudaMemoryTypeHost;
        else cudaGetLastError();
    }
    size_t max_group_bytes = 0;
    for (auto& grp : b->groups) max_group_bytes = std::max(max_group_bytes, (size_t)(grp.g1 - grp.g0) * per_graph * sizeof(float));
    static const bool use_ring = [] { const char* e = getenv("WAE_STAGE_RING"); return e && atoi(e) != 0; }();
    static const size_t piece_bytes = [] { const char* e = getenv("WAE_STAGE_PIECE_KB"); long kb = e ? atol(e) : 2048; return (size_t)std::max(64l, std::min(65536l, kb)) * 1024; }();
    static const int ring_slots = [] { const char* e = getenv("WAE_STAGE_SLOTS"); int n = e ? atoi(e) : 8; return std::max(2, std::min(64, n)); }();
    const bool ring = !out_pinned && use_ring;
    if (result == WAE_OK && ring && !eng->ensure_ring(piece_bytes * (size_t)ring_slots)) set_fail(WAE_OUT_OF_MEMORY, "out of memory (page-locked staging ring of the rendered PCM)");
    if (result == WAE_OK && !out_pinned && !ring && !eng->ensure_stage(max_group_bytes)) set_fail(WAE_OUT_OF_MEMORY, "out of memory (page-locked staging of the rendered PCM)");
    std::vector<char> ring_busy(ring ? ring_slots : 0, 0);
    std::vector<cudaEvent_t> ring_ev(ring ? ring_slots : 0, nullptr);
    for (auto& e : ring_ev)
        if (result == WAE_OK && cudaEventCreateWithFlags(&e, cudaEventDisableTiming | cudaEventBlockingSync) != cudaSuccess) set_fail(WAE_CUDA_ERROR, "cudaEventCreate failed");
    int issued_groups = 0;
    bool pump_abort = false;
    std::string pump_error;
    std::thread pump;
    if (result == WAE_OK && ring)
        pump = std::thread([&] {
            cudaSetDevice(eng->device);
            size_t piece_no = 0;
            for (int k = 0; k < n_groups; k++) {
                {
                    std::unique_lock<std::mutex> lk(mu);
                    cv.wait(lk, [&] { return issued_groups > k || pump_abort; });
                    if (issued_groups <= k) return;
                }
                wae_batch::Group& grp = b->groups[k];
                if (cudaStreamWaitEvent(eng->s_d2h, grp.ev_done, 0) != cudaSuccess) {
                    std::lock_guard<std::mutex> lk(mu);
                    pump_error = "cudaStreamWaitEvent failed";
                    return;
                }
                const size_t off = (size_t)grp.g0 * per_graph * sizeof(float), bytes = (size_t)(grp.g1 - grp.g0) * per_graph * sizeof(float);
                for (size_t a0 = 0; a0 < bytes; a0 += piece_bytes, piece_no++) {
                    const size_t nb = std::min(piece_bytes, bytes - a0);
                    const int slot = (int)(piece_no % (size_t)ring_slots);
                    {
                        std::unique_lock<std::mutex> lk(mu);
                        cv.wait(lk, [&] { return !ring_busy[slot]; });
                        ring_busy[slot] = 1;
                        pending++;
                    }
                    char* stage = eng->h_ring + (size_t)slot * piece_bytes;
                    if (cudaMemcpyAsync(stage, (const char*)b->d_out + off + a0, nb, cudaMemcpyDeviceToHost, eng->s_d2h) != cudaSuccess ||
                        cudaEventRecord(ring_ev[slot], eng->s_d2h) != cudaSuccess) {
                        std::lock_guard<std::mutex> lk(mu);
                        pump_error = "D2H failed";
                        ring_busy[slot] = 0;
                        pending--;
                        cv.notify_all();
                        return;
                    }
                    char* dst = (char*)out + off + a0;
                    pool->submit([&, slot, stage, dst, nb] {
                        cudaEventSynchronize(ring_ev[slot]);
                        copy_streaming(dst, stage, nb);
                        {
                            std::lock_guard<std::mutex> lk(mu);
                            ring_busy[slot] = 0;
                        }
                        task_done();
                    });
                }
            }
        });
    constexpr int SLOTS = wae_engine::kStageSlots;
    bool slot_busy[SLOTS] = {false, false, false, false};
    std::vector<cudaEvent_t> ev_copy((out_pinned || ring) ? 0 : n_groups, nullptr);
    std::vector<std::unique_ptr<std::atomic<int>>> parts_left;
    for (auto& e : ev_copy)
        if (result == WAE_OK && cudaEventCreateWithFlags(&e, cudaEventDisableTiming | cudaEventBlockingSync) != cudaSuccess)
            set_fail(WAE_CUDA_ERROR, "cudaEventCreate failed");
    static const int env_parts = [] { const char* e = getenv("WAE_COPY_PARTS"); return e ? atoi(e) : 0; }();
    const int copy_parts = env_parts > 0 ? std::min(env_parts, 32) : std::max(1, std::min(8, pool->size() / 2));
    if (result == WAE_OK) {
        if (cudaEventCreate(&b->ev0) != cudaSuccess || cudaEventCreate(&b->ev1) != cudaSuccess || cudaEventRecord(b->ev0, s) != cudaSuccess)
            set_fail(WAE_CUDA_ERROR, "cudaEventCreate failed");
    }
    for (int k = 0; k < n_groups && result == WAE_OK; k++) {
        {
            std::unique_lock<std::mutex> lk(mu);
            cv.wait(lk, [&] { return planned[k] != 0; });
        }
        if (gps[k].code != WAE_OK) {
            set_fail(gps[k].code, gps[k].error);
            break;
        }
        prep_append_group(b, k, ps, gps[k]);
        wae_batch::Group& grp = b->groups[k];
        if (grp.src_floats && cudaStreamWaitEvent(s, grp.ev_h2d, 0) != cudaSuccess) {
            set_fail(WAE_CUDA_ERROR, "cudaStreamWaitEvent failed");
            break;
        }
        if (run_group(b, grp) != WAE_OK) {
            set_fail(WAE_CUDA_ERROR, wae_last_error());
            break;
        }
        const size_t off = (size_t)grp.g0 * per_graph, bytes = (size_t)(grp.g1 - grp.g0) * per_graph * sizeof(float);
        if (cudaEventRecord(grp.ev_done, s) != cudaSuccess || (!ring && cudaStreamWaitEvent(eng->s_d2h, grp.ev_done, 0) != cudaSuccess)) {
            set_fail(WAE_CUDA_ERROR, "event record / wait failed");
            break;
        }
        if (out_pinned) {
            if (cudaMemcpyAsync(out + off, b->d_out + off, bytes, cudaMemcpyDeviceToHost, eng->s_d2h) != cudaSuccess) set_fail(WAE_CUDA_ERROR, "D2H failed");
            continue;
        }
        if (ring) {
            std::lock_guard<std::mutex> lk(mu);
            issued_groups = k + 1;
            cv.notify_all();
            continue;
        }
        const int slot = k % SLOTS;
        {
            std::unique_lock<std::mutex> lk(mu);
            cv.wait(lk, [&] { return !slot_busy[slot]; });
            slot_busy[slot] = true;
            pending += copy_parts;
        }
        if (cudaMemcpyAsync(eng->h_stage[slot], b->d_out + off, bytes, cudaMemcpyDeviceToHost, eng->s_d2h) != cudaSuccess ||
            cudaEventRecord(ev_copy[k], eng->s_d2h) != cudaSuccess) {
            set_fail(WAE_CUDA_ERROR, "D2H failed");
            std::lock_guard<std::mutex> lk(mu);
            pending -= copy_parts;
            slot_busy[slot] = false;
            break;
        }
        parts_left.emplace_back(new std::atomic<int>(copy_parts));
        std::atomic<int>* left = parts_left.back().get();
        for (int part = 0; part < copy_parts; part++)
            pool->submit([&, k, slot, part, left, off, bytes] {
                cudaEventSynchronize(ev_copy[k]);
                const size_t chunk = (bytes / copy_parts + 63) / 64 * 64;
                const size_t a0 = std::min(bytes, (size_t)part * chunk), a1 = std::min(bytes, a0 + chunk);
                static const bool nt = [] { const char* e = getenv("WAE_STAGE_NT"); return !e || atoi(e) != 0; }();
                if (a1 > a0) {
                    if (nt) copy_streaming((char*)(out + off) + a0, (const char*)eng->h_stage[slot] + a0, a1 - a0);
                    else std::memcpy((char*)(out + off) + a0, (const char*)eng->h_stage[slot] + a0, a1 - a0);
                }
                if (left->fetch_sub(1) == 1) {
                    std::lock_guard<std::mutex> lk(mu);
                    slot_busy[slot] = false;
                }
                task_done();
            });
    }
    if (result == WAE_OK && cudaEventRecord(b->ev1, s) != cudaSuccess) set_fail(WAE_CUDA_ERROR, "cudaEventRecord failed");
    if (pump.joinable()) {
        {
            std::lock_guard<std::mutex> lk(mu);
            if (issued_groups < n_groups) pump_abort = true;
            cv.notify_all();
        }
        pump.join();
        if (!pump_error.empty()) set_fail(WAE_CUDA_ERROR, "one-shot render: " + pump_error);
    }
    drain();
    if (cudaStreamSynchronize(eng->s_d2h) != cudaSuccess || cudaStreamSynchronize(s) != cudaSuccess || cudaStreamSynchronize(eng->s_h2d) != cudaSuccess)
        set_fail(WAE_CUDA_ERROR, std::string("one-shot render: ") + cudaGetErrorString(cudaGetLastError()));
    cudaError_t le = cudaGetLastError();
    if (le != cudaSuccess) set_fail(WAE_CUDA_ERROR, std::string("one-shot render: ") + cudaGetErrorString(le));
    for (auto& e : ev_copy)
        if (e) cudaEventDestroy(e);
    for (auto& e : ring_ev)
        if (e) cudaEventDestroy(e);
    wae_batch_destroy(b);
    if (result != WAE_OK) return fail(result, result_msg);
    return WAE_OK;
}

WAE_API wae_status wae_host_alloc(wae_engine* eng, uint64_t bytes, void** out) {
    if (!eng || !out || bytes == 0) return fail(WAE_INVALID_ARGUMENT, "null engine / out pointer or zero size");
    CUDA_TRY(cudaSetDevice(eng->device));
    if (cudaHostAlloc(out, bytes, cudaHostAllocPortable) != cudaSuccess) {
        cudaGetLastError();
        return fail(WAE_OUT_OF_MEMORY, "out of page-locked host memory");
    }
    return WAE_OK;
}
WAE_API wae_status wae_host_free(wae_engine* eng, void* p) {
    if (!eng) return fail(WAE_INVALID_ARGUMENT, "null engine");
    if (p) CUDA_TRY(cudaFreeHost(p));
    return WAE_OK;
}
WAE_API wae_status wae_host_register(wae_engine* eng, void* p, uint64_t bytes) {
    if (!eng || !p || bytes == 0) return fail(WAE_INVALID_ARGUMENT, "null engine / pointer or zero size");
    CUDA_TRY(cudaSetDevice(eng->device));
    if (cudaHostRegister(p, bytes, cudaHostRegisterPortable) != cudaSuccess) {
        const std::string msg = std::string("cudaHostRegister: ") + cudaGetErrorString(cudaGetLastError());
        return fail(WAE_CUDA_ERROR, msg);
    }
    return WAE_OK;
}
WAE_API wae_status wae_host_unregister(wae_engine* eng, void* p) {
    if (!eng || !p) return fail(WAE_INVALID_ARGUMENT, "null engine / pointer");
    CUDA_TRY(cudaHostUnregister(p));
    return WAE_OK;
}

WAE_API wae_status wae_selftest_conv_fft(float* data, uint32_t mode) {
    if (!data || mode > 3) return fail(WAE_INVALID_ARGUMENT, "wae_selftest_conv_fft: null data or mode > 3");
    conv_fft_selftest(data, (int)mode);
    return WAE_OK;
}

WAE_API wae_status wae_render_batch(wae_engine* eng, wae_graph* const* graphs, uint32_t n_graphs, float* out, uint32_t flags) {
    if (!(flags & WAE_RENDER_OUT_DEVICE)) return render_oneshot_host(eng, graphs, n_graphs, out);
    wae_batch* b = nullptr;
    wae_status st = wae_batch_prepare(eng, graphs, n_graphs, &b);
    if (st != WAE_OK) return st;
    st = wae_batch_run(b);
    if (st == WAE_OK) st = wae_batch_sync(b);
    if (st == WAE_OK) {
        size_t bytes = (size_t)b->n_graphs * b->channels * b->length * sizeof(float);
        cudaError_t e = cudaMemcpyAsync(out, b->d_out, bytes, cudaMemcpyDeviceToDevice, eng->stream);
        if (e == cudaSuccess) e = cudaStreamSynchronize(eng->stream);
        if (e != cudaSuccess) st = fail(WAE_CUDA_ERROR, cudaGetErrorString(e));
    }
    std::string saved = wae_last_error();
    wae_batch_destroy(b);
    if (st != WAE_OK) set_error(saved);
    return st;
}

static const AnalyserRec* find_analyser(wae_batch* b, uint32_t gi, wae_node_id node) {
    for (auto& a : b->analysers)
        if (a.graph_index == gi && a.node == node) return &a;
    return nullptr;
}

WAE_API wae_status wae_analyser_get_float_time_domain_data(wae_batch* b, uint32_t graph_index, wae_node_id node, float* out, uint32_t len) {
    const AnalyserRec* a = find_analyser(b, graph_index, node);
    if (!a) return fail(WAE_INVALID_ARGUMENT, "not an analyser of this batch");
    const uint32_t RING = 32768 + 128;
    std::vector<float> ring(RING);
    CUDA_TRY(cudaSetDevice(b->engine->device));
    CUDA_TRY(cudaMemcpy(ring.data(), a->d_ring, RING * sizeof(float), cudaMemcpyDeviceToHost));
    uint32_t n = std::min(len, a->fft_size);
    uint64_t write_index = (uint64_t)b->lq % RING;
    for (uint32_t i = 0; i < n; i++) out[i] = ring[(RING + write_index - n + i) % RING];
    return WAE_OK;
}

WAE_API wae_status wae_analyser_get_float_frequency_data(wae_batch* b, uint32_t graph_index, wae_node_id node, float* out, uint32_t len) {
    AnalyserRec* a = const_cast<AnalyserRec*>(find_analyser(b, graph_index, node));
    if (!a) return fail(WAE_INVALID_ARGUMENT, "not an analyser of this batch");
    CUDA_TRY(cudaSetDevice(b->engine->device));
    const uint32_t RING = 32768 + 128;
    const uint32_t bins = a->fft_size / 2;
    if (!a->computed) {
        launch_analyser_fft(a->d_ring, (uint32_t)((uint64_t)b->lq % RING), (int)a->fft_size, (float)a->smoothing, a->d_last_fft, a->d_db,
                            b->engine->stream);
        a->computed = true;
    }
    uint32_t n = std::min(len, bins);
    CUDA_TRY(cudaMemcpyAsync(out, a->d_db, n * sizeof(float), cudaMemcpyDeviceToHost, b->engine->stream));
    CUDA_TRY(cudaStreamSynchronize(b->engine->stream));
    return WAE_OK;
}

WAE_API wae_status wae_analyser_get_byte_time_domain_data(wae_batch* b, uint32_t graph_index, wae_node_id node, uint8_t* out, uint32_t len) {
    std::vector<float> tmp(len, 0.f);
    wae_status st = wae_analyser_get_float_time_domain_data(b, graph_index, node, tmp.data(), len);
    if (st != WAE_OK) return st;
    const AnalyserRec* a = find_analyser(b, graph_index, node);
    const uint32_t n = std::min(len, a->fft_size);
    for (uint32_t i = 0; i < n; i++) {
        float scaled = 128.f * (1.f + tmp[i]);
        scaled = scaled < 0.f ? 0.f : (scaled > 255.f ? 255.f : scaled);
        out[i] = (uint8_t)scaled;
    }
    return WAE_OK;
}

WAE_API wae_status wae_analyser_get_byte_frequency_data(wae_batch* b, uint32_t graph_index, wae_node_id node, uint8_t* out, uint32_t len) {
    const AnalyserRec* a = find_analyser(b, graph_index, node);
    if (!a) return fail(WAE_INVALID_ARGUMENT, "not an analyser of this batch");
    const uint32_t n = std::min(len, a->fft_size / 2);
    std::vector<float> db(n, 0.f);
    wae_status st = wae_analyser_get_float_frequency_data(b, graph_index, node, db.data(), n);
    if (st != WAE_OK) return st;
    const float mn = (float)a->min_db, mx = (float)a->max_db;
    for (uint32_t i = 0; i < n; i++) {
        float scaled = 255.f / (mx - mn) * (db[i] - mn);
        scaled = !(scaled > 0.f) ? 0.f : (scaled > 255.f ? 255.f : scaled);
        out[i] = (uint8_t)scaled;
    }
    return WAE_OK;
}

WAE_API wae_status wae_compressor_reduction(wae_batch* b, uint32_t graph_index, wae_node_id node, float* out) {
    if (!b || !out) return fail(WAE_INVALID_ARGUMENT, "null argument");
    for (auto& c : b->compressors)
        if (c.graph == graph_index && c.node == node) {
            CUDA_TRY(cudaSetDevice(b->engine->device));
            CUDA_TRY(cudaMemcpyAsync(out, c.d_state + 1, sizeof(float), cudaMemcpyDeviceToHost, b->engine->stream));
            CUDA_TRY(cudaStreamSynchronize(b->engine->stream));
            return WAE_OK;
        }
    return fail(WAE_INVALID_ARGUMENT, "not a dynamics compressor of this batch");
}

WAE_API wae_status wae_resample_linear(wae_engine* eng, const float* in, uint64_t len, float from_rate, float to_rate, float* out,
                                       uint64_t out_cap, uint64_t* out_len) {
    if (!eng || !in || !out || !out_len) return fail(WAE_INVALID_ARGUMENT, "null argument");
    if (std::fabs(from_rate - to_rate) <= 0.1f || len == 0) {
        if (out_cap < len) return fail(WAE_INVALID_ARGUMENT, "output capacity too small");
        std::memcpy(out, in, len * sizeof(float));
        *out_len = len;
        return WAE_OK;
    }
    uint64_t target = (uint64_t)std::ceil((double)len * ((double)to_rate / (double)from_rate));
    if (out_cap < target) return fail(WAE_INVALID_ARGUMENT, "output capacity too small");
    CUDA_TRY(cudaSetDevice(eng->device));
    float *d_in = nullptr, *d_out = nullptr;
    CUDA_TRY(cudaMalloc(&d_in, len * sizeof(float)));
    if (cudaMalloc(&d_out, target * sizeof(float)) != cudaSuccess) {
        cudaFree(d_in);
        return fail(WAE_OUT_OF_MEMORY, "out of device memory (resample)");
    }
    cudaMemcpyAsync(d_in, in, len * sizeof(float), cudaMemcpyHostToDevice, eng->stream);
    launch_resample_linear(d_in, (int64_t)len, d_out, (int64_t)target, eng->stream);
    cudaMemcpyAsync(out, d_out, target * sizeof(float), cudaMemcpyDeviceToHost, eng->stream);
    cudaError_t e = cudaStreamSynchronize(eng->stream);
    cudaFree(d_in);
    cudaFree(d_out);
    if (e != cudaSuccess) return fail(WAE_CUDA_ERROR, cudaGetErrorString(e));
    *out_len = target;
    return WAE_OK;
}

}
```

Baseline: 1.401 billion.

## Overlap producer and consumer chunk stages on two streams with double-buffered arena

After: 1.401 billion (median of 6 runs). About the same (+0.0%).

```diff
diff --git a/include/wae.h b/include/wae.h
--- a/include/wae.h
+++ b/include/wae.h
@@ -194,7 +194,8 @@
     WAE_OPT_CHAIN_TMA = 8,
     WAE_OPT_CHAIN_WAVES = 9,
     WAE_OPT_CHAIN_PREPASS = 10,
-    WAE_OPT_VOICE_SUM = 11
+    WAE_OPT_VOICE_SUM = 11,
+    WAE_OPT_CHUNK_OVERLAP = 12
 };
 WAE_API wae_status wae_engine_set_option(wae_engine* engine, uint32_t option, int64_t value);
 WAE_API wae_status wae_engine_stream(wae_engine* engine, void** out_stream);
@@ -290,6 +291,7 @@
     float last_run_ms;
     float dominant_kernel_ms;
     char dominant_kernel[64];
+    uint64_t overlapped_segments;
 } wae_batch_stats;
 WAE_API wae_status wae_batch_get_stats(wae_batch* batch, wae_batch_stats* out);
 WAE_API wae_status wae_batch_stage_time(wae_batch* batch, uint32_t index, char* name64, float* ms, uint32_t* n_instances);
diff --git a/web-audio-api-rs_b200/__init__.py b/web-audio-api-rs_b200/__init__.py
--- a/web-audio-api-rs_b200/__init__.py
+++ b/web-audio-api-rs_b200/__init__.py
@@ -68,3 +68,4 @@
 
 OPT_CHUNK_FRAMES, OPT_FUSE, OPT_SERIAL_FILTERS, OPT_PIPELINE_GROUPS, OPT_PARAM_PARALLEL = 1, 2, 3, 4, 5
 OPT_BIND_NUMA, OPT_HOST_WORKERS, OPT_CHAIN_TMA, OPT_CHAIN_WAVES, OPT_CHAIN_PREPASS, OPT_VOICE_SUM = 6, 7, 8, 9, 10, 11
+OPT_CHUNK_OVERLAP = 12
diff --git a/web-audio-api-rs_b200/_binding.py b/web-audio-api-rs_b200/_binding.py
--- a/web-audio-api-rs_b200/_binding.py
+++ b/web-audio-api-rs_b200/_binding.py
@@ -108,7 +108,7 @@
     _fields_ = [("kernel_launches_per_run", C.c_uint64), ("stages", C.c_uint64), ("chunks", C.c_uint64),
                 ("arena_bytes", C.c_uint64), ("asset_bytes", C.c_uint64), ("algorithmic_bytes", C.c_uint64),
                 ("graph_quanta", C.c_uint64), ("last_run_ms", C.c_float), ("dominant_kernel_ms", C.c_float),
-                ("dominant_kernel", C.c_char * 64)]
+                ("dominant_kernel", C.c_char * 64), ("overlapped_segments", C.c_uint64)]
 
 
 STATUS_NAMES = {0: "OK", 1: "INVALID_ARGUMENT", 2: "INVALID_STATE", 3: "NOT_SUPPORTED", 4: "UNSUPPORTED",
diff --git a/web-audio-api-rs_b200/csrc/wae_engine.cu b/web-audio-api-rs_b200/csrc/wae_engine.cu
--- a/web-audio-api-rs_b200/csrc/wae_engine.cu
+++ b/web-audio-api-rs_b200/csrc/wae_engine.cu
@@ -100,6 +100,8 @@
     int device = 0;
     cudaStream_t stream = nullptr;
     cudaStream_t s_h2d = nullptr, s_d2h = nullptr;
+    cudaStream_t s_consume = nullptr;
+    int chunk_overlap = 1;
     int64_t chunk_frames = 0;
     bool fuse = true;
     int voice_sum = -1;
@@ -297,6 +299,8 @@
     void* d_a = nullptr;
     void* d_b = nullptr;
     void* d_c = nullptr;
+    void* d_a1 = nullptr;
+    void* d_b1 = nullptr;
     float ms = 0.f;
     ChainAux chain;
 };
@@ -332,6 +336,7 @@
         uint32_t g0 = 0, g1 = 0;
         size_t stage0 = 0, stage1 = 0;
         std::vector<std::pair<size_t, size_t>> seg_stages;
+        std::vector<size_t> seg_prefix;
         std::vector<int64_t> seg_bounds;
         float* d_src = nullptr;
         float* h_src = nullptr;
@@ -361,6 +366,7 @@
     wae_batch_stats stats{};
     cudaEvent_t ev0 = nullptr, ev1 = nullptr;
     std::vector<cudaEvent_t> stage_events;
+    cudaEvent_t ev_fork = nullptr, ev_prod[2] = {nullptr, nullptr}, ev_cons[2] = {nullptr, nullptr};
     bool time_stages = false;
     size_t timed_events_used = 0;
     std::atomic<uint64_t> arena_bytes{0}, asset_bytes{0};
@@ -708,6 +714,8 @@
     }
     std::map<int, std::vector<float*>> arena_pool;
     std::map<int, size_t> arena_used;
+    std::map<float*, size_t> arena_sizes;
+    std::map<float*, float*> arena_twins;
     std::map<std::pair<uint32_t, uint32_t>, size_t> src_offsets;
     std::unordered_map<const PcmBuffer*, size_t> buf_offsets;
     struct ParamRecord {
@@ -797,11 +805,13 @@
                 r.p = pool[used++];
             } else {
                 const size_t floats = (size_t)ch * (size_t)b->chunk;
-                float* p = b->dalloc<float>(floats + ((size_t)ch * mstride + 3) / 4);
+                const size_t with_meta_floats = floats + ((size_t)ch * mstride + 3) / 4;
+                float* p = b->dalloc<float>(with_meta_floats);
                 b->arena_bytes += floats * 4;
                 if (p) {
                     pool.push_back(p);
                     used++;
+                    arena_sizes[p] = with_meta_floats;
                 }
                 r.p = p;
             }
@@ -2638,6 +2648,9 @@
     CUDA_TRY(cudaStreamCreateWithFlags(&eng->stream, cudaStreamNonBlocking));
     CUDA_TRY(cudaStreamCreateWithFlags(&eng->s_h2d, cudaStreamNonBlocking));
     CUDA_TRY(cudaStreamCreateWithFlags(&eng->s_d2h, cudaStreamNonBlocking));
+    int prio_greatest = 0;
+    CUDA_TRY(cudaDeviceGetStreamPriorityRange(nullptr, &prio_greatest));
+    CUDA_TRY(cudaStreamCreateWithPriority(&eng->s_consume, cudaStreamNonBlocking, prio_greatest));
     if (const char* e = getenv("WAE_BIND_NUMA"))
         if (atoi(e) != 0) bind_to_device_numa_node(eng);
     std::vector<float> sine = hm::sine_table();
@@ -2666,6 +2679,7 @@
     if (eng->stream) cudaStreamDestroy(eng->stream);
     if (eng->s_h2d) cudaStreamDestroy(eng->s_h2d);
     if (eng->s_d2h) cudaStreamDestroy(eng->s_d2h);
+    if (eng->s_consume) cudaStreamDestroy(eng->s_consume);
     delete eng;
     return WAE_OK;
 }
@@ -2742,6 +2756,7 @@
             chain_set_tuning(-1, (int)value);
             return WAE_OK;
         case WAE_OPT_CHAIN_PREPASS: chain_set_prepass(value != 0 ? 1 : 0); return WAE_OK;
+        case WAE_OPT_CHUNK_OVERLAP: eng->chunk_overlap = value != 0; return WAE_OK;
         default: return fail(WAE_INVALID_ARGUMENT, "unknown option");
     }
 }
@@ -2762,6 +2777,8 @@
     for (void* p : b->allocs) b->engine->dev_release(p);
     if (b->ev0) cudaEventDestroy(b->ev0);
     if (b->ev1) cudaEventDestroy(b->ev1);
+    for (cudaEvent_t e : {b->ev_fork, b->ev_prod[0], b->ev_prod[1], b->ev_cons[0], b->ev_cons[1]})
+        if (e) cudaEventDestroy(e);
     for (auto e : b->stage_events) cudaEventDestroy(e);
     delete b;
     return WAE_OK;
@@ -2786,10 +2803,127 @@
 struct GroupPlan {
     std::vector<Stage> stages;
     std::vector<std::pair<size_t, size_t>> seg_ranges;
+    std::vector<size_t> seg_prefix;
     uint64_t algorithmic_bytes = 0;
     int code = WAE_OK;
     std::string error;
 };
+
+extern "C++" {
+template <typename F>
+static void for_each_table(const StageBuild& s, F&& f) {
+    auto v = [&](const auto& vec) { f(reinterpret_cast<const char*>(vec.data()), vec.size() * sizeof(vec[0])); };
+    v(s.osc); v(s.cst); v(s.absn); v(s.biquad); v(s.chain); v(s.param); v(s.osc_ar); v(s.biquad_ar); v(s.absn_slow); v(s.scan_coef);
+    v(s.iir); v(s.gain); v(s.shaper); v(s.span); v(s.span_gains); v(s.pan); v(s.hrtf); v(s.hrtf_sel); v(s.pan_dyn); v(s.absn_serial);
+    v(s.shaper_os); v(s.route); v(s.delay); v(s.comp); v(s.analyser); v(s.mix); v(s.mix_edges); v(s.mix_dyn); v(s.meta); v(s.conv_in);
+    v(s.conv_path); v(s.conv_cmp); v(s.vgroups);
+}
+}
+
+static bool plan_overlap(wae_batch* b, Planner& pl, std::vector<Stage>& stages, size_t s0, const std::vector<const StageBuild*>& builds,
+                         size_t* prefix) {
+    const int64_t seg_len = pl.seg_end - pl.seg_start;
+    *prefix = 0;
+    const size_t s1 = stages.size();
+    if (!b->engine->chunk_overlap || seg_len <= b->chunk) return true;
+    auto reads_arena = [](const ChainInst& c) { return (c.in.p && !c.in.absolute) || (c.cst.track.p && !c.cst.track.absolute); };
+    size_t p = s0;
+    while (p < s1 && stages[p].kind == S_CHAIN && stages[p].cls == 0 && std::none_of(builds[p - s0]->chain.begin(), builds[p - s0]->chain.end(), reads_arena))
+        p++;
+    if (p == s0 || p == s1) return true;
+    for (size_t i = s0; i < s1; i++)
+        if (stages[i].cls != 0) return true;
+    auto alloc_of = [&](const void* q) -> float* {
+        auto it = pl.arena_sizes.upper_bound((float*)q);
+        if (it == pl.arena_sizes.begin()) return nullptr;
+        --it;
+        return (const float*)q < it->first + it->second ? it->first : nullptr;
+    };
+    std::map<float*, float*> twin;
+    for (size_t i = s0; i < p; i++)
+        for (const ChainInst& c : builds[i - s0]->chain) {
+            float* a = c.out.absolute ? nullptr : alloc_of(c.out.p);
+            if (!a) return true;
+            twin[a] = nullptr;
+        }
+    auto moved = [&](BufRef r) {
+        if (float* a = r.absolute ? nullptr : alloc_of(r.p)) {
+            auto it = twin.find(a);
+            if (it != twin.end()) {
+                float* t = it->second;
+                r.meta = r.meta && t ? reinterpret_cast<uint8_t*>(t) + (r.meta - reinterpret_cast<uint8_t*>(a)) : nullptr;
+                r.p = t ? t + (r.p - a) : nullptr;
+            }
+        }
+        return r;
+    };
+    std::vector<std::vector<ChainInst>> chains(s1 - s0);
+    std::vector<std::vector<MixEdge>> edges(s1 - s0);
+    std::vector<std::vector<ConvInput>> conv_ins(s1 - s0);
+    auto build_odd = [&]() {
+        for (size_t i = s0; i < s1; i++) {
+            const StageBuild& s = *builds[i - s0];
+            if (s.kind == S_CHAIN) {
+                chains[i - s0] = s.chain;
+                for (ChainInst& c : chains[i - s0]) {
+                    c.in = moved(c.in);
+                    c.out = moved(c.out);
+                }
+            } else if (s.kind == S_MIX || s.kind == S_MIX_DYN) {
+                edges[i - s0] = s.mix_edges;
+                for (MixEdge& e : edges[i - s0]) e.src = moved(e.src);
+            } else if (s.kind == S_CONV_FFT) {
+                conv_ins[i - s0] = s.conv_in;
+                for (ConvInput& ci : conv_ins[i - s0]) ci.in = moved(ci.in);
+            }
+        }
+    };
+    build_odd();
+    for (size_t i = s0; i < s1; i++) {
+        const StageBuild& s = *builds[i - s0];
+        for (const MetaInst& m : s.meta)
+            if (m.more) return true;
+        const char* replaced[3] = {reinterpret_cast<const char*>(s.chain.data()), reinterpret_cast<const char*>(s.mix_edges.data()),
+                                   reinterpret_cast<const char*>(s.conv_in.data())};
+        bool hit = false;
+        const uintptr_t lo = (uintptr_t)twin.begin()->first, hi = (uintptr_t)(twin.rbegin()->first + pl.arena_sizes[twin.rbegin()->first]);
+        auto scan = [&](const char* d, size_t bytes) {
+            for (size_t o = 0; o + sizeof(void*) <= bytes && !hit; o += sizeof(void*)) {
+                uintptr_t q;
+                std::memcpy(&q, d + o, sizeof q);
+                if (q < lo || q >= hi) continue;
+                if (float* a = alloc_of((const void*)q)) hit = twin.count(a) != 0;
+            }
+        };
+        for_each_table(s, [&](const char* d, size_t bytes) {
+            if (bytes == 0) return;
+            if (d == replaced[0] && !chains[i - s0].empty()) return;
+            if (d == replaced[1] && !edges[i - s0].empty()) return;
+            if (d == replaced[2] && !conv_ins[i - s0].empty()) return;
+            scan(d, bytes);
+        });
+        scan(reinterpret_cast<const char*>(chains[i - s0].data()), chains[i - s0].size() * sizeof(ChainInst));
+        scan(reinterpret_cast<const char*>(edges[i - s0].data()), edges[i - s0].size() * sizeof(MixEdge));
+        scan(reinterpret_cast<const char*>(conv_ins[i - s0].data()), conv_ins[i - s0].size() * sizeof(ConvInput));
+        if (hit) return true;
+    }
+    for (auto& kv : twin) {
+        float*& t = pl.arena_twins[kv.first];
+        if (!t) t = b->dalloc<float>(pl.arena_sizes[kv.first]);
+        if (!t) return false;
+        kv.second = t;
+    }
+    build_odd();
+    for (size_t i = s0; i < s1; i++) {
+        Stage& st = stages[i];
+        if (!chains[i - s0].empty()) st.d_a1 = up(b, chains[i - s0]);
+        else if (!edges[i - s0].empty()) st.d_b1 = up(b, edges[i - s0]);
+        else if (!conv_ins[i - s0].empty()) st.d_a1 = up(b, conv_ins[i - s0]);
+        if ((!chains[i - s0].empty() || !edges[i - s0].empty() || !conv_ins[i - s0].empty()) && !st.d_a1 && !st.d_b1) return false;
+    }
+    *prefix = p - s0;
+    return true;
+}
 
 static wae_status prep_begin(wae_engine* eng, wae_graph* const* graphs, uint32_t n_graphs, wae_plan_info* plan, wae_batch** out_b, PrepState& ps,
                              bool want_d_out) {
@@ -3153,6 +3287,7 @@
         if (split_parts >= 2) {
             struct Run {
                 Builds builds;
+                std::map<float*, size_t> arena_sizes;
                 uint64_t algorithmic_bytes = 0;
                 int code = WAE_OK;
                 std::string error;
@@ -3178,6 +3313,7 @@
                     }
                 }
                 runs[t].builds = std::move(rp.builds);
+                runs[t].arena_sizes = std::move(rp.arena_sizes);
                 runs[t].algorithmic_bytes = rp.algorithmic_bytes;
             });
             for (auto& r : runs) {
@@ -3187,6 +3323,7 @@
                     return;
                 }
                 merge_builds(pl.builds, r.builds);
+                pl.arena_sizes.insert(r.arena_sizes.begin(), r.arena_sizes.end());
                 pl.algorithmic_bytes += r.algorithmic_bytes;
             }
         } else
@@ -3200,6 +3337,7 @@
         }
         gp.algorithmic_bytes += (uint64_t)((double)(pl.algorithmic_bytes - alg_before) * (double)(pl.seg_end - pl.seg_start) / (double)b->lq);
         const size_t seg_stage0 = gp.stages.size();
+        std::vector<const StageBuild*> seg_builds;
         void* last_conv_inputs = nullptr;
         for (auto& kv : pl.builds) {
             StageBuild& s = kv.second;
@@ -3305,9 +3443,14 @@
             if (st.n > 0) {
                 if (!st.d_a) return oom("stage tables");
                 gp.stages.push_back(st);
-            }
-        }
+                seg_builds.push_back(&s);
+            }
+        }
+        size_t prefix = 0;
+        if (!plan_overlap(b, pl, gp.stages, seg_stage0, seg_builds, &prefix)) return oom("second copy of the voice buffers");
+        seg_builds.clear();
         gp.seg_ranges.push_back({seg_stage0, gp.stages.size()});
+        gp.seg_prefix.push_back(prefix);
     }
     b->flush_uploads();
 }
@@ -3316,6 +3459,7 @@
     wae_batch::Group& grp = b->groups[k];
     grp.stage0 = b->stages.size();
     for (auto& r : gp.seg_ranges) grp.seg_stages.push_back({grp.stage0 + r.first, grp.stage0 + r.second});
+    grp.seg_prefix = gp.seg_prefix;
     for (auto& st : gp.stages) b->stages.push_back(st);
     grp.stage1 = b->stages.size();
     ps.algorithmic_bytes += gp.algorithmic_bytes;
@@ -3327,9 +3471,16 @@
     return WAE_OK;
 }
 
+static bool create_overlap_events(wae_batch* b) {
+    for (cudaEvent_t* e : {&b->ev_fork, &b->ev_prod[0], &b->ev_prod[1], &b->ev_cons[0], &b->ev_cons[1]})
+        if (cudaEventCreateWithFlags(e, cudaEventDisableTiming) != cudaSuccess) return false;
+    return true;
+}
+
 static wae_status prep_finish(wae_batch* b, PrepState& ps) {
     CUDA_TRY(cudaEventCreate(&b->ev0));
     CUDA_TRY(cudaEventCreate(&b->ev1));
+    if (!create_overlap_events(b)) return fail(WAE_CUDA_ERROR, "cudaEventCreate failed");
     int64_t n_chunks = 0;
     for (auto& grp : b->groups)
     {
@@ -3349,6 +3500,8 @@
     b->stats.kernel_launches_per_run = launches;
     b->stats.stages = b->stages.size();
     b->stats.chunks = (uint64_t)n_chunks;
+    for (auto& grp : b->groups)
+        for (size_t p : grp.seg_prefix) b->stats.overlapped_segments += p > 0;
     b->stats.arena_bytes = b->arena_bytes;
     b->stats.asset_bytes = b->asset_bytes;
     b->stats.algorithmic_bytes = ps.algorithmic_bytes;
@@ -3415,49 +3568,50 @@
     return prepare_impl(&host_only, graphs, n_graphs, nullptr, info);
 }
 
-static void launch_stage(wae_batch* b, Stage& st, ChunkInfo ci) {
-    cudaStream_t s = b->engine->stream;
+static void launch_stage(wae_batch* b, Stage& st, ChunkInfo ci, cudaStream_t s, bool odd) {
+    void* const d_a = odd && st.d_a1 ? st.d_a1 : st.d_a;
+    void* const d_b = odd && st.d_b1 ? st.d_b1 : st.d_b;
     switch (st.kind) {
-        case S_MIX: launch_mix((MixInst*)st.d_a, (MixEdge*)st.d_b, st.n, ci, s, st.n_b); break;
-        case S_MIX_DYN: launch_mix_dyn((MixDynInst*)st.d_a, (MixEdge*)st.d_b, st.n, ci, s); break;
-        case S_META: launch_meta((MetaInst*)st.d_a, st.n, ci, s); break;
-        case S_DELAY_MONO: launch_delay_mono((DelayInst*)st.d_a, st.n, ci, s); break;
-        case S_OSC: launch_oscillator((OscInst*)st.d_a, st.n, ci, s); break;
-        case S_CONST: launch_constant((ConstInst*)st.d_a, st.n, ci, s); break;
-        case S_ABSN: launch_buffer_source((AbsnInst*)st.d_a, st.n, ci, s); break;
+        case S_MIX: launch_mix((MixInst*)d_a, (MixEdge*)d_b, st.n, ci, s, st.n_b); break;
+        case S_MIX_DYN: launch_mix_dyn((MixDynInst*)d_a, (MixEdge*)d_b, st.n, ci, s); break;
+        case S_META: launch_meta((MetaInst*)d_a, st.n, ci, s); break;
+        case S_DELAY_MONO: launch_delay_mono((DelayInst*)d_a, st.n, ci, s); break;
+        case S_OSC: launch_oscillator((OscInst*)d_a, st.n, ci, s); break;
+        case S_CONST: launch_constant((ConstInst*)d_a, st.n, ci, s); break;
+        case S_ABSN: launch_buffer_source((AbsnInst*)d_a, st.n, ci, s); break;
         case S_BIQUAD:
-            launch_biquad_serial((BiquadInst*)st.d_a, st.n, st.max_ch, ci, s);
+            launch_biquad_serial((BiquadInst*)d_a, st.n, st.max_ch, ci, s);
             break;
-        case S_PARAM: launch_param((ParamInst*)st.d_a, st.n, ci, s, b->engine->param_parallel); break;
-        case S_OSC_AR: launch_osc_arate((OscArInst*)st.d_a, st.n, ci, s); break;
-        case S_ABSN_SLOW: launch_buffer_source_slow((AbsnSlowInst*)st.d_a, st.n, ci, s); break;
-        case S_BIQUAD_AR: launch_biquad_arate((BiquadArInst*)st.d_a, st.n, st.max_ch, ci, s); break;
+        case S_PARAM: launch_param((ParamInst*)d_a, st.n, ci, s, b->engine->param_parallel); break;
+        case S_OSC_AR: launch_osc_arate((OscArInst*)d_a, st.n, ci, s); break;
+        case S_ABSN_SLOW: launch_buffer_source_slow((AbsnSlowInst*)d_a, st.n, ci, s); break;
+        case S_BIQUAD_AR: launch_biquad_arate((BiquadArInst*)d_a, st.n, st.max_ch, ci, s); break;
         case S_CHAIN:
             st.chain.epoch++;
-            launch_chain(st.variant, (ChainInst*)st.d_a, (ScanCoef*)st.d_b, st.n, st.max_ch, ci, s, st.chain);
+            launch_chain(st.variant, (ChainInst*)d_a, (ScanCoef*)d_b, st.n, st.max_ch, ci, s, st.chain);
             break;
         case S_VSUM:
             st.chain.epoch++;
-            launch_voice_sum(st.variant, (ChainInst*)st.d_a, (ScanCoef*)st.d_b, (VoiceGroup*)st.d_c, st.n, ci, s, st.chain);
+            launch_voice_sum(st.variant, (ChainInst*)d_a, (ScanCoef*)d_b, (VoiceGroup*)st.d_c, st.n, ci, s, st.chain);
             break;
-        case S_IIR: launch_iir((IirInst*)st.d_a, st.n, st.max_ch, ci, s); break;
-        case S_GAIN: launch_gain((GainInst*)st.d_a, st.n, ci, s); break;
-        case S_SHAPER: launch_shaper((ShaperInst*)st.d_a, st.n, ci, s); break;
-        case S_SPAN: launch_stereo_panner((SPanInst*)st.d_a, (float2*)st.d_b, st.n, ci, s); break;
-        case S_PAN: launch_panner_eq((PanInst*)st.d_a, st.n, ci, s); break;
-        case S_HRTF: launch_hrtf((HrtfInst*)st.d_a, st.n, (HrtfSelInst*)st.d_b, st.n_b, st.max_ch, ci, s); break;
-        case S_PAN_DYN: launch_panner_dyn((PanDynInst*)st.d_a, st.n, ci, s); break;
-        case S_ABSN_SERIAL: launch_buffer_source_serial((AbsnSerialInst*)st.d_a, st.n, ci, s); break;
-        case S_SHAPER_OS: launch_shaper_os((ShaperOsInst*)st.d_a, st.n, st.max_ch, ci, s); break;
-        case S_ROUTE: launch_route((RouteInst*)st.d_a, st.n, ci, s); break;
-        case S_DELAY: launch_delay_read((DelayInst*)st.d_a, st.n, ci, s); break;
-        case S_DELAY_WRITE: launch_ring_write((DelayInst*)st.d_a, st.n, ci, s); break;
-        case S_COMP: launch_compressor((CompInst*)st.d_a, st.n, ci, s); break;
-        case S_ANALYSER: launch_analyser((AnalyserInst*)st.d_a, st.n, ci, s); break;
-        case S_CONV_FFT: launch_conv_fft_in((ConvInput*)st.d_a, st.n, ci, s); break;
+        case S_IIR: launch_iir((IirInst*)d_a, st.n, st.max_ch, ci, s); break;
+        case S_GAIN: launch_gain((GainInst*)d_a, st.n, ci, s); break;
+        case S_SHAPER: launch_shaper((ShaperInst*)d_a, st.n, ci, s); break;
+        case S_SPAN: launch_stereo_panner((SPanInst*)d_a, (float2*)d_b, st.n, ci, s); break;
+        case S_PAN: launch_panner_eq((PanInst*)d_a, st.n, ci, s); break;
+        case S_HRTF: launch_hrtf((HrtfInst*)d_a, st.n, (HrtfSelInst*)d_b, st.n_b, st.max_ch, ci, s); break;
+        case S_PAN_DYN: launch_panner_dyn((PanDynInst*)d_a, st.n, ci, s); break;
+        case S_ABSN_SERIAL: launch_buffer_source_serial((AbsnSerialInst*)d_a, st.n, ci, s); break;
+        case S_SHAPER_OS: launch_shaper_os((ShaperOsInst*)d_a, st.n, st.max_ch, ci, s); break;
+        case S_ROUTE: launch_route((RouteInst*)d_a, st.n, ci, s); break;
+        case S_DELAY: launch_delay_read((DelayInst*)d_a, st.n, ci, s); break;
+        case S_DELAY_WRITE: launch_ring_write((DelayInst*)d_a, st.n, ci, s); break;
+        case S_COMP: launch_compressor((CompInst*)d_a, st.n, ci, s); break;
+        case S_ANALYSER: launch_analyser((AnalyserInst*)d_a, st.n, ci, s); break;
+        case S_CONV_FFT: launch_conv_fft_in((ConvInput*)d_a, st.n, ci, s); break;
         case S_CONV_MAC:
-        case S_CONV_MAC_ACC: launch_conv_mac_ifft((ConvPath*)st.d_a, (ConvInput*)st.d_b, st.n, ci, s); break;
-        case S_CONV_CMP: launch_conv_compact((ConvCmpInst*)st.d_a, st.n, ci, s); break;
+        case S_CONV_MAC_ACC: launch_conv_mac_ifft((ConvPath*)d_a, (ConvInput*)d_b, st.n, ci, s); break;
+        case S_CONV_CMP: launch_conv_compact((ConvCmpInst*)d_a, st.n, ci, s); break;
     }
 }
 
@@ -3506,8 +3660,8 @@
 }
 
 static wae_status run_group(wae_batch* b, const wae_batch::Group& g) {
-    cudaStream_t s = b->engine->stream;
-    size_t e_prev = (size_t)-1;
+    cudaStream_t s = b->engine->stream, sc = b->engine->s_consume;
+    size_t e_prev[2] = {(size_t)-1, (size_t)-1};
     auto next_event = [&]() -> size_t {
         if (b->timed_events_used == b->stage_events.size()) {
             cudaEvent_t e;
@@ -3516,41 +3670,71 @@
         }
         return b->timed_events_used++;
     };
-    auto run = [&](size_t i, const ChunkInfo& ci) -> bool {
-        launch_stage(b, b->stages[i], ci);
+    auto mark = [&](int k, cudaStream_t st) -> bool {
+        if (!b->time_stages) return true;
+        e_prev[k] = next_event();
+        return e_prev[k] != (size_t)-1 && cudaEventRecord(b->stage_events[e_prev[k]], st) == cudaSuccess;
+    };
+    auto run = [&](size_t i, const ChunkInfo& ci, int k, cudaStream_t st, bool odd) -> bool {
+        launch_stage(b, b->stages[i], ci, st, odd);
         if (b->time_stages) {
             size_t e = next_event();
             if (e == (size_t)-1) return false;
-            if (cudaEventRecord(b->stage_events[e], s) != cudaSuccess) return false;
-            b->timed.push_back({i, e_prev, e});
-            e_prev = e;
+            if (cudaEventRecord(b->stage_events[e], st) != cudaSuccess) return false;
+            b->timed.push_back({i, e_prev[k], e});
+            e_prev[k] = e;
         }
         return true;
     };
     for (size_t sg = 0; sg + 1 < g.seg_bounds.size(); sg++) {
         const size_t s0 = g.seg_stages[sg].first, s1 = g.seg_stages[sg].second;
+        const int64_t seg0 = g.seg_bounds[sg], seg_end = g.seg_bounds[sg + 1];
+        if (const size_t pe = s0 + g.seg_prefix[sg]; pe > s0) {
+            const int64_t n = (seg_end - seg0 + b->chunk - 1) / b->chunk;
+            auto chunk = [&](int64_t c) {
+                const int64_t f0 = seg0 + c * b->chunk;
+                return ChunkInfo{f0, (int32_t)std::min<int64_t>(b->chunk, seg_end - f0), 0};
+            };
+            CUDA_TRY(cudaEventRecord(b->ev_fork, s));
+            CUDA_TRY(cudaStreamWaitEvent(sc, b->ev_fork, 0));
+            for (int64_t c = -1; c < n; c++) {
+                if (c + 1 < n) {
+                    const int h = (int)((c + 1) & 1);
+                    if (c + 1 >= 2) CUDA_TRY(cudaStreamWaitEvent(s, b->ev_cons[h], 0));
+                    if (!mark(0, s)) return fail(WAE_CUDA_ERROR, "cudaEventRecord failed");
+                    for (size_t i = s0; i < pe; i++)
+                        if (!run(i, chunk(c + 1), 0, s, h != 0)) return fail(WAE_CUDA_ERROR, "cudaEventRecord failed");
+                    CUDA_TRY(cudaEventRecord(b->ev_prod[h], s));
+                }
+                if (c >= 0) {
+                    const int h = (int)(c & 1);
+                    CUDA_TRY(cudaStreamWaitEvent(sc, b->ev_prod[h], 0));
+                    if (!mark(1, sc)) return fail(WAE_CUDA_ERROR, "cudaEventRecord failed");
+                    for (size_t i = pe; i < s1; i++)
+                        if (!run(i, chunk(c), 1, sc, h != 0)) return fail(WAE_CUDA_ERROR, "cudaEventRecord failed");
+                    CUDA_TRY(cudaEventRecord(b->ev_cons[h], sc));
+                }
+            }
+            CUDA_TRY(cudaStreamWaitEvent(s, b->ev_cons[(n - 1) & 1], 0));
+            continue;
+        }
         size_t c1 = s0, c2 = s0;
         while (c1 < s1 && b->stages[c1].cls == 0) c1++;
         c2 = c1;
         while (c2 < s1 && b->stages[c2].cls == 1) c2++;
-        const int64_t seg_end = g.seg_bounds[sg + 1];
-        for (int64_t f0 = g.seg_bounds[sg]; f0 < seg_end; f0 += b->chunk) {
+        for (int64_t f0 = seg0; f0 < seg_end; f0 += b->chunk) {
             const ChunkInfo ci{f0, (int32_t)std::min<int64_t>(b->chunk, seg_end - f0), 0};
-            if (b->time_stages) {
-                e_prev = next_event();
-                if (e_prev == (size_t)-1) return fail(WAE_CUDA_ERROR, "cudaEventCreate failed");
-                CUDA_TRY(cudaEventRecord(b->stage_events[e_prev], s));
-            }
+            if (!mark(0, s)) return fail(WAE_CUDA_ERROR, "cudaEventCreate failed");
             for (size_t i = s0; i < c1; i++)
-                if (!run(i, ci)) return fail(WAE_CUDA_ERROR, "cudaEventRecord failed");
+                if (!run(i, ci, 0, s, false)) return fail(WAE_CUDA_ERROR, "cudaEventRecord failed");
             if (c2 > c1)
                 for (int32_t sub = 0; sub < ci.nf; sub += 128) {
                     const ChunkInfo cq{f0 + sub, 128, sub};
                     for (size_t i = c1; i < c2; i++)
-                        if (!run(i, cq)) return fail(WAE_CUDA_ERROR, "cudaEventRecord failed");
+                        if (!run(i, cq, 0, s, false)) return fail(WAE_CUDA_ERROR, "cudaEventRecord failed");
                 }
             for (size_t i = c2; i < s1; i++)
-                if (!run(i, ci)) return fail(WAE_CUDA_ERROR, "cudaEventRecord failed");
+                if (!run(i, ci, 0, s, false)) return fail(WAE_CUDA_ERROR, "cudaEventRecord failed");
         }
     }
     return WAE_OK;
@@ -3852,7 +4036,8 @@
     static const int env_parts = [] { const char* e = getenv("WAE_COPY_PARTS"); return e ? atoi(e) : 0; }();
     const int copy_parts = env_parts > 0 ? std::min(env_parts, 32) : std::max(1, std::min(8, pool->size() / 2));
     if (result == WAE_OK) {
-        if (cudaEventCreate(&b->ev0) != cudaSuccess || cudaEventCreate(&b->ev1) != cudaSuccess || cudaEventRecord(b->ev0, s) != cudaSuccess)
+        if (cudaEventCreate(&b->ev0) != cudaSuccess || cudaEventCreate(&b->ev1) != cudaSuccess || !create_overlap_events(b) ||
+            cudaEventRecord(b->ev0, s) != cudaSuccess)
             set_fail(WAE_CUDA_ERROR, "cudaEventCreate failed");
     }
     for (int k = 0; k < n_groups && result == WAE_OK; k++) {
```
